# openGemini/openGemini

Measured on NVIDIA H100. Metric: decoded+aggregated rows/s, higher is better.
Workload: dtype f64

## Files before the change

### include/ogpu.h

```cpp
#ifndef OGPU_H
#define OGPU_H

#include <stddef.h>
#include <stdint.h>

#ifdef __cplusplus
extern "C" {
#endif

#define OG_API __attribute__((visibility("default")))

enum {
    OG_OK = 0,
    OG_EOF = 1,
    OG_E_INVAL = -1,
    OG_E_CUDA = -2,
    OG_E_NOMEM = -3,
    OG_E_UNSUPPORTED = -4,
    OG_E_CORRUPT = -5,
    OG_E_ABORTED = -6,
    OG_E_TYPE = -7,
    OG_E_STATE = -8
};

enum { OG_TYPE_INT = 1, OG_TYPE_FLOAT = 3, OG_TYPE_STRING = 4, OG_TYPE_BOOL = 5 };

enum { OG_AGG_COUNT = 1, OG_AGG_SUM = 2, OG_AGG_MIN = 3, OG_AGG_MAX = 4, OG_AGG_FIRST = 5, OG_AGG_LAST = 6 };

enum { OG_F_TERM = 0, OG_F_AND = 1, OG_F_OR = 2 };
enum { OG_OP_LT = 0, OG_OP_LTE = 1, OG_OP_GT = 2, OG_OP_GTE = 3, OG_OP_EQ = 4, OG_OP_NEQ = 5 };

typedef struct og_filter_item {
    int32_t kind;
    int32_t column;
    int32_t op;
    int32_t const_is_float;
    double fval;
    int64_t ival;
} og_filter_item;

typedef struct og_call {
    int32_t func;
    int32_t column;
} og_call;

enum { OG_GROUP_ALL = 0, OG_GROUP_PER_SERIES = 1, OG_GROUP_MAP = 2 };
enum {
    OG_Q_STRICT_ORDER = 1u << 0
    ,
    OG_Q_NO_FUSED = 1u << 1
    ,
    OG_Q_NO_FAST = 1u << 2
    ,
    OG_Q_RESERVED_8 = 1u << 3
    ,
    OG_Q_QUERY_GRID = 1u << 4
};

typedef struct og_query_desc {
    int64_t interval;
    int64_t offset;
    int64_t tmin, tmax;
    int32_t ascending;
    uint32_t n_calls;
    const og_call *calls;
    uint32_t n_filter;
    const og_filter_item *filter;
    int32_t group_mode;
    uint32_t n_groups;
    const uint32_t *series_group;
    int32_t chunk_size;
    uint32_t flags;
} og_query_desc;

typedef struct og_column_desc {
    const char *name;
    int32_t type;
    const uint64_t *page_off;
    const uint32_t *page_len;
} og_column_desc;

enum {
    OG_SHARD_DEVICE_DATA = 1u << 0
};

typedef struct og_shard_desc {
    const uint8_t *data;
    uint64_t data_len;
    uint32_t n_series;
    const uint64_t *sids;
    const uint32_t *series_seg_begin;
    uint32_t n_segments;
    const int64_t *seg_tmin;
    const int64_t *seg_tmax;
    uint32_t n_columns;
    const og_column_desc *columns;
    const uint64_t *time_page_off;
    const uint32_t *time_page_len;
    uint32_t flags;
} og_shard_desc;

typedef struct og_colval_view {
    const uint8_t *val;
    uint64_t val_bytes;
    const uint8_t *bitmap;
    const int64_t *times;
    int32_t type;
    int32_t len;
    int32_t nil_count;
    int32_t bitmap_offset;
} og_colval_view;

typedef struct og_record_view {
    uint32_t n_cols;
    const og_colval_view *cols;
    const int64_t *times;
    int32_t rows;
    uint32_t group;
    uint64_t sid;
} og_record_view;

typedef struct og_dense_col {
    void *values;
    uint8_t *valid;
    int64_t *times;
    int32_t type;
    int32_t func;
} og_dense_col;

typedef struct og_dense_view {
    uint32_t n_groups;
    uint32_t n_buckets;
    int64_t start;
    int64_t interval;
    uint32_t n_cols;
    const og_dense_col *cols;
    void *stream;
} og_dense_view;

typedef struct og_stats {
    uint64_t rows_decoded;
    uint64_t segments_scanned;
    uint64_t page_bytes;
    uint64_t dir_bytes;
    uint64_t out_bytes;
    double kernel_ms;
    double h2d_ms;
    double main_kernel_ms;
    uint32_t kernel_launches;
    int32_t path;
    int32_t il_state;
    int32_t per_series_cells_used;
    double il_build_ms;
    uint64_t il_bytes;
    uint64_t general_segments;
    double merge_ms;
    uint64_t il_packed_segments;
} og_stats;

typedef struct og_shard og_shard;
typedef struct og_query og_query;

OG_API int og_init(int device_ordinal);
OG_API int og_device_count(void);
OG_API const char *og_strerror(int status);
OG_API const char *og_last_error(void);
OG_API const char *og_version(void);
OG_API int og_release_cached_memory(void);

typedef struct og_tssp og_tssp;
OG_API int og_tssp_parse(const uint8_t *file, uint64_t len, og_tssp **out);
OG_API int og_tssp_desc(const og_tssp *t, og_shard_desc *out);
OG_API const char *og_tssp_measurement(const og_tssp *t);
OG_API int og_tssp_time_range(const og_tssp *t, int64_t *min_time, int64_t *max_time);
OG_API void og_tssp_free(og_tssp *t);

OG_API int og_shard_open(const og_shard_desc *desc, og_shard **out);
OG_API void og_shard_close(og_shard *s);
OG_API int og_shard_info(const og_shard *s, uint64_t *n_series, uint64_t *n_segments, uint64_t *n_rows,
                         uint64_t *page_bytes, int64_t *tmin, int64_t *tmax);

enum { OG_FILE_OUT_OF_ORDER = 1u << 0 };
OG_API int og_shard_open_files(const og_shard_desc *files, const uint32_t *file_flags, uint32_t n_files, og_shard **out);
typedef struct og_merge_info {
    uint32_t n_files, n_out_of_order_files;
    uint64_t series_merged;
    uint64_t out_of_order_rows;
    uint64_t rows_replaced;
    uint64_t rows_after_merge;
    uint64_t segments_kept;
    uint64_t segments_rewritten_in, segments_rewritten_out;
    double merge_ms;
} og_merge_info;
OG_API int og_shard_merge_info(const og_shard *s, og_merge_info *out);

OG_API int og_query_create(og_shard *s, const og_query_desc *desc, og_query **out);
OG_API int og_query_run(og_query *q);
OG_API int og_query_next(og_query *q, og_record_view *out);
OG_API int og_query_dense(og_query *q, og_dense_view *out);
OG_API int og_query_stats(const og_query *q, og_stats *out);
OG_API void og_query_abort(og_query *q);
OG_API void og_query_destroy(og_query *q);

OG_API int og_query_merge_dense(og_query *q, const og_dense_view *other);

typedef struct og_comm og_comm;
OG_API int og_comm_unique_id(uint8_t id[128]);
OG_API int og_comm_init_rank(const uint8_t id[128], int rank, int world, og_comm **out);
OG_API void og_comm_destroy(og_comm *c);
OG_API int og_comm_info(const og_comm *c, int *rank, int *world, int *nccl_version);
OG_API int og_comm_allreduce_f64(og_comm *c, double *vals, int n, int op_max);
OG_API int og_query_allreduce(og_query *q, og_comm *c);

OG_API int og_decode_segment(og_shard *s, uint32_t segment, og_record_view *out);
enum { OG_DECODE_DESCENDING = 1u << 0 };
OG_API int og_decode_segment_ex(og_shard *s, uint32_t segment, uint32_t flags, og_record_view *out);
OG_API int og_decode_column_device(og_shard *s, uint32_t column, uint32_t seg_begin, uint32_t seg_end,
                                   void *d_values, uint64_t value_stride_bytes, uint32_t *d_rows_out);

enum { OG_SYNTH_F_HI = 0, OG_SYNTH_F_LO = 1, OG_SYNTH_INT_WALK = 2, OG_SYNTH_BOOL = 3 };
typedef struct og_synth_column {
    int32_t type;
    int32_t dist;
    uint32_t null_permille;
} og_synth_column;
typedef struct og_synth_desc {
    uint32_t n_series;
    uint32_t rows_per_series;
    uint32_t rows_per_segment;
    int64_t t0;
    int64_t dt;
    uint64_t seed;
    uint32_t n_columns;
    const og_synth_column *columns;
    uint32_t series_base;
} og_synth_desc;
OG_API int og_shard_synth(const og_synth_desc *desc, og_shard **out);
typedef struct og_shard_layout {
    uint64_t data_len;
    uint32_t n_series, n_segments, n_columns;
} og_shard_layout;
OG_API int og_shard_layout_get(const og_shard *s, og_shard_layout *out);
OG_API int og_shard_export(const og_shard *s, uint8_t *data, uint64_t *sids, uint32_t *series_seg_begin,
                           int64_t *seg_tmin, int64_t *seg_tmax, uint64_t *page_off ,
                           uint32_t *page_len, int32_t *col_types );

OG_API int og_encode_pages(int32_t type, int32_t is_time, const void *d_values, const uint8_t *d_valid,
                           const uint32_t *d_rows , uint32_t n_segments,
                           uint32_t rows_per_segment, uint8_t *d_out, uint64_t out_cap, uint64_t *d_page_off,
                           uint32_t *d_page_len, uint64_t *total_bytes_out);

typedef struct og_downsampled og_downsampled;
OG_API int og_downsample(og_shard *s, uint32_t column, int64_t interval, int64_t tmin, int64_t tmax, og_downsampled **out);

typedef struct og_downsample_ops {
    int32_t type;
    uint32_t n_funcs;
    const int32_t *funcs;
} og_downsample_ops;
typedef struct og_downsample_desc {
    int64_t interval, tmin, tmax;
    uint32_t n_types;
    const og_downsample_ops *ops;
} og_downsample_desc;
OG_API int og_downsample_shard(og_shard *s, const og_downsample_desc *d, og_downsampled **out);
OG_API int og_downsampled_timing(const og_downsampled *d, double phase_ms[4]);
OG_API int og_downsampled_desc(const og_downsampled *d, og_shard_desc *desc, uint64_t *rows );
OG_API int og_downsampled_export(const og_downsampled *d, uint8_t *host_data );
OG_API void og_downsampled_free(og_downsampled *d);

typedef struct og_tssp_write_desc {
    const char *measurement;
    uint32_t series_begin, series_end;
    uint32_t flags;
} og_tssp_write_desc;
typedef struct og_tssp_image og_tssp_image;
OG_API int og_shard_write_tssp(og_shard *s, const og_tssp_write_desc *d, og_tssp_image **out);
OG_API int og_tssp_image_size(const og_tssp_image *f, uint64_t *bytes);
OG_API int og_tssp_image_export(const og_tssp_image *f, uint8_t *host);
OG_API int og_tssp_image_timing(const og_tssp_image *f, double phase_ms[4]);
OG_API void og_tssp_image_free(og_tssp_image *f);

#ifdef __cplusplus
}
#endif
#endif
```

### opengemini_b200/_lib.py

```python
import ctypes as C
import os

_HERE = os.path.dirname(os.path.abspath(__file__))
LIB_PATH = os.environ.get("OGPU_LIB") or os.path.join(_HERE, "libogpu.so")

OG_OK, OG_EOF = 0, 1
OG_E_INVAL, OG_E_CUDA, OG_E_NOMEM, OG_E_UNSUPPORTED, OG_E_CORRUPT, OG_E_ABORTED, OG_E_TYPE, OG_E_STATE = -1, -2, -3, -4, -5, -6, -7, -8
TYPE_INT, TYPE_FLOAT, TYPE_STRING, TYPE_BOOL = 1, 3, 4, 5
AGG_COUNT, AGG_SUM, AGG_MIN, AGG_MAX, AGG_FIRST, AGG_LAST = 1, 2, 3, 4, 5, 6
F_TERM, F_AND, F_OR = 0, 1, 2
OP_LT, OP_LTE, OP_GT, OP_GTE, OP_EQ, OP_NEQ = 0, 1, 2, 3, 4, 5
GROUP_ALL, GROUP_PER_SERIES, GROUP_MAP = 0, 1, 2
Q_STRICT_ORDER = 1
Q_NO_FUSED = 2
Q_NO_FAST = 4
Q_QUERY_GRID = 16
SYNTH_F_HI, SYNTH_F_LO, SYNTH_INT_WALK, SYNTH_BOOL = 0, 1, 2, 3
SHARD_DEVICE_DATA = 1
FILE_OUT_OF_ORDER = 1

u8p, u32p, u64p, i64p, i32p = C.POINTER(C.c_uint8), C.POINTER(C.c_uint32), C.POINTER(C.c_uint64), C.POINTER(C.c_int64), C.POINTER(C.c_int32)


class FilterItem(C.Structure):
    _fields_ = [("kind", C.c_int32), ("column", C.c_int32), ("op", C.c_int32), ("const_is_float", C.c_int32),
                ("fval", C.c_double), ("ival", C.c_int64)]


class Call(C.Structure):
    _fields_ = [("func", C.c_int32), ("column", C.c_int32)]


class QueryDesc(C.Structure):
    _fields_ = [("interval", C.c_int64), ("offset", C.c_int64), ("tmin", C.c_int64), ("tmax", C.c_int64),
                ("ascending", C.c_int32), ("n_calls", C.c_uint32), ("calls", C.POINTER(Call)),
                ("n_filter", C.c_uint32), ("filter", C.POINTER(FilterItem)), ("group_mode", C.c_int32),
                ("n_groups", C.c_uint32), ("series_group", u32p), ("chunk_size", C.c_int32), ("flags", C.c_uint32)]


class ColumnDesc(C.Structure):
    _fields_ = [("name", C.c_char_p), ("type", C.c_int32), ("page_off", u64p), ("page_len", u32p)]


class ShardDesc(C.Structure):
    _fields_ = [("data", u8p), ("data_len", C.c_uint64), ("n_series", C.c_uint32), ("sids", u64p),
                ("series_seg_begin", u32p), ("n_segments", C.c_uint32), ("seg_tmin", i64p), ("seg_tmax", i64p),
                ("n_columns", C.c_uint32), ("columns", C.POINTER(ColumnDesc)), ("time_page_off", u64p),
                ("time_page_len", u32p), ("flags", C.c_uint32)]


class ColValView(C.Structure):
    _fields_ = [("val", u8p), ("val_bytes", C.c_uint64), ("bitmap", u8p), ("times", i64p), ("type", C.c_int32),
                ("len", C.c_int32), ("nil_count", C.c_int32), ("bitmap_offset", C.c_int32)]


class RecordView(C.Structure):
    _fields_ = [("n_cols", C.c_uint32), ("cols", C.POINTER(ColValView)), ("times", i64p), ("rows", C.c_int32),
                ("group", C.c_uint32), ("sid", C.c_uint64)]


class DenseCol(C.Structure):
    _fields_ = [("values", C.c_void_p), ("valid", C.c_void_p), ("times", C.c_void_p), ("type", C.c_int32), ("func", C.c_int32)]


class DenseView(C.Structure):
    _fields_ = [("n_groups", C.c_uint32), ("n_buckets", C.c_uint32), ("start", C.c_int64), ("interval", C.c_int64),
                ("n_cols", C.c_uint32), ("cols", C.POINTER(DenseCol)), ("stream", C.c_void_p)]


class Stats(C.Structure):
    _fields_ = [("rows_decoded", C.c_uint64), ("segments_scanned", C.c_uint64), ("page_bytes", C.c_uint64),
                ("dir_bytes", C.c_uint64), ("out_bytes", C.c_uint64), ("kernel_ms", C.c_double), ("h2d_ms", C.c_double), ("main_kernel_ms", C.c_double),
                ("kernel_launches", C.c_uint32), ("path", C.c_int32), ("il_state", C.c_int32), ("per_series_cells_used", C.c_int32),
                ("il_build_ms", C.c_double), ("il_bytes", C.c_uint64), ("general_segments", C.c_uint64), ("merge_ms", C.c_double),
                ("il_packed_segments", C.c_uint64)]


class SynthColumn(C.Structure):
    _fields_ = [("type", C.c_int32), ("dist", C.c_int32), ("null_permille", C.c_uint32)]


class SynthDesc(C.Structure):
    _fields_ = [("n_series", C.c_uint32), ("rows_per_series", C.c_uint32), ("rows_per_segment", C.c_uint32),
                ("t0", C.c_int64), ("dt", C.c_int64), ("seed", C.c_uint64), ("n_columns", C.c_uint32),
                ("columns", C.POINTER(SynthColumn)), ("series_base", C.c_uint32)]


class ShardLayout(C.Structure):
    _fields_ = [("data_len", C.c_uint64), ("n_series", C.c_uint32), ("n_segments", C.c_uint32), ("n_columns", C.c_uint32)]


class DownsampleOps(C.Structure):
    _fields_ = [("type", C.c_int32), ("n_funcs", C.c_uint32), ("funcs", i32p)]


class DownsampleDesc(C.Structure):
    _fields_ = [("interval", C.c_int64), ("tmin", C.c_int64), ("tmax", C.c_int64), ("n_types", C.c_uint32),
                ("ops", C.POINTER(DownsampleOps))]


class MergeInfo(C.Structure):
    _fields_ = [("n_files", C.c_uint32), ("n_out_of_order_files", C.c_uint32), ("series_merged", C.c_uint64),
                ("out_of_order_rows", C.c_uint64), ("rows_replaced", C.c_uint64), ("rows_after_merge", C.c_uint64),
                ("segments_kept", C.c_uint64), ("segments_rewritten_in", C.c_uint64), ("segments_rewritten_out", C.c_uint64),
                ("merge_ms", C.c_double)]


class TsspWriteDesc(C.Structure):
    _fields_ = [("measurement", C.c_char_p), ("series_begin", C.c_uint32), ("series_end", C.c_uint32), ("flags", C.c_uint32)]


EXPORTS = [
    "og_init", "og_device_count", "og_strerror", "og_last_error", "og_version", "og_shard_open", "og_shard_close",
    "og_shard_info", "og_query_create", "og_query_run", "og_query_next", "og_query_dense", "og_query_stats",
    "og_query_abort", "og_query_destroy", "og_query_merge_dense", "og_decode_segment", "og_decode_segment_ex", "og_decode_column_device",
    "og_shard_synth", "og_shard_layout_get", "og_shard_export", "og_encode_pages",
    "og_release_cached_memory", "og_comm_unique_id", "og_comm_init_rank", "og_comm_destroy", "og_comm_info", "og_comm_allreduce_f64", "og_query_allreduce",
    "og_downsample", "og_downsampled_desc", "og_downsampled_export", "og_downsampled_free",
    "og_downsample_shard", "og_downsampled_timing",
    "og_tssp_parse", "og_tssp_desc", "og_tssp_measurement", "og_tssp_time_range", "og_tssp_free",
    "og_shard_open_files", "og_shard_merge_info",
    "og_shard_write_tssp", "og_tssp_image_size", "og_tssp_image_export", "og_tssp_image_timing", "og_tssp_image_free",
]

_lib = None


class OgpuError(RuntimeError):
    def __init__(self, status, where):
        self.status = status
        msg = lib().og_last_error().decode(errors="replace")
        super().__init__(f"{where}: {lib().og_strerror(status).decode()} ({status}) {msg}")


def lib():
    global _lib
    if _lib is not None:
        return _lib
    if not os.path.exists(LIB_PATH):
        raise RuntimeError(f"{LIB_PATH} is missing: run `python -c 'import __graft_entry__ as g; g.build()'` "
                           "(nvcc, sm_90a). There is no CPU fallback for the scan/aggregate path.")
    L = C.CDLL(LIB_PATH)
    L.og_strerror.restype = C.c_char_p
    L.og_strerror.argtypes = [C.c_int]
    L.og_last_error.restype = C.c_char_p
    L.og_version.restype = C.c_char_p
    L.og_init.argtypes = [C.c_int]
    L.og_shard_open.argtypes = [C.POINTER(ShardDesc), C.POINTER(C.c_void_p)]
    L.og_shard_open_files.argtypes = [C.POINTER(ShardDesc), u32p, C.c_uint32, C.POINTER(C.c_void_p)]
    L.og_shard_merge_info.argtypes = [C.c_void_p, C.POINTER(MergeInfo)]
    L.og_shard_close.argtypes = [C.c_void_p]
    L.og_shard_close.restype = None
    L.og_shard_info.argtypes = [C.c_void_p, u64p, u64p, u64p, u64p, i64p, i64p]
    L.og_query_create.argtypes = [C.c_void_p, C.POINTER(QueryDesc), C.POINTER(C.c_void_p)]
    L.og_query_run.argtypes = [C.c_void_p]
    L.og_query_next.argtypes = [C.c_void_p, C.POINTER(RecordView)]
    L.og_query_dense.argtypes = [C.c_void_p, C.POINTER(DenseView)]
    L.og_query_stats.argtypes = [C.c_void_p, C.POINTER(Stats)]
    L.og_query_abort.argtypes = [C.c_void_p]
    L.og_query_abort.restype = None
    L.og_query_destroy.argtypes = [C.c_void_p]
    L.og_query_destroy.restype = None
    L.og_query_merge_dense.argtypes = [C.c_void_p, C.POINTER(DenseView)]
    L.og_decode_segment.argtypes = [C.c_void_p, C.c_uint32, C.POINTER(RecordView)]
    L.og_downsample.argtypes = [C.c_void_p, C.c_uint32, C.c_int64, C.c_int64, C.c_int64, C.POINTER(C.c_void_p)]
    L.og_downsample_shard.argtypes = [C.c_void_p, C.POINTER(DownsampleDesc), C.POINTER(C.c_void_p)]
    L.og_downsampled_timing.argtypes = [C.c_void_p, C.POINTER(C.c_double)]
    L.og_downsampled_desc.argtypes = [C.c_void_p, C.POINTER(ShardDesc), C.POINTER(C.c_uint64)]
    L.og_downsampled_export.argtypes = [C.c_void_p, C.c_void_p]
    L.og_downsampled_free.argtypes = [C.c_void_p]
    L.og_downsampled_free.restype = None
    L.og_tssp_parse.argtypes = [C.c_void_p, C.c_uint64, C.POINTER(C.c_void_p)]
    L.og_tssp_desc.argtypes = [C.c_void_p, C.POINTER(ShardDesc)]
    L.og_tssp_measurement.argtypes = [C.c_void_p]
    L.og_tssp_measurement.restype = C.c_char_p
    L.og_tssp_time_range.argtypes = [C.c_void_p, C.POINTER(C.c_int64), C.POINTER(C.c_int64)]
    L.og_tssp_free.argtypes = [C.c_void_p]
    L.og_tssp_free.restype = None
    L.og_shard_write_tssp.argtypes = [C.c_void_p, C.POINTER(TsspWriteDesc), C.POINTER(C.c_void_p)]
    L.og_tssp_image_size.argtypes = [C.c_void_p, u64p]
    L.og_tssp_image_export.argtypes = [C.c_void_p, C.c_void_p]
    L.og_tssp_image_timing.argtypes = [C.c_void_p, C.POINTER(C.c_double)]
    L.og_tssp_image_free.argtypes = [C.c_void_p]
    L.og_tssp_image_free.restype = None
    L.og_decode_segment_ex.argtypes = [C.c_void_p, C.c_uint32, C.c_uint32, C.POINTER(RecordView)]
    L.og_decode_column_device.argtypes = [C.c_void_p, C.c_uint32, C.c_uint32, C.c_uint32, C.c_void_p, C.c_uint64, C.c_void_p]
    L.og_shard_synth.argtypes = [C.POINTER(SynthDesc), C.POINTER(C.c_void_p)]
    L.og_shard_layout_get.argtypes = [C.c_void_p, C.POINTER(ShardLayout)]
    L.og_shard_export.argtypes = [C.c_void_p, C.c_void_p, C.c_void_p, C.c_void_p, C.c_void_p, C.c_void_p, C.c_void_p, C.c_void_p, C.c_void_p]
    L.og_encode_pages.argtypes = [C.c_int32, C.c_int32, C.c_void_p, C.c_void_p, C.c_void_p, C.c_uint32, C.c_uint32,
                                  C.c_void_p, C.c_uint64, C.c_void_p, C.c_void_p, u64p]
    L.og_comm_unique_id.argtypes = [C.c_void_p]
    L.og_comm_init_rank.argtypes = [C.c_void_p, C.c_int, C.c_int, C.POINTER(C.c_void_p)]
    L.og_comm_destroy.argtypes = [C.c_void_p]
    L.og_comm_destroy.restype = None
    L.og_comm_info.argtypes = [C.c_void_p, C.POINTER(C.c_int), C.POINTER(C.c_int), C.POINTER(C.c_int)]
    L.og_comm_allreduce_f64.argtypes = [C.c_void_p, C.POINTER(C.c_double), C.c_int, C.c_int]
    L.og_query_allreduce.argtypes = [C.c_void_p, C.c_void_p]
    _lib = L
    return L


def check(status, where):
    if status != OG_OK:
        raise OgpuError(status, where)
```

### opengemini_b200/csrc/agg_kernels.cuh

```cuda
#pragma once
#include "agg_ops.cuh"
#include "decode.cuh"
#include "internal.h"

namespace ogpu {

#define OG_NO_BUCKET 0xFFFFFFFFu

struct DirP {
    const uint8_t *data;
    const uint64_t *page_off;
    const uint32_t *page_len;
    const uint32_t *seg_series, *seg_rows, *series_seg_begin;
    const int64_t *seg_tmin, *seg_tmax;
    uint32_t n_segments, n_columns;
};

struct ChunkP {
    uint32_t series_begin, series_end;
    uint32_t seg_begin, seg_end;
    Tri cells[OG_MAX_CALLS];
    uint32_t nb;
    Tri edges[OG_MAX_CALLS];
    uint32_t *edge_bucket;
    Tri gcells[OG_MAX_CALLS];
    uint32_t gc_cols, gc_tail0, gc_edge0, gc_col0;
    uint32_t J;
    int *err;
    int *flags;
};

__device__ __forceinline__ size_t cell_idx(const ChunkP &ch, uint32_t series, uint32_t b) { return (size_t)(series - ch.series_begin) * ch.nb + b; }

__device__ __forceinline__ void report_err(int *err, int code, uint32_t seg) {
    if (atomicCAS(&err[0], 0, code) == 0) err[1] = (int)seg;
}

__device__ __forceinline__ void store_part(const Tri &a, size_t i, const Part &p) {
    a.val[i] = p.v; a.ok[i] = (uint8_t)p.ok;
    if (a.tim) a.tim[i] = p.t;
}
__device__ __forceinline__ Part load_part(const Tri &a, size_t i) {
    Part p; p.ok = a.ok[i]; p.v = a.val[i]; p.t = a.tim ? a.tim[i] : 0; return p;
}
__device__ __forceinline__ void store_cell(const ChunkP &ch, int call, uint32_t series, uint32_t b, const Part &p) {
    store_part(ch.cells[call], cell_idx(ch, series, b), p);
    ch.flags[0] = 1;
}

struct SegWindows {
    const QueryP &q; const ChunkP &ch;
    const uint32_t seg; const size_t e; const uint32_t series;
    uint32_t cur_b = OG_NO_BUCKET, head_b = OG_NO_BUCKET; bool head_done = false;
    int64_t we = 0;

    __device__ __forceinline__ SegWindows(const QueryP &q_, const ChunkP &ch_, uint32_t seg_, size_t e_, uint32_t series_)
        : q(q_), ch(ch_), seg(seg_), e(e_), series(series_) {}
    template <int NC> __device__ __forceinline__ void flush(const Part (&parts)[NC], bool final) {
        if (cur_b == OG_NO_BUCKET) return;
#pragma unroll
        for (int c = 0; c < NC; c++) {
            if (!head_done) store_part(ch.edges[c], e, parts[c]);
            else if (final) store_part(ch.edges[c], e + 1, parts[c]);
            else if (parts[c].ok) store_cell(ch, c, series, cur_b, parts[c]);
        }
        if (!head_done) { head_done = true; head_b = cur_b; }
    }
    template <int NC> __device__ __forceinline__ bool enter(int64_t t, Part (&parts)[NC]) {
        if (cur_b != OG_NO_BUCKET && t < we) return true;
        flush(parts, false);
        cur_b = bucket_of(t, q.start, q.interval);
        if (cur_b >= q.n_buckets) { report_err(ch.err, D_CORRUPT, seg); cur_b = OG_NO_BUCKET; return false; }
        we = q.start + (int64_t)(cur_b + 1) * q.interval;
#pragma unroll
        for (int c = 0; c < NC; c++) parts[c] = part_empty();
        return true;
    }
    template <int NC> __device__ __forceinline__ void end(const Part (&parts)[NC]) {
        const uint32_t last_b = cur_b;
        const bool single = !head_done;
        flush(parts, true);
        ch.edge_bucket[e] = head_b;
        ch.edge_bucket[e + 1] = (single || head_b == OG_NO_BUCKET) ? OG_NO_BUCKET : last_b;
        if (head_b != OG_NO_BUCKET) ch.flags[1] = 1;
    }
};

__global__ void k_validate(DirP d, const int32_t *col_types, uint32_t *seg_rows, unsigned long long *totals ,
                           uint32_t *max_rows, int *err) {
    uint32_t seg = blockIdx.x * blockDim.x + threadIdx.x;
    if (seg >= d.n_segments) return;
    size_t ti = (size_t)d.n_columns * d.n_segments + seg;
    TimeDesc t;
    int rc = parse_time_page(d.data + d.page_off[ti], d.page_len[ti], t);
    if (rc == D_OK && t.rows == 0) rc = D_CORRUPT;
    if (rc == D_OK) {
        int64_t last = t.t0; bool unsorted = false;
        if (t.kind == 0) last = (int64_t)((uint64_t)t.t0 + (uint64_t)(t.rows - 1) * t.delta);
        else {
            TimeIter it; it.init(t);
            for (uint32_t i = 0; i < t.rows; i++) { const int64_t x = it.next(); unsorted |= x < last; last = x; }
            it.finish(); rc = it.err;
        }
        if (rc == D_OK && (t.t0 < d.seg_tmin[seg] || last > d.seg_tmax[seg] || last < t.t0 || unsorted)) rc = D_CORRUPT;
    }
    if (rc != D_OK) { report_err(err, rc, seg); seg_rows[seg] = 0; return; }
    seg_rows[seg] = t.rows;
    unsigned long long bytes = d.page_len[ti];
    for (uint32_t c = 0; c < d.n_columns; c++) {
        size_t pi = (size_t)c * d.n_segments + seg;
        uint32_t len = d.page_len[pi];
        if (len == 0) continue;
        bytes += len;
        PageHdr h;
        rc = parse_field_header(d.data + d.page_off[pi], len, col_types[c], t.rows, h);
        if (rc == D_OK && h.rows != t.rows) rc = D_CORRUPT;
        if (rc == D_OK && h.bitmap && hdr_valid_rows(h) != h.rows - h.nil_count) rc = D_CORRUPT;
        if (rc == D_OK && !h.one_row && h.nil_count < h.rows) {
            if (h.block_len < 1) rc = D_CORRUPT;
            else {
                int tag = __ldg(h.block) >> 4, ty = col_types[c];
                if (ty == OG_TYPE_FLOAT) rc = (tag == 0 || tag == 3 || tag == 4 || tag == 5) ? D_OK : (tag == 1 || tag == 2 || tag == 6) ? D_UNSUPPORTED : D_CORRUPT;
                else if (ty == OG_TYPE_INT) rc = (tag == 1 || tag == 2 || tag == 4) ? D_OK : tag == 3 ? D_UNSUPPORTED : D_CORRUPT;
                else if (ty == OG_TYPE_BOOL) rc = tag == 1 ? D_OK : D_CORRUPT;
                else if (ty == OG_TYPE_STRING) rc = D_OK;
                else rc = D_UNSUPPORTED;
            }
        }
        if (rc != D_OK) { report_err(err, rc, seg); return; }
    }
    atomicAdd(&totals[0], (unsigned long long)t.rows);
    atomicAdd(&totals[1], bytes);
    atomicMax(max_rows, t.rows);
    if (t.kind != 0 && t.kind != 3) atomicAdd(&totals[2], 1ull);
}

__global__ void k_fill_seg_series(const uint32_t *series_seg_begin, uint32_t n_series, uint32_t *seg_series) {
    uint32_t s = blockIdx.x;
    if (s >= n_series) return;
    for (uint32_t g = series_seg_begin[s] + threadIdx.x; g < series_seg_begin[s + 1]; g += blockDim.x) seg_series[g] = s;
}

struct TileP {
    uint32_t tile_begin, tile_end, R;
    uint32_t S;
    uint64_t *vals[OG_MAX_COLS];
    uint8_t *okb[OG_MAX_COLS];
    int64_t *times;
    uint8_t *keep;
};

__global__ void k_decode_tile(DirP d, QueryP q, TileP tp, int *err) {
    uint32_t seg = tp.tile_begin + blockIdx.x * blockDim.x + threadIdx.x;
    if (seg >= tp.tile_end) return;
    uint32_t slot = blockIdx.y;
    const size_t base = seg - tp.tile_begin, S = tp.S;
    uint32_t rows = d.seg_rows[seg];
    if (slot == q.n_cols) {
        size_t ti = (size_t)d.n_columns * d.n_segments + seg;
        TimeDesc t;
        int rc = parse_time_page(d.data + d.page_off[ti], d.page_len[ti], t);
        if (rc == D_OK) {
            TimeIter it; it.init(t);
            for (uint32_t i = 0; i < t.rows; i++) tp.times[base + i * S] = it.next();
            it.finish(); rc = it.err;
        }
        if (rc != D_OK) report_err(err, rc, seg);
        return;
    }
    size_t pi = (size_t)q.col_index[slot] * d.n_segments + seg;
    uint64_t *out = tp.vals[slot] + base; uint8_t *okb = tp.okb[slot] + base;
    ColIter it;
    it.init(d.data + d.page_off[pi], d.page_len[pi], q.col_type[slot], rows);
    for (uint32_t i = 0; i < rows; i++) { uint64_t v = 0; okb[i * S] = it.next(v); out[i * S] = v; }
    it.finish();
    if (it.err != D_OK) report_err(err, it.err, seg);
}

__device__ __forceinline__ bool term_pass(const FilterP &f, uint64_t raw) {
    if (f.type == OG_TYPE_FLOAT || (f.type == OG_TYPE_INT && f.const_is_float)) {
        double v = f.type == OG_TYPE_FLOAT ? u2d(raw) : (double)(int64_t)raw;
        double c = f.const_is_float ? f.fval : (double)f.ival;
        switch (f.op) {
        case OG_OP_LT: return !(v >= c);
        case OG_OP_LTE: return !(v > c);
        case OG_OP_GT: return !(v <= c);
        case OG_OP_GTE: return !(v < c);
        case OG_OP_EQ: return !(v != c);
        default: return !(v == c);
        }
    }
    int64_t v = f.type == OG_TYPE_BOOL ? (int64_t)(raw != 0) : (int64_t)raw, c = f.ival;
    switch (f.op) {
    case OG_OP_LT: return !(v >= c);
    case OG_OP_LTE: return !(v > c);
    case OG_OP_GT: return !(v <= c);
    case OG_OP_GTE: return !(v < c);
    case OG_OP_EQ: return !(v != c);
    default: return !(v == c);
    }
}

__global__ void k_filter_tile(DirP d, QueryP q, TileP tp) {
    size_t idx = (size_t)blockIdx.x * blockDim.x + threadIdx.x;
    size_t total = (size_t)tp.S * tp.R;
    if (idx >= total) return;
    uint32_t row = (uint32_t)(idx / tp.S), sl = (uint32_t)(idx % tp.S);
    if (sl >= tp.tile_end - tp.tile_begin) return;
    if (row >= d.seg_rows[tp.tile_begin + sl]) { tp.keep[idx] = 0; return; }
    int64_t t = tp.times[idx];
    bool keep = t >= q.tmin && t <= q.tmax;
    if (keep && q.n_filter) {
        uint32_t stack = 0; int sp = 0;
        for (uint32_t i = 0; i < q.n_filter; i++) {
            const FilterP &f = q.filter[i];
            if (f.kind == OG_F_TERM) {
                bool pass = tp.okb[f.col_slot][idx] && term_pass(f, tp.vals[f.col_slot][idx]);
                stack |= (uint32_t)pass << sp; sp++;
            } else {
                uint32_t b = (stack >> (sp - 1)) & 1, a = (stack >> (sp - 2)) & 1;
                uint32_t r = f.kind == OG_F_AND ? (a & b) : (a | b);
                sp -= 2; stack &= ~(3u << sp); stack |= r << sp; sp++;
            }
        }
        keep = stack & 1;
    }
    tp.keep[idx] = keep;
}

__global__ void k_window_reduce(DirP d, QueryP q, TileP tp, ChunkP ch) {
    uint32_t sl = blockIdx.x * blockDim.x + threadIdx.x;
    uint32_t seg = tp.tile_begin + sl;
    if (seg >= tp.tile_end) return;
    const uint32_t rows = d.seg_rows[seg], series = d.seg_series[seg];
    const size_t S = tp.S, e = 2 * (size_t)(seg - ch.seg_begin);
    Part parts[OG_MAX_CALLS];
    uint32_t cur_b = OG_NO_BUCKET, head_b = OG_NO_BUCKET; bool head_done = false;
    int64_t we = 0;
    auto flush = [&](bool final) {
        if (cur_b == OG_NO_BUCKET) return;
        for (uint32_t c = 0; c < q.n_calls; c++) {
            if (!head_done) store_part(ch.edges[c], e, parts[c]);
            else if (final) store_part(ch.edges[c], e + 1, parts[c]);
            else if (parts[c].ok) store_cell(ch, (int)c, series, cur_b, parts[c]);
        }
        if (!head_done) { head_done = true; head_b = cur_b; }
    };
    for (uint32_t r = 0; r < rows; r++) {
        const size_t ix = (size_t)r * S + sl;
        const int64_t t = tp.times[ix];
        if (t < q.tmin) continue;
        if (t > q.tmax) break;
        if (cur_b == OG_NO_BUCKET || t >= we) {
            flush(false);
            cur_b = bucket_of(t, q.start, q.interval);
            if (cur_b >= q.n_buckets) { report_err(ch.err, D_CORRUPT, seg); cur_b = OG_NO_BUCKET; break; }
            we = q.start + (int64_t)(cur_b + 1) * q.interval;
#pragma unroll
            for (uint32_t c = 0; c < OG_MAX_CALLS; c++) parts[c] = part_empty();
        }
        if (!tp.keep[ix]) continue;
#pragma unroll
        for (uint32_t c = 0; c < OG_MAX_CALLS; c++) {
            if (c >= q.n_calls) break;
            const CallP &cp = q.calls[c];
            if (tp.okb[cp.col_slot][ix]) acc_row(cp.func, cp.type, parts[c], tp.vals[cp.col_slot][ix], t);
        }
    }
    flush(true);
    ch.edge_bucket[e] = head_b;
    ch.edge_bucket[e + 1] = (head_b == OG_NO_BUCKET || cur_b == head_b) ? OG_NO_BUCKET : cur_b;
}

struct EdgeRuns { uint32_t hb, tb, s_end; bool head_leader; };
__device__ __forceinline__ EdgeRuns edge_runs(const DirP &d, const ChunkP &ch, uint32_t seg, uint32_t series) {
    EdgeRuns r;
    const uint32_t s_first = d.series_seg_begin[series];
    r.s_end = d.series_seg_begin[series + 1];
    const uint32_t *eb = ch.edge_bucket;
    const size_t e = 2 * (size_t)(seg - ch.seg_begin);
    r.hb = eb[e]; r.tb = eb[e + 1];
    r.head_leader = true;
    if (r.hb != OG_NO_BUCKET && seg > s_first) {
        const size_t pe = e - 2;
        const uint32_t pb = eb[pe + 1] != OG_NO_BUCKET ? eb[pe + 1] : eb[pe];
        if (pb != OG_NO_BUCKET && pb == r.hb) r.head_leader = false;
    }
    return r;
}
__device__ __forceinline__ Part edge_stitch(const QueryP &q, const ChunkP &ch, const EdgeRuns &r, uint32_t seg, int which, uint32_t c) {
    const CallP &cp = q.calls[c];
    const uint32_t *eb = ch.edge_bucket;
    const size_t e = 2 * (size_t)(seg - ch.seg_begin);
    const uint32_t b = which == 0 ? r.hb : r.tb;
    Part acc = load_part(ch.edges[c], e + which);
    if (which == 1 || r.tb == OG_NO_BUCKET) {
        for (uint32_t nx = seg + 1; nx < r.s_end; nx++) {
            const size_t ne = 2 * (size_t)(nx - ch.seg_begin);
            if (eb[ne] != b) break;
            acc = series_merge(cp.func, cp.type, acc, load_part(ch.edges[c], ne));
            if (eb[ne + 1] != OG_NO_BUCKET) break;
        }
    }
    return acc;
}

__global__ void k_fix_edges(DirP d, QueryP q, ChunkP ch) {
    uint32_t seg = ch.seg_begin + blockIdx.x * blockDim.x + threadIdx.x;
    if (seg >= ch.seg_end) return;
    const uint32_t series = d.seg_series[seg];
    const EdgeRuns r = edge_runs(d, ch, seg, series);
    if (r.hb == OG_NO_BUCKET) return;
    for (int which = 0; which < 2; which++) {
        if (which == 0 && !r.head_leader) continue;
        if (which == 1 && r.tb == OG_NO_BUCKET) continue;
        const uint32_t b = which == 0 ? r.hb : r.tb;
        if (b >= q.n_buckets) { report_err(ch.err, D_CORRUPT, seg); continue; }
        for (uint32_t c = 0; c < q.n_calls; c++) {
            const Part acc = edge_stitch(q, ch, r, seg, which, c);
            if (acc.ok) store_cell(ch, (int)c, series, b, acc);
        }
    }
}

__device__ __forceinline__ Part shfl_xor_part(const Part &p, int o, bool with_time) {
    Part r; r.v = __shfl_xor_sync(0xffffffffu, p.v, o); r.ok = __shfl_xor_sync(0xffffffffu, p.ok, o);
    r.t = with_time ? __shfl_xor_sync(0xffffffffu, p.t, o) : 0;
    return r;
}
__device__ __forceinline__ Part warp_fold(int func, int type, bool multi, Part p, bool with_time) {
#pragma unroll
    for (int o = 16; o; o >>= 1) { const Part other = shfl_xor_part(p, o, with_time); group_update(func, type, multi, p, other); }
    return p;
}
__device__ __forceinline__ bool call_has_time(const QueryP &q, uint32_t c) { return q.calls[c].func >= OG_AGG_MIN && !(q.multi && q.calls[c].func <= OG_AGG_MAX); }
__device__ __forceinline__ int call_ftype(const QueryP &q, uint32_t c) { return q.calls[c].func == OG_AGG_COUNT ? OG_TYPE_INT : q.calls[c].type; }

__global__ void k_fix_edges_fold(DirP d, QueryP q, ChunkP ch) {
    if (ch.flags[1] == 0) return;
    const uint32_t w = (blockIdx.x * blockDim.x + threadIdx.x) >> 5, lane = threadIdx.x & 31;
    const uint32_t n_blk = (ch.series_end - ch.series_begin + 31) / 32;
    if (w >= n_blk * ch.J) return;
    const uint32_t blk = w / ch.J, j = w % ch.J;
    const uint32_t series = ch.series_begin + blk * 32 + lane;
    const bool in = series < ch.series_end;
    const uint32_t seg = in ? d.series_seg_begin[series] + j : 0;
    EdgeRuns r; r.hb = r.tb = OG_NO_BUCKET; r.head_leader = false; r.s_end = 0;
    if (in) r = edge_runs(d, ch, seg, series);
    const uint32_t n_bk = (ch.gc_cols - ch.gc_edge0) / 3;
    for (int which = 0; which < 2; which++) {
        const uint32_t gcol = ch.gc_edge0 + (which ? 2u : (j & 1u)) * n_bk + ch.series_begin / 32 + blk - ch.gc_col0;
        const bool has = r.hb != OG_NO_BUCKET && (which == 0 ? r.head_leader : r.tb != OG_NO_BUCKET);
        const uint32_t b = which == 0 ? r.hb : r.tb;
        const uint32_t hm = __ballot_sync(0xffffffffu, has);
        if (hm == 0) continue;
        const int leader = __ffs(hm) - 1;
        const uint32_t bL = __shfl_sync(0xffffffffu, b, leader);
        const bool unif = __all_sync(0xffffffffu, !has || b == bL) && bL < q.n_buckets;
        if (!unif && has && b >= q.n_buckets) { report_err(ch.err, D_CORRUPT, seg); continue; }
        for (uint32_t c = 0; c < q.n_calls; c++) {
            Part acc = part_empty();
            if (has) acc = edge_stitch(q, ch, r, seg, which, c);
            if (unif) {
                acc = warp_fold(q.calls[c].func, call_ftype(q, c), q.multi != 0, acc, call_has_time(q, c));
                if ((int)lane == leader && acc.ok) store_part(ch.gcells[c], (size_t)bL * ch.gc_cols + gcol, acc);
            } else if (has && acc.ok) store_cell(ch, (int)c, series, b, acc);
        }
    }
}

struct GroupP {
    const uint32_t *grp_begin;
    const uint32_t *grp_series;
    uint32_t n_groups;
    Tri dense[OG_MAX_CALLS];
};

__global__ void k_merge_groups(QueryP q, ChunkP ch, GroupP gp) {
    if (ch.flags[0] == 0) return;
    size_t idx = (size_t)blockIdx.x * blockDim.x + threadIdx.x;
    size_t total = (size_t)gp.n_groups * q.n_buckets;
    if (idx >= total) return;
    uint32_t g = (uint32_t)(idx / q.n_buckets), b = (uint32_t)(idx % q.n_buckets);
    uint32_t lo = gp.grp_begin[g], hi = gp.grp_begin[g + 1];
    {
        uint32_t a = lo, z = hi;
        while (a < z) { uint32_t m = (a + z) >> 1; if (gp.grp_series[m] < ch.series_begin) a = m + 1; else z = m; }
        lo = a;
    }
    if (lo >= hi || gp.grp_series[lo] >= ch.series_end) return;
    {
        const uint32_t c = blockIdx.y;
        const CallP &cp = q.calls[c];
        Part acc = load_part(gp.dense[c], idx);
        const Tri cells = ch.cells[c];
        constexpr int U = 16;
        for (uint32_t i = lo; i < hi; i += U) {
            uint32_t okv[U]; uint64_t vv[U]; int64_t tt[U];
#pragma unroll
            for (int u = 0; u < U; u++) {
                uint32_t ii = i + u;
                uint32_t s = ii < hi ? gp.grp_series[ii] : 0xffffffffu;
                bool in = s < ch.series_end;
                size_t ci = in ? cell_idx(ch, s, b) : 0;
                okv[u] = in ? cells.ok[ci] : 0;
                vv[u] = okv[u] ? cells.val[ci] : 0;
                tt[u] = (okv[u] && cells.tim) ? cells.tim[ci] : 0;
            }
#pragma unroll
            for (int u = 0; u < U; u++) {
                if (!okv[u]) continue;
                Part p; p.ok = 1; p.v = vv[u]; p.t = tt[u];
                group_update(cp.func, cp.out_type == OG_TYPE_INT && cp.func == OG_AGG_COUNT ? OG_TYPE_INT : cp.type, q.multi != 0, acc, p);
            }
        }
        store_part(gp.dense[c], idx, acc);
    }
}

__global__ void k_merge_per_series(QueryP q, ChunkP ch, GroupP gp) {
    const uint32_t c = blockIdx.y;
    const size_t n = (size_t)(ch.series_end - ch.series_begin) * q.n_buckets;
    const size_t i = (size_t)blockIdx.x * blockDim.x + threadIdx.x;
    if (i >= n) return;
    const CallP &cp = q.calls[c];
    const int ftype = cp.out_type == OG_TYPE_INT && cp.func == OG_AGG_COUNT ? OG_TYPE_INT : cp.type;
    const uint32_t b = (uint32_t)(i % q.n_buckets);
    Part p; p.ok = ch.cells[c].ok[i]; p.v = p.ok ? ch.cells[c].val[i] : 0; p.t = (p.ok && ch.cells[c].tim) ? ch.cells[c].tim[i] : 0;
    Part a; a.v = 0; a.ok = 0; a.t = q.multi ? 0 : q.start + (int64_t)b * q.interval;
    group_update(cp.func, ftype, q.multi != 0, a, p);
    store_part(gp.dense[c], (size_t)ch.series_begin * q.n_buckets + i, a);
}

#define OG_MERGE_SB 256u
__global__ void __launch_bounds__(128) k_merge_all_blocks(QueryP q, ChunkP ch, GroupP gp) {
    if (ch.flags[0] == 0) return;
    const uint32_t b = blockIdx.x * blockDim.x + threadIdx.x, blk = blockIdx.y, c = blockIdx.z;
    if (b >= q.n_buckets) return;
    const uint32_t nS = ch.series_end - ch.series_begin;
    const uint32_t s0 = blk * OG_MERGE_SB, s1 = min(nS, s0 + OG_MERGE_SB);
    const int func = q.calls[c].func, ftype = call_ftype(q, c);
    const bool multi = q.multi != 0;
    const Tri cells = ch.cells[c];
    Part acc = part_empty();
    constexpr int U = 8;
    for (uint32_t s = s0; s < s1; s += U) {
        uint32_t okv[U]; uint64_t vv[U]; int64_t tt[U];
#pragma unroll
        for (int u = 0; u < U; u++) {
            const bool in = s + u < s1;
            const size_t ci = in ? (size_t)(s + u) * ch.nb + b : 0;
            okv[u] = in ? cells.ok[ci] : 0;
            vv[u] = okv[u] ? cells.val[ci] : 0;
            tt[u] = (okv[u] && cells.tim) ? cells.tim[ci] : 0;
        }
#pragma unroll
        for (int u = 0; u < U; u++) {
            if (!okv[u]) continue;
            Part p; p.ok = 1; p.v = vv[u]; p.t = tt[u];
            group_update(func, ftype, multi, acc, p);
        }
    }
    if (acc.ok) store_part(ch.gcells[c], (size_t)b * ch.gc_cols + blk, acc);
}

__global__ void k_merge_folded(QueryP q, ChunkP ch, GroupP gp) {
    const uint32_t b = (blockIdx.x * blockDim.x + threadIdx.x) >> 5, lane = threadIdx.x & 31, c = blockIdx.y;
    if (b >= q.n_buckets) return;
    const int func = q.calls[c].func, ftype = call_ftype(q, c);
    const bool wt = call_has_time(q, c), multi = q.multi != 0;
    const Tri g = ch.gcells[c];
    Part acc = part_empty();
    const size_t row = (size_t)b * ch.gc_cols;
    for (uint32_t col = lane; col < ch.gc_cols; col += 32) {
        if (!g.ok[row + col]) continue;
        Part p; p.ok = 1; p.v = g.val[row + col]; p.t = wt ? g.tim[row + col] : 0;
        group_update(func, ftype, multi, acc, p);
    }
    acc = warp_fold(func, ftype, multi, acc, wt);
    if (lane == 0 && acc.ok) {
        Part a = load_part(gp.dense[c], b);
        group_update(func, ftype, multi, a, acc);
        store_part(gp.dense[c], b, a);
    }
}

__global__ void k_init_dense(QueryP q, GroupP gp) {
    size_t idx = (size_t)blockIdx.x * blockDim.x + threadIdx.x;
    size_t total = (size_t)gp.n_groups * q.n_buckets;
    if (idx >= total) return;
    uint32_t b = (uint32_t)(idx % q.n_buckets);
    for (uint32_t c = 0; c < q.n_calls; c++) {
        gp.dense[c].val[idx] = 0; gp.dense[c].ok[idx] = 0;
        if (gp.dense[c].tim) gp.dense[c].tim[idx] = q.multi ? 0 : q.start + (int64_t)b * q.interval;
    }
}

__global__ void k_merge_dense(QueryP q, GroupP mine, GroupP other) {
    size_t idx = (size_t)blockIdx.x * blockDim.x + threadIdx.x;
    size_t total = (size_t)mine.n_groups * q.n_buckets;
    if (idx >= total) return;
    for (uint32_t c = 0; c < q.n_calls; c++) {
        const CallP &cp = q.calls[c];
        Part a = load_part(mine.dense[c], idx), p = load_part(other.dense[c], idx);
        group_update(cp.func, cp.func == OG_AGG_COUNT ? OG_TYPE_INT : cp.type, q.multi != 0, a, p);
        store_part(mine.dense[c], idx, a);
    }
}

}
```

### opengemini_b200/csrc/api.cu

```cuda
#include <algorithm>
#include <cstdarg>
#include <cstdio>
#include <cstring>
#include <numeric>

#include "agg_kernels.cuh"
#include "il_build.cuh"
#include "fused_multi.cuh"
#include "fused_cols.cuh"
#include "snappy_load.cuh"
#include <cub/device/device_scan.cuh>
#include <cub/device/device_radix_sort.cuh>
#include "internal.h"

namespace ogpu {

static thread_local char g_err[512] = "";
void set_error(const char *fmt, ...) {
    va_list ap; va_start(ap, fmt); vsnprintf(g_err, sizeof g_err, fmt, ap); va_end(ap);
}
int cuda_fail(cudaError_t e, const char *what, const char *file, int line) {
    set_error("CUDA error %d (%s) at %s:%d: %s", (int)e, cudaGetErrorString(e), file, line, what);
    return OG_E_CUDA;
}
static int g_device = -1;
cudaError_t dev_mem_info(size_t *free_b, size_t *total_b) {
    cudaError_t e = cudaMemGetInfo(free_b, total_b);
    if (e != cudaSuccess) return e;
    cudaMemPool_t pool; uint64_t reserved = 0, used = 0; int dev = 0;
    if (cudaGetDevice(&dev) == cudaSuccess && cudaDeviceGetDefaultMemPool(&pool, dev) == cudaSuccess &&
        cudaMemPoolGetAttribute(pool, cudaMemPoolAttrReservedMemCurrent, &reserved) == cudaSuccess &&
        cudaMemPoolGetAttribute(pool, cudaMemPoolAttrUsedMemCurrent, &used) == cudaSuccess && reserved > used) *free_b += (size_t)(reserved - used);
    else cudaGetLastError();
    return cudaSuccess;
}

static int map_dev_err(int code) {
    switch (code) {
    case D_UNSUPPORTED: return OG_E_UNSUPPORTED;
    case D_TYPE: return OG_E_TYPE;
    case D_WATCHDOG: return OG_E_CUDA;
    default: return OG_E_CORRUPT;
    }
}

template <class T> static int dalloc(T **p, size_t n) {
    *p = nullptr;
    if (n == 0) n = 1;
    cudaError_t e = dev_malloc((void **)p, n * sizeof(T));
    if (e != cudaSuccess) { set_error("cudaMalloc(%zu bytes) failed: %s", n * sizeof(T), cudaGetErrorString(e)); return e == cudaErrorMemoryAllocation ? OG_E_NOMEM : OG_E_CUDA; }
    return OG_OK;
}

static DirP make_dir(const og_shard *s) {
    DirP d;
    d.data = s->d_data; d.page_off = s->d_page_off; d.page_len = s->d_page_len; d.seg_series = s->d_seg_series;
    d.seg_rows = s->d_seg_rows; d.series_seg_begin = s->d_series_seg_begin; d.seg_tmin = s->d_tmin; d.seg_tmax = s->d_tmax;
    d.n_segments = s->n_segments; d.n_columns = s->n_columns;
    return d;
}

int shard_finalize(og_shard *s, bool scan_snappy) {
    int rc;
    s->il.resize(s->n_columns);
    if ((rc = dalloc(&s->d_seg_series, s->n_segments))) return rc;
    if ((rc = dalloc(&s->d_seg_rows, s->n_segments))) return rc;
    int32_t *d_types; unsigned long long *d_tot; uint32_t *d_max; int *d_err;
    if ((rc = dalloc(&d_types, s->n_columns))) return rc;
    if ((rc = dalloc(&d_tot, 3))) return rc;
    if ((rc = dalloc(&d_max, 1))) return rc;
    if ((rc = dalloc(&d_err, 2))) return rc;
    CU(cudaMemcpy(d_types, s->col_types.data(), s->n_columns * sizeof(int32_t), cudaMemcpyHostToDevice));
    CU(cudaMemset(d_tot, 0, 24)); CU(cudaMemset(d_max, 0, 4)); CU(cudaMemset(d_err, 0, 8));
    if (s->n_series) k_fill_seg_series<<<s->n_series, 128>>>(s->d_series_seg_begin, s->n_series, s->d_seg_series);
    if (s->n_segments && scan_snappy) {
        const size_t n_pages = (size_t)(s->n_columns + 1) * s->n_segments;
        uint32_t *tr_size; unsigned long long *d_cnt;
        if ((rc = dalloc(&tr_size, n_pages))) return rc;
        if ((rc = dalloc(&d_cnt, 3))) { dev_free(tr_size); return rc; }
        struct Free2 { void *a, *b; ~Free2() { dev_free(a); dev_free(b); } } f2{tr_size, d_cnt};
        CU(cudaMemset(d_cnt, 0, 24));
        k_snappy_scan<<<(s->n_segments + 127) / 128, 128>>>(make_dir(s), d_types, tr_size, d_cnt);
        unsigned long long cnt[3];
        CU(cudaMemcpy(cnt, d_cnt, 24, cudaMemcpyDeviceToHost));
        if (cnt[0]) {
            if (!s->owns_data) { set_error("shard has %llu Snappy pages: they are transcoded at open, which needs a library-owned copy of the data (do not pass OG_SHARD_DEVICE_DATA)", cnt[0]); return OG_E_UNSUPPORTED; }
            uint64_t *tr_off; void *tmp = nullptr; size_t tb = 0;
            if ((rc = dalloc(&tr_off, n_pages))) return rc;
            struct Free1 { void *a; ~Free1() { dev_free(a); } } f1{tr_off};
            CU(cub::DeviceScan::ExclusiveSum(nullptr, tb, tr_size, tr_off, (int)n_pages));
            CU(dev_malloc((void **)&tmp, tb ? tb : 1));
            struct Free3 { void *a; ~Free3() { dev_free(a); } } f3{tmp};
            CU(cub::DeviceScan::ExclusiveSum(tmp, tb, tr_size, tr_off, (int)n_pages));
            const uint64_t new_base = (s->data_len + 15) & ~15ull, new_len = new_base + cnt[2];
            uint8_t *nd;
            if ((rc = dalloc(&nd, (size_t)new_len + 1024))) return rc;
            CU(cudaMemcpy(nd, s->d_data, s->data_len, cudaMemcpyDeviceToDevice));
            CU(cudaMemset(nd + s->data_len, 0, new_len + 1024 - s->data_len));
            k_snappy_transcode<<<(unsigned)((n_pages + 127) / 128), 128>>>(make_dir(s), tr_size, tr_off, nd, new_base, s->d_page_off, s->d_page_len, d_err);
            CU(cudaGetLastError());
            CU(cudaDeviceSynchronize());
            dev_free(s->d_data); s->d_data = nd; s->data_len = new_len;
            s->snappy_pages = cnt[0]; s->snappy_bytes_in = cnt[1]; s->snappy_bytes_out = cnt[2];
        }
    }
    if (s->n_segments) k_validate<<<(s->n_segments + 127) / 128, 128>>>(make_dir(s), d_types, s->d_seg_rows, d_tot, d_max, d_err);
    CU(cudaGetLastError());
    unsigned long long tot[3]; int err[2]; uint32_t mx;
    CU(cudaMemcpy(tot, d_tot, 24, cudaMemcpyDeviceToHost));
    CU(cudaMemcpy(err, d_err, 8, cudaMemcpyDeviceToHost));
    CU(cudaMemcpy(&mx, d_max, 4, cudaMemcpyDeviceToHost));
    dev_free(d_types); dev_free(d_tot); dev_free(d_max); dev_free(d_err);
    if (err[0]) {
        set_error("segment %d: %s page (device validation code %d)", err[1], err[0] == D_UNSUPPORTED ? "unsupported codec in" : err[0] == D_TYPE ? "type mismatch in" : "corrupt", err[0]);
        return map_dev_err(err[0]);
    }
    s->n_rows = tot[0]; s->page_bytes = tot[1] - s->snappy_bytes_out + s->snappy_bytes_in;
    s->max_seg_rows = mx; s->irregular_time_pages = tot[2];
    return OG_OK;
}

}

using namespace ogpu;

extern "C" {

OG_API int og_device_count(void) { int n = 0; if (cudaGetDeviceCount(&n) != cudaSuccess) return 0; return n; }

OG_API int og_init(int device_ordinal) {
    int n = og_device_count();
    if (n <= 0) { set_error("no CUDA device visible: libogpu has no CPU path"); return OG_E_CUDA; }
    if (device_ordinal < 0 || device_ordinal >= n) { set_error("device ordinal %d out of range (%d devices)", device_ordinal, n); return OG_E_INVAL; }
    CU(cudaSetDevice(device_ordinal));
    CU(cudaFree(0));
    {
        cudaMemPool_t pool; uint64_t thr = ~0ull;
        if (cudaDeviceGetDefaultMemPool(&pool, device_ordinal) == cudaSuccess) cudaMemPoolSetAttribute(pool, cudaMemPoolAttrReleaseThreshold, &thr);
        else cudaGetLastError();
    }
    g_device = device_ordinal;
    return OG_OK;
}

OG_API const char *og_strerror(int st) {
    switch (st) {
    case OG_OK: return "ok";
    case OG_EOF: return "end of stream";
    case OG_E_INVAL: return "invalid argument";
    case OG_E_CUDA: return "CUDA failure or no device bound";
    case OG_E_NOMEM: return "out of device memory";
    case OG_E_UNSUPPORTED: return "unsupported codec or option on the GPU path";
    case OG_E_CORRUPT: return "corrupt page";
    case OG_E_ABORTED: return "query aborted";
    case OG_E_TYPE: return "column type mismatch";
    case OG_E_STATE: return "call sequence error";
    default: return "unknown status";
    }
}
OG_API const char *og_last_error(void) { return g_err; }
OG_API const char *og_version(void) { return "ogpu 0.2 (sm_90a)"; }
OG_API int og_release_cached_memory(void) {
    if (g_device < 0) return OG_OK;
    CU(cudaSetDevice(g_device));
    CU(cudaDeviceSynchronize());
    cudaMemPool_t pool;
    CU(cudaDeviceGetDefaultMemPool(&pool, g_device));
    CU(cudaMemPoolTrimTo(pool, 0));
    return OG_OK;
}

}
namespace ogpu {
int ensure_device() {
    if (g_device < 0) { int rc = og_init(0); if (rc != OG_OK) return rc; }
    else CU(cudaSetDevice(g_device));
    return OG_OK;
}
}
static int need_device() { return ogpu::ensure_device(); }
extern "C" {

OG_API void og_shard_close(og_shard *s) {
    if (!s) return;
    if (s->owns_data && s->d_data) dev_free(s->d_data);
    dev_free(s->d_series_seg_begin); dev_free(s->d_seg_series); dev_free(s->d_seg_rows); dev_free(s->d_tmin); dev_free(s->d_tmax);
    dev_free(s->d_page_off); dev_free(s->d_page_len); dev_free(s->d_sids);
    if (s->h_seg_buf) cudaFreeHost(s->h_seg_buf);
    if (s->d_seg_buf) dev_free(s->d_seg_buf);
    for (auto &c : s->il) {
        dev_free(c.words); dev_free(c.grp_off); dev_free(c.grp_rows); dev_free(c.grp_col); dev_free(c.lane_seg); dev_free(c.lane_rows); dev_free(c.lane_win);
        dev_free(c.lane_series); dev_free(c.lane_t0); dev_free(c.lane_dt); dev_free(c.gen_list);
    }
    delete s;
}

}
namespace ogpu {
int check_desc(const og_shard_desc *d) {
    if (d->n_columns > 64 || (d->n_segments && (!d->seg_tmin || !d->seg_tmax || !d->time_page_off || !d->time_page_len)) || (d->n_series && !d->series_seg_begin)) { set_error("bad shard descriptor"); return OG_E_INVAL; }
    for (uint32_t s = 0; s < d->n_series; s++) if (d->series_seg_begin[s] > d->series_seg_begin[s + 1]) { set_error("series_seg_begin not monotone at %u", s); return OG_E_INVAL; }
    if (d->n_series && d->series_seg_begin[d->n_series] != d->n_segments) { set_error("series_seg_begin[n_series] != n_segments"); return OG_E_INVAL; }
    for (uint32_t c = 0; c < d->n_columns; c++)
        if (d->columns[c].type != OG_TYPE_INT && d->columns[c].type != OG_TYPE_FLOAT && d->columns[c].type != OG_TYPE_BOOL && d->columns[c].type != OG_TYPE_STRING) {
            set_error("column %u: unknown column type %d", c, d->columns[c].type); return OG_E_UNSUPPORTED;
        }
    for (size_t c = 0; c <= d->n_columns; c++) {
        const uint64_t *po = c < d->n_columns ? d->columns[c].page_off : d->time_page_off;
        const uint32_t *pl = c < d->n_columns ? d->columns[c].page_len : d->time_page_len;
        for (size_t g = 0; g < d->n_segments; g++)
            if (po[g] + pl[g] > d->data_len) { set_error("column %zu segment %zu: page [%llu,+%u) outside data (%llu bytes)", c, g, (unsigned long long)po[g], pl[g], (unsigned long long)d->data_len); return OG_E_INVAL; }
    }
    for (uint32_t sr = 0; sr < d->n_series; sr++)
        for (uint32_t g = d->series_seg_begin[sr]; g < d->series_seg_begin[sr + 1]; g++)
            if (d->seg_tmin[g] > d->seg_tmax[g] || (g > d->series_seg_begin[sr] && d->seg_tmin[g] <= d->seg_tmax[g - 1])) {
                set_error("series %u: segment %u is not time-ordered (only ordered TSSP files are supported)", sr, g); return OG_E_UNSUPPORTED;
            }
    return OG_OK;
}
}
extern "C" {

OG_API int og_shard_open(const og_shard_desc *d, og_shard **out) {
    if (!d || !out) { set_error("null argument"); return OG_E_INVAL; }
    *out = nullptr;
    int rc = need_device(); if (rc) return rc;
    if ((rc = check_desc(d))) return rc;
    og_shard *s = new og_shard;
    s->device = g_device; s->n_series = d->n_series; s->n_segments = d->n_segments; s->n_columns = d->n_columns;
    s->data_len = d->data_len;
    for (uint32_t c = 0; c < d->n_columns; c++) {
        s->col_types.push_back(d->columns[c].type);
        s->col_names.push_back(d->columns[c].name ? d->columns[c].name : "");
    }
    s->sids.assign(d->sids, d->sids + d->n_series);
    s->h_series_seg_begin.assign(d->series_seg_begin, d->series_seg_begin + d->n_series + 1);
    size_t nseg = d->n_segments, ncol1 = (size_t)d->n_columns + 1;
    std::vector<uint64_t> off(ncol1 * nseg); std::vector<uint32_t> len(ncol1 * nseg);
    for (size_t c = 0; c < ncol1; c++) {
        const uint64_t *po = c < d->n_columns ? d->columns[c].page_off : d->time_page_off;
        const uint32_t *pl = c < d->n_columns ? d->columns[c].page_len : d->time_page_len;
        for (size_t g = 0; g < nseg; g++) { off[c * nseg + g] = po[g]; len[c * nseg + g] = pl[g]; }
    }
    s->tmin = INT64_MAX; s->tmax = INT64_MIN;
    if (d->n_series)
        for (uint32_t g = d->series_seg_begin[0]; g < d->series_seg_begin[d->n_series]; g++) { s->tmin = std::min(s->tmin, d->seg_tmin[g]); s->tmax = std::max(s->tmax, d->seg_tmax[g]); }
#define TRY(x) do { rc = (x); if (rc) { og_shard_close(s); return rc; } } while (0)
#define TRYCU(x) do { cudaError_t e_ = (x); if (e_ != cudaSuccess) { rc = cuda_fail(e_, #x, __FILE__, __LINE__); og_shard_close(s); return rc; } } while (0)
    if (d->flags & OG_SHARD_DEVICE_DATA) { s->d_data = (uint8_t *)d->data; s->owns_data = false; }
    else {
        TRY(dalloc(&s->d_data, d->data_len + 1024));
        TRYCU(cudaMemcpy(s->d_data, d->data, d->data_len, cudaMemcpyHostToDevice));
        TRYCU(cudaMemset(s->d_data + d->data_len, 0, 1024));
    }
    TRY(dalloc(&s->d_series_seg_begin, (size_t)d->n_series + 1));
    TRY(dalloc(&s->d_tmin, nseg)); TRY(dalloc(&s->d_tmax, nseg));
    TRY(dalloc(&s->d_page_off, ncol1 * nseg)); TRY(dalloc(&s->d_page_len, ncol1 * nseg)); TRY(dalloc(&s->d_sids, (size_t)d->n_series));
    TRYCU(cudaMemcpy(s->d_series_seg_begin, d->series_seg_begin, ((size_t)d->n_series + 1) * 4, cudaMemcpyHostToDevice));
    TRYCU(cudaMemcpy(s->d_tmin, d->seg_tmin, nseg * 8, cudaMemcpyHostToDevice));
    TRYCU(cudaMemcpy(s->d_tmax, d->seg_tmax, nseg * 8, cudaMemcpyHostToDevice));
    TRYCU(cudaMemcpy(s->d_page_off, off.data(), off.size() * 8, cudaMemcpyHostToDevice));
    TRYCU(cudaMemcpy(s->d_page_len, len.data(), len.size() * 4, cudaMemcpyHostToDevice));
    TRYCU(cudaMemcpy(s->d_sids, d->sids, (size_t)d->n_series * 8, cudaMemcpyHostToDevice));
    TRY(shard_finalize(s, true));
    *out = s;
    return OG_OK;
}

OG_API int og_shard_info(const og_shard *s, uint64_t *n_series, uint64_t *n_segments, uint64_t *n_rows, uint64_t *page_bytes, int64_t *tmin, int64_t *tmax) {
    if (!s) return OG_E_INVAL;
    if (n_series) *n_series = s->n_series;
    if (n_segments) *n_segments = s->n_segments;
    if (n_rows) *n_rows = s->n_rows;
    if (page_bytes) *page_bytes = s->page_bytes;
    if (tmin) *tmin = s->tmin;
    if (tmax) *tmax = s->tmax;
    return OG_OK;
}

OG_API int og_shard_layout_get(const og_shard *s, og_shard_layout *out) {
    if (!s || !out) return OG_E_INVAL;
    out->data_len = s->data_len; out->n_series = s->n_series; out->n_segments = s->n_segments; out->n_columns = s->n_columns;
    return OG_OK;
}

OG_API int og_shard_export(const og_shard *s, uint8_t *data, uint64_t *sids, uint32_t *series_seg_begin, int64_t *seg_tmin,
                           int64_t *seg_tmax, uint64_t *page_off, uint32_t *page_len, int32_t *col_types) {
    if (!s) return OG_E_INVAL;
    CU(cudaSetDevice(s->device));
    size_t nseg = s->n_segments, ncol1 = (size_t)s->n_columns + 1;
    if (data) CU(cudaMemcpy(data, s->d_data, s->data_len, cudaMemcpyDeviceToHost));
    if (sids) memcpy(sids, s->sids.data(), s->sids.size() * 8);
    if (series_seg_begin) memcpy(series_seg_begin, s->h_series_seg_begin.data(), s->h_series_seg_begin.size() * 4);
    if (seg_tmin) CU(cudaMemcpy(seg_tmin, s->d_tmin, nseg * 8, cudaMemcpyDeviceToHost));
    if (seg_tmax) CU(cudaMemcpy(seg_tmax, s->d_tmax, nseg * 8, cudaMemcpyDeviceToHost));
    if (page_off) CU(cudaMemcpy(page_off, s->d_page_off, ncol1 * nseg * 8, cudaMemcpyDeviceToHost));
    if (page_len) CU(cudaMemcpy(page_len, s->d_page_len, ncol1 * nseg * 4, cudaMemcpyDeviceToHost));
    if (col_types) memcpy(col_types, s->col_types.data(), s->col_types.size() * 4);
    return OG_OK;
}

static const int64_t MIN_TIME = INT64_MIN + 2, MAX_TIME = INT64_MAX - 1;
static void window_of(int64_t interval, int64_t offset, int64_t tmin, int64_t tmax, int64_t t, int64_t *s, int64_t *e) {
    if (interval == 0) { *s = tmin; *e = tmax + 1; return; }
    t -= offset;
    int64_t dt = t % interval;
    if (dt < 0) dt += interval;
    int64_t st = ((int64_t)((uint64_t)MIN_TIME + (uint64_t)dt) >= t) ? MIN_TIME : t - dt;
    st += offset;
    int64_t d2 = interval - dt;
    int64_t en = (MAX_TIME - d2 <= t) ? MAX_TIME : t + d2;
    en += offset;
    *s = st; *e = en;
}
static bool window_clamped(int64_t interval, int64_t offset, int64_t t) {
    const __int128 x = (__int128)t - offset;
    __int128 r = x % interval;
    if (r < 0) r += interval;
    const __int128 s = x - r, e = s + interval;
    return s < MIN_TIME || e > MAX_TIME || s + offset < INT64_MIN || e + offset > INT64_MAX;
}

}
namespace { void free_plan(void *plan); }
extern "C" {
void og_query_free_merge_state(void *p);
OG_API void og_query_destroy(og_query *q) {
    if (!q) return;
    if (q->merge_state) og_query_free_merge_state(q->merge_state);
    free_plan(q->plan);
    for (void *p : q->scratch) dev_free(p);
    for (int c = 0; c < OG_MAX_CALLS; c++) { dev_free(q->dense[c].val); dev_free(q->dense[c].ok); dev_free(q->dense[c].tim); }
    dev_free(q->d_group_of_series);
    if (q->ev0) cudaEventDestroy(q->ev0);
    if (q->ev1) cudaEventDestroy(q->ev1);
    for (cudaEvent_t e : q->main_ev) cudaEventDestroy(e);
    if (q->stream) cudaStreamDestroy(q->stream);
    delete q;
}

OG_API int og_query_create(og_shard *s, const og_query_desc *d_in, og_query **out) {
    if (!s || !d_in || !out) { set_error("null argument"); return OG_E_INVAL; }
    *out = nullptr;
    og_query_desc d_clamped = *d_in;
    d_clamped.tmin = std::max(d_in->tmin, MIN_TIME); d_clamped.tmax = std::min(d_in->tmax, MAX_TIME);
    const og_query_desc *d = &d_clamped;
    CU(cudaSetDevice(s->device));
    if (d->n_calls == 0 || d->n_calls > OG_MAX_CALLS) { set_error("n_calls must be 1..%d", OG_MAX_CALLS); return OG_E_INVAL; }
    if (d->n_filter > OG_MAX_FILTER) { set_error("filter too long (max %d items)", OG_MAX_FILTER); return OG_E_INVAL; }
    if (d->interval < 0 || d->tmin > d->tmax) { set_error("bad interval or time range"); return OG_E_INVAL; }
    og_query *q = new og_query;
    q->sh = s; q->desc = *d;
    q->calls.assign(d->calls, d->calls + d->n_calls);
    if (d->n_filter) q->filter.assign(d->filter, d->filter + d->n_filter);
    q->desc.calls = q->calls.data(); q->desc.filter = q->filter.data();
    QueryP &p = q->qp;
    memset(&p, 0, sizeof p);
    auto slot_of = [&](int col) -> int {
        for (uint32_t i = 0; i < p.n_cols; i++) if (p.col_index[i] == col) return (int)i;
        if (p.n_cols >= OG_MAX_COLS) return -1;
        p.col_index[p.n_cols] = col; p.col_type[p.n_cols] = s->col_types[col];
        return (int)p.n_cols++;
    };
    for (uint32_t i = 0; i < d->n_calls; i++) {
        const og_call &c = d->calls[i];
        if (c.column < 0 || (uint32_t)c.column >= s->n_columns || c.func < OG_AGG_COUNT || c.func > OG_AGG_LAST) { set_error("call %u: bad column or function", i); delete q; return OG_E_INVAL; }
        int type = s->col_types[c.column];
        if (type == OG_TYPE_STRING && c.func != OG_AGG_COUNT) { set_error("call %u: only count() is pushed down for string columns (their values are never decoded on the GPU path)", i); delete q; return OG_E_UNSUPPORTED; }
        if (c.func == OG_AGG_SUM && type == OG_TYPE_BOOL) { set_error("sum() over a boolean column (unsupported sum iterator type, series_call_processor.go:140)"); delete q; return OG_E_INVAL; }
        int sl = slot_of(c.column);
        if (sl < 0) { set_error("too many distinct columns"); delete q; return OG_E_INVAL; }
        p.calls[i].func = c.func; p.calls[i].col_slot = sl; p.calls[i].type = type;
        p.calls[i].out_type = c.func == OG_AGG_COUNT ? OG_TYPE_INT : type;
    }
    p.n_calls = d->n_calls; p.multi = d->n_calls > 1;
    int sp = 0;
    for (uint32_t i = 0; i < d->n_filter; i++) {
        const og_filter_item &f = d->filter[i];
        FilterP &fp = p.filter[i];
        fp.kind = f.kind;
        if (f.kind == OG_F_TERM) {
            if (f.column < 0 || (uint32_t)f.column >= s->n_columns || f.op < OG_OP_LT || f.op > OG_OP_NEQ) { set_error("filter item %u: bad column or op", i); delete q; return OG_E_INVAL; }
            if (s->col_types[f.column] == OG_TYPE_STRING) { set_error("filter item %u: WHERE on a string column is not pushed down", i); delete q; return OG_E_UNSUPPORTED; }
            int sl = slot_of(f.column);
            if (sl < 0) { set_error("too many distinct columns"); delete q; return OG_E_INVAL; }
            fp.col_slot = sl; fp.op = f.op; fp.type = s->col_types[f.column]; fp.const_is_float = f.const_is_float; fp.fval = f.fval; fp.ival = f.ival;
            sp++;
        } else if (f.kind == OG_F_AND || f.kind == OG_F_OR) {
            if (sp < 2) { set_error("filter RPN underflow at item %u", i); delete q; return OG_E_INVAL; }
            sp--;
        } else { set_error("filter item %u: bad kind", i); delete q; return OG_E_INVAL; }
    }
    if (d->n_filter && sp != 1) { set_error("filter RPN does not reduce to one value"); delete q; return OG_E_INVAL; }
    p.n_filter = d->n_filter;
    int64_t gmin = std::max(d->tmin, s->tmin), gmax = std::min(d->tmax, s->tmax);
    bool overlap = gmin <= gmax;
    if (!overlap) gmin = gmax = d->tmin;
    if (d->flags & OG_Q_QUERY_GRID) {
        if (d_in->tmin <= MIN_TIME || d_in->tmax >= MAX_TIME) { set_error("OG_Q_QUERY_GRID needs a bounded time range"); delete q; return OG_E_INVAL; }
        gmin = d->tmin; gmax = d->tmax; overlap = true;
    }
    int64_t s0, e0, s1, e1;
    if (d->interval == 0) { s0 = gmin; e0 = gmax + 1; s1 = s0; e1 = e0; }
    else {
        if (overlap && (window_clamped(d->interval, d->offset, gmin) || window_clamped(d->interval, d->offset, gmax))) {
            set_error("the first or last window of the range is clamped at the int64 time limits"); delete q; return OG_E_UNSUPPORTED;
        }
        window_of(d->interval, d->offset, d->tmin, d->tmax, gmin, &s0, &e0);
        window_of(d->interval, d->offset, d->tmin, d->tmax, gmax + 1, &s1, &e1);
    }
    p.tmin = d->tmin; p.tmax = d->tmax; p.start = s0; p.interval = e0 - s0;
    if (p.interval <= 0) { set_error("degenerate window"); delete q; return OG_E_INVAL; }
    uint64_t nb = d->interval ? (uint64_t)(e1 - s0) / (uint64_t)p.interval : 1;
    if (nb == 0 || nb > 0x7fffffffull) { set_error("query range yields %llu buckets", (unsigned long long)nb); delete q; return OG_E_INVAL; }
    p.n_buckets = (uint32_t)nb;
    q->n_groups = d->group_mode == OG_GROUP_ALL ? 1 : d->group_mode == OG_GROUP_PER_SERIES ? s->n_series : d->n_groups;
    if (d->group_mode == OG_GROUP_MAP) {
        if (!d->series_group || d->n_groups == 0) { set_error("OG_GROUP_MAP needs series_group and n_groups"); delete q; return OG_E_INVAL; }
        q->series_group.assign(d->series_group, d->series_group + s->n_series);
        for (uint32_t g : q->series_group) if (g >= d->n_groups) { set_error("series_group entry out of range"); delete q; return OG_E_INVAL; }
    } else if (d->group_mode != OG_GROUP_ALL && d->group_mode != OG_GROUP_PER_SERIES) { set_error("bad group_mode"); delete q; return OG_E_INVAL; }
    if (q->n_groups == 0) q->n_groups = 1;
    cudaError_t e = cudaStreamCreateWithFlags(&q->stream, cudaStreamNonBlocking);
    if (e != cudaSuccess) { delete q; return cuda_fail(e, "cudaStreamCreate", __FILE__, __LINE__); }
    cudaEventCreate(&q->ev0); cudaEventCreate(&q->ev1);
    *out = q;
    return OG_OK;
}

OG_API void og_query_abort(og_query *q) { if (q) q->aborted = 1; }

}
namespace {
struct Plan {
    ChunkP ch; TileP tp; GroupP gp;
    bool fused;
    bool cols;
    bool multi;
    bool fast;
    bool blockmerge;
    bool fold;
    int fm; bool times;
    IlP il;
    const og_shard::IlCol *ic;
};
void free_plan(void *plan) { delete (Plan *)plan; }
template <class T> int salloc(og_query *q, T **p, size_t n) { int rc = dalloc(p, n); if (rc == OG_OK) q->scratch.push_back(*p); return rc; }

template <int NC> void launch_fused(const DirP &d, const QueryP &p, const ChunkP &ch, const uint32_t *list, uint32_t n, cudaStream_t st) {
    if (n) k_fused_segment<NC><<<(n + 127) / 128, 128, 0, st>>>(d, p, ch, list, n);
}
template <int FM, bool TIMES> void launch_fast_t(bool fold, const IlP &il, uint32_t g0, uint32_t g1, const QueryP &p, const ChunkP &ch, cudaStream_t st) {
    constexpr uint32_t WPB = OG_FAST_THREADS / 32;
    dim3 grid((g1 - g0 + WPB - 1) / WPB), block(OG_FAST_THREADS);
    if (fold) k_fused_il<FM, TIMES, true><<<grid, block, WPB * il_acc_bytes(p.n_calls, TIMES), st>>>(p, ch, il, g0, g1);
    else k_fused_il<FM, TIMES, false><<<grid, block, 0, st>>>(p, ch, il, g0, g1);
}
void launch_fast(int fm, bool times, bool fold, const IlP &il, uint32_t g0, uint32_t g1, const QueryP &p, const ChunkP &ch, cudaStream_t st) {
    if (g1 <= g0) return;
    if (!times) {
        switch (fm) {
        case FM_SUM | FM_COUNT: return launch_fast_t<FM_SUM | FM_COUNT, false>(fold, il, g0, g1, p, ch, st);
        case FM_SUM | FM_COUNT | FM_MAX: return launch_fast_t<FM_SUM | FM_COUNT | FM_MAX, false>(fold, il, g0, g1, p, ch, st);
        case FM_SUM | FM_COUNT | FM_MIN | FM_MAX: return launch_fast_t<FM_SUM | FM_COUNT | FM_MIN | FM_MAX, false>(fold, il, g0, g1, p, ch, st);
        case FM_COUNT: return launch_fast_t<FM_COUNT, false>(fold, il, g0, g1, p, ch, st);
        default: break;
        }
    } else {
        switch (fm) {
        case FM_MAX | FM_COUNT: return launch_fast_t<FM_MAX | FM_COUNT, true>(fold, il, g0, g1, p, ch, st);
        case FM_MIN | FM_COUNT: return launch_fast_t<FM_MIN | FM_COUNT, true>(fold, il, g0, g1, p, ch, st);
        default: break;
        }
    }
    return launch_fast_t<63, true>(fold, il, g0, g1, p, ch, st);
}

template <int NCOL, int NCALL> void launch_multi_t(const QueryP &p, const DirP &d, const ChunkP &ch, uint32_t nseg, cudaStream_t st) {
    bool simple = true;
    for (uint32_t c = 0; c < p.n_calls; c++) simple &= p.calls[c].func == OG_AGG_COUNT || p.calls[c].func == OG_AGG_SUM;
    const unsigned gb = (nseg + 127) / 128;
    if (simple) k_fused_multi<NCOL, NCALL, true><<<gb, 128, 0, st>>>(d, p, ch);
    else k_fused_multi<NCOL, NCALL, false><<<gb, 128, 0, st>>>(d, p, ch);
}
template <int NCOL> void launch_multi_c(const QueryP &p, const DirP &d, const ChunkP &ch, uint32_t nseg, cudaStream_t st) {
    switch (p.n_calls) {
    case 1: return launch_multi_t<NCOL, 1>(p, d, ch, nseg, st);
    case 2: return launch_multi_t<NCOL, 2>(p, d, ch, nseg, st);
    case 3: return launch_multi_t<NCOL, 3>(p, d, ch, nseg, st);
    case 4: return launch_multi_t<NCOL, 4>(p, d, ch, nseg, st);
    case 5: return launch_multi_t<NCOL, 5>(p, d, ch, nseg, st);
    case 6: return launch_multi_t<NCOL, 6>(p, d, ch, nseg, st);
    case 7: return launch_multi_t<NCOL, 7>(p, d, ch, nseg, st);
    default: return launch_multi_t<NCOL, 8>(p, d, ch, nseg, st);
    }
}
void launch_cols(const QueryP &p, const DirP &d, const ChunkP &ch, uint32_t nseg, cudaStream_t st) {
    bool simple = true;
    for (uint32_t c = 0; c < p.n_calls; c++) simple &= p.calls[c].func == OG_AGG_COUNT || p.calls[c].func == OG_AGG_SUM;
    const unsigned gb = (nseg + 127) / 128;
    if (simple) k_fused_cols<true><<<gb, 128, 0, st>>>(d, p, ch);
    else k_fused_cols<false><<<gb, 128, 0, st>>>(d, p, ch);
}
void launch_multi(const QueryP &p, const DirP &d, const ChunkP &ch, uint32_t nseg, cudaStream_t st) {
    switch (p.n_cols) {
    case 1: return launch_multi_c<1>(p, d, ch, nseg, st);
    case 2: return launch_multi_c<2>(p, d, ch, nseg, st);
    case 3: return launch_multi_c<3>(p, d, ch, nseg, st);
#ifdef OG_WIDE_MULTI
    case 5: return launch_multi_c<5>(p, d, ch, nseg, st);
    case 6: return launch_multi_c<6>(p, d, ch, nseg, st);
    case 7: return launch_multi_c<7>(p, d, ch, nseg, st);
    case 8: return launch_multi_c<8>(p, d, ch, nseg, st);
#endif
    default: return launch_multi_c<4>(p, d, ch, nseg, st);
    }
}

struct TmpBufs { std::vector<void *> v; ~TmpBufs() { for (void *p : v) dev_free(p); } template <class T> int get(T **p, size_t n) { int rc = dalloc(p, n); if (rc == OG_OK) v.push_back(*p); return rc; } };

int ensure_il(og_shard *s, int col, cudaStream_t st) {
    std::lock_guard<std::mutex> lock(s->il_mu);
    if (s->il.size() != s->n_columns) s->il.resize(s->n_columns);
    og_shard::IlCol &ic = s->il[col];
    if (ic.state != 0) return OG_OK;
    ic.state = -1;
    if (s->n_segments == 0 || s->col_types[col] != OG_TYPE_FLOAT) return OG_OK;
    const uint32_t nseg = s->n_segments;
    uint32_t J = s->n_series ? s->h_series_seg_begin[1] - s->h_series_seg_begin[0] : 0;
    for (uint32_t i = 0; i < s->n_series && J; i++) if (s->h_series_seg_begin[i + 1] - s->h_series_seg_begin[i] != J) J = 0;
    const uint32_t n_super = J ? (s->n_series + OG_IL_SUPER - 1) / OG_IL_SUPER : 1;
    const uint64_t n_dom64 = J ? (uint64_t)n_super * J : 1;
    if (n_dom64 >= (1ull << 31)) return OG_OK;
    const uint32_t n_dom = (uint32_t)n_dom64;
    int rc;
    struct Ev { cudaEvent_t e = nullptr; Ev() { cudaEventCreate(&e); } ~Ev() { if (e) cudaEventDestroy(e); } } ev0, ev1;
    cudaEventRecord(ev0.e, st);
    TmpBufs tmp;
    IlScanOut so{};
    uint32_t *seg_words; uint64_t *keys2; uint32_t *vals2;
    if ((rc = tmp.get(&so.seg_win, nseg)) || (rc = tmp.get(&so.n_packed, 1)) ||
        (rc = tmp.get(&seg_words, nseg)) || (rc = tmp.get(&so.seg_t0, nseg)) || (rc = tmp.get(&so.seg_dt, nseg)) || (rc = tmp.get(&so.keys, nseg)) ||
        (rc = tmp.get(&so.vals, nseg)) || (rc = tmp.get(&keys2, nseg)) || (rc = tmp.get(&vals2, nseg)) || (rc = tmp.get(&so.dom_cnt, n_dom))) return rc;
    so.seg_words = seg_words;
    if ((rc = tmp.get(&so.misaligned, 1))) return rc;
    CU(cudaMemsetAsync(so.dom_cnt, 0, (size_t)n_dom * 4, st));
    CU(cudaMemsetAsync(so.misaligned, 0, 4, st));
    CU(cudaMemsetAsync(so.n_packed, 0, 8, st));
    DirP d = make_dir(s);
    k_il_scan<<<(nseg + 255) / 256, 256, 0, st>>>(d, col, s->col_types[col], J, so);
    CU(cudaGetLastError());
    int dbits = 1; while ((1ull << dbits) < n_dom64 + 1) dbits++;
    {
        size_t tb = 0;
        CU(cub::DeviceRadixSort::SortPairs(nullptr, tb, so.keys, keys2, so.vals, vals2, (int)nseg, 0, (int)OG_IL_WORD_BITS + dbits, st));
        void *dtmp; if ((rc = tmp.get((uint8_t **)&dtmp, tb))) return rc;
        CU(cub::DeviceRadixSort::SortPairs(dtmp, tb, so.keys, keys2, so.vals, vals2, (int)nseg, 0, (int)OG_IL_WORD_BITS + dbits, st));
    }
    std::vector<uint32_t> dom_cnt(n_dom); uint32_t misaligned = 1; unsigned long long n_packed = 0;
    CU(cudaMemcpyAsync(dom_cnt.data(), so.dom_cnt, (size_t)n_dom * 4, cudaMemcpyDeviceToHost, st));
    CU(cudaMemcpyAsync(&misaligned, so.misaligned, 4, cudaMemcpyDeviceToHost, st));
    CU(cudaMemcpyAsync(&n_packed, so.n_packed, 8, cudaMemcpyDeviceToHost, st));
    CU(cudaStreamSynchronize(st));
    std::vector<uint32_t> elem_first(n_dom), grp_first(n_dom);
    uint64_t n_elig = 0, ng64 = 0;
    for (uint32_t i = 0; i < n_dom; i++) { elem_first[i] = (uint32_t)n_elig; grp_first[i] = (uint32_t)ng64; n_elig += dom_cnt[i]; ng64 += (dom_cnt[i] + 31) / 32; }
    const uint32_t n_gen = nseg - (uint32_t)n_elig;
    if (n_gen) {
        if ((rc = dalloc(&ic.gen_list, (size_t)n_gen))) return rc;
        CU(cudaMemcpyAsync(ic.gen_list, vals2 + n_elig, (size_t)n_gen * 4, cudaMemcpyDeviceToDevice, st));
        ic.gen_host.resize(n_gen);
        CU(cudaMemcpyAsync(ic.gen_host.data(), vals2 + n_elig, (size_t)n_gen * 4, cudaMemcpyDeviceToHost, st));
        CU(cudaStreamSynchronize(st));
    }
    if (n_elig == 0) return OG_OK;
    const uint32_t ng = (uint32_t)ng64;
    ic.n_groups = ng; ic.J = J; ic.aligned = J != 0 && misaligned == 0; ic.n_super = n_super; ic.cols_per_super = OG_IL_SUPER / 32 + 1;
    ic.super_grp_first.assign(n_super + 1, ng);
    for (uint32_t sp = 0; sp < n_super; sp++) ic.super_grp_first[sp] = grp_first[J ? sp * J : 0];
    uint32_t *d_elem_first, *d_grp_first;
    if ((rc = tmp.get(&d_elem_first, n_dom)) || (rc = tmp.get(&d_grp_first, n_dom))) return rc;
    CU(cudaMemcpyAsync(d_elem_first, elem_first.data(), (size_t)n_dom * 4, cudaMemcpyHostToDevice, st));
    CU(cudaMemcpyAsync(d_grp_first, grp_first.data(), (size_t)n_dom * 4, cudaMemcpyHostToDevice, st));
    const size_t n_slots = (size_t)ng * 32;
    if ((rc = dalloc(&ic.lane_seg, n_slots)) || (rc = dalloc(&ic.lane_rows, n_slots)) || (rc = dalloc(&ic.lane_win, n_slots)) || (rc = dalloc(&ic.lane_series, n_slots)) ||
        (rc = dalloc(&ic.lane_t0, n_slots)) || (rc = dalloc(&ic.lane_dt, n_slots)) || (rc = dalloc(&ic.grp_col, (size_t)ng)) ||
        (rc = dalloc(&ic.grp_rows, (size_t)ng)) || (rc = dalloc(&ic.grp_off, (size_t)ng))) return rc;
    CU(cudaMemsetAsync(ic.lane_seg, 0xff, n_slots * 4, st));
    CU(cudaMemsetAsync(ic.lane_rows, 0, n_slots * 4, st));
    CU(cudaMemsetAsync(ic.lane_win, 0, n_slots * 2, st));
    IlAssign as{};
    as.keys = keys2; as.segs = vals2; as.elem_first = d_elem_first; as.grp_first = d_grp_first;
    as.seg_words = seg_words; as.seg_t0 = so.seg_t0; as.seg_dt = so.seg_dt; as.seg_win = so.seg_win;
    as.lane_seg = ic.lane_seg; as.lane_rows = ic.lane_rows; as.lane_series = ic.lane_series; as.grp_col = ic.grp_col; as.lane_win = ic.lane_win; as.lane_t0 = ic.lane_t0; as.lane_dt = ic.lane_dt;
    as.n_elig = (uint32_t)n_elig; as.J = J; as.cols_per_super = ic.cols_per_super;
    k_il_assign<<<(unsigned)((n_elig + 255) / 256), 256, 0, st>>>(d, as);
    k_il_group_rows<<<(unsigned)((n_slots + 255) / 256), 256, 0, st>>>(ng, ic.lane_seg, seg_words, ic.grp_rows);
    CU(cudaGetLastError());
    std::vector<uint32_t> gw(ng); std::vector<uint64_t> go(ng);
    CU(cudaMemcpyAsync(gw.data(), ic.grp_rows, (size_t)ng * 4, cudaMemcpyDeviceToHost, st));
    CU(cudaStreamSynchronize(st));
    uint64_t total = 0;
    for (uint32_t g = 0; g < ng; g++) { go[g] = total; total += (uint64_t)gw[g] * 32; }
    size_t free_b = 0, total_b = 0;
    CU(dev_mem_info(&free_b, &total_b));
    size_t headroom = (size_t)8 << 30;
    if (const char *ov = getenv("OGPU_IL_HEADROOM_MB")) headroom = (size_t)atoll(ov) << 20;
    if (total * 4 + headroom > free_b || dev_malloc((void **)&ic.words, total * 4) != cudaSuccess) {
        cudaGetLastError(); ic.words = nullptr; ic.state = -2;
        return OG_OK;
    }
    CU(cudaMemcpyAsync(ic.grp_off, go.data(), (size_t)ng * 8, cudaMemcpyHostToDevice, st));
    k_il_repack<<<(unsigned)((n_slots + 127) / 128), 128, 0, st>>>(d, col, ic.lane_seg, ic.lane_win, ic.grp_off, ic.grp_rows, ng, ic.words);
    CU(cudaGetLastError());
    cudaEventRecord(ev1.e, st);
    CU(cudaStreamSynchronize(st));
    float ms = 0; cudaEventElapsedTime(&ms, ev0.e, ev1.e);
    ic.n_words = total; ic.n_packed = n_packed; ic.build_ms = ms; ic.state = 1;
    return OG_OK;
}

int build_plan(og_query *q) {
    og_shard *s = q->sh;
    const QueryP &p = q->qp;
    cudaStream_t st = q->stream;
    int rc;
    Plan *pl = new Plan;
    memset((void *)pl, 0, sizeof *pl);
    q->plan = pl;
    size_t cells_dense = (size_t)q->n_groups * p.n_buckets;
    for (uint32_t c = 0; c < p.n_calls; c++) {
        bool sel = p.calls[c].func >= OG_AGG_MIN && !(p.multi && p.calls[c].func <= OG_AGG_MAX);
        if ((rc = dalloc(&q->dense[c].val, cells_dense))) return rc;
        if ((rc = dalloc(&q->dense[c].ok, cells_dense))) return rc;
        if (sel && (rc = dalloc(&q->dense[c].tim, cells_dense))) return rc;
    }
    std::vector<uint32_t> grp_begin(q->n_groups + 1, 0), grp_series(s->n_series);
    if (q->desc.group_mode == OG_GROUP_MAP) {
        for (uint32_t sr = 0; sr < s->n_series; sr++) grp_begin[q->series_group[sr] + 1]++;
        for (uint32_t g = 0; g < q->n_groups; g++) grp_begin[g + 1] += grp_begin[g];
        std::vector<uint32_t> cur(grp_begin.begin(), grp_begin.end() - 1);
        for (uint32_t sr = 0; sr < s->n_series; sr++) grp_series[cur[q->series_group[sr]]++] = sr;
    } else if (q->desc.group_mode == OG_GROUP_PER_SERIES) {
        for (uint32_t g = 0; g <= q->n_groups; g++) grp_begin[g] = std::min(g, s->n_series);
        std::iota(grp_series.begin(), grp_series.end(), 0u);
    } else { grp_begin[1] = s->n_series; std::iota(grp_series.begin(), grp_series.end(), 0u); }
    uint32_t *d_grp_begin, *d_grp_series;
    if ((rc = salloc(q, &d_grp_begin, grp_begin.size()))) return rc;
    if ((rc = salloc(q, &d_grp_series, grp_series.size()))) return rc;
    if ((rc = salloc(q, &q->d_err, 16))) return rc;
    CU(cudaMemcpyAsync(d_grp_begin, grp_begin.data(), grp_begin.size() * 4, cudaMemcpyHostToDevice, st));
    CU(cudaMemcpyAsync(d_grp_series, grp_series.data(), grp_series.size() * 4, cudaMemcpyHostToDevice, st));
    CU(cudaStreamSynchronize(st));
    pl->gp.grp_begin = d_grp_begin; pl->gp.grp_series = d_grp_series; pl->gp.n_groups = q->n_groups;
    for (uint32_t c = 0; c < p.n_calls; c++) pl->gp.dense[c] = q->dense[c];

    bool has_string = false;
    for (uint32_t k = 0; k < p.n_cols; k++) has_string |= p.col_type[k] == OG_TYPE_STRING;
    pl->fused = p.n_cols == 1 && p.n_filter == 0 && !has_string && !(q->desc.flags & OG_Q_NO_FUSED);
    const bool multi_ok = !pl->fused && (has_string || !(q->desc.flags & OG_Q_NO_FUSED));
    pl->cols = false;
    if (multi_ok && !(q->desc.flags & OG_Q_NO_FAST) && s->irregular_time_pages == 0 && s->max_seg_rows <= OG_COLS_MAXROWS &&
        (p.n_filter == 0 || (p.n_filter == 1 && p.filter[0].kind == OG_F_TERM)) && !getenv("OGPU_NO_COLS")) {
        pl->cols = true;
        for (uint32_t k = 0; k < p.n_cols; k++) {
            int n = 0;
            for (uint32_t c = 0; c < p.n_calls; c++) n += p.calls[c].col_slot == (int)k;
            if (n > OG_COLS_MAXMINE) pl->cols = false;
        }
    }
    if (has_string && !pl->cols && p.n_cols > OG_MULTI_MAXC) { set_error("a query that counts a string column may touch at most %d columns on this shard", OG_MULTI_MAXC); return OG_E_UNSUPPORTED; }
    pl->multi = pl->cols || (multi_ok && p.n_cols <= OG_MULTI_MAXC);
    q->path_used = pl->fused ? 1 : pl->cols ? 5 : pl->multi ? 4 : 0;
    const bool want_fast = pl->fused && p.col_type[0] == OG_TYPE_FLOAT && !(q->desc.flags & OG_Q_NO_FAST) && s->n_segments;
    if (want_fast && (rc = ensure_il(s, p.col_index[0], st))) return rc;
    pl->fast = want_fast && s->il[p.col_index[0]].state == 1;
    const og_shard::IlCol *ic = pl->fast ? &s->il[p.col_index[0]] : nullptr;
    pl->ic = ic;
    pl->fold = pl->fast && ic->J != 0 && ic->aligned && q->desc.group_mode == OG_GROUP_ALL && !(q->desc.flags & OG_Q_STRICT_ORDER);

    size_t cell_bytes_per_series = 0;
    for (uint32_t c = 0; c < p.n_calls; c++) cell_bytes_per_series += (size_t)p.n_buckets * (9 + (p.calls[c].func >= OG_AGG_MIN ? 8 : 0));
    size_t free_b = 0, total_b = 0;
    CU(dev_mem_info(&free_b, &total_b));
    size_t budget = std::min<size_t>(free_b / 3, (size_t)24 << 30);
    q->chunk_series = (uint32_t)std::max<size_t>(1, std::min<size_t>(s->n_series, budget / std::max<size_t>(1, cell_bytes_per_series)));
    if (const char *ov = getenv("OGPU_CHUNK_SERIES")) {
        long v = atol(ov);
        if (v > 0) q->chunk_series = (uint32_t)std::min<long>(v, (long)std::max<uint32_t>(1, s->n_series));
    }
    if (q->chunk_series < s->n_series) {
        if (q->chunk_series >= OG_IL_SUPER) q->chunk_series = q->chunk_series / OG_IL_SUPER * OG_IL_SUPER;
        else q->chunk_series = std::max<uint32_t>(32, q->chunk_series & ~31u);
    }
    uint32_t max_chunk_segs = 0;
    for (uint32_t a = 0; a < s->n_series; a += q->chunk_series) {
        uint32_t b = std::min(s->n_series, a + q->chunk_series);
        max_chunk_segs = std::max(max_chunk_segs, s->h_series_seg_begin[b] - s->h_series_seg_begin[a]);
    }
    ChunkP &ch = pl->ch;
    ch.err = q->d_err; ch.flags = q->d_err + 2;
    ch.nb = p.n_buckets;
    ch.J = ic ? ic->J : 0;
    size_t chunk_cells = (size_t)std::min(q->chunk_series, s->n_series) * p.n_buckets;
    for (uint32_t c = 0; c < p.n_calls; c++) {
        bool sel = p.calls[c].func >= OG_AGG_MIN;
        if ((rc = salloc(q, &ch.cells[c].val, chunk_cells))) return rc;
        if ((rc = salloc(q, &ch.cells[c].ok, chunk_cells))) return rc;
        if (sel && (rc = salloc(q, &ch.cells[c].tim, chunk_cells))) return rc;
        if ((rc = salloc(q, &ch.edges[c].val, 2 * (size_t)max_chunk_segs))) return rc;
        if ((rc = salloc(q, &ch.edges[c].ok, 2 * (size_t)max_chunk_segs))) return rc;
        if (sel && (rc = salloc(q, &ch.edges[c].tim, 2 * (size_t)max_chunk_segs))) return rc;
    }
    if ((rc = salloc(q, &ch.edge_bucket, 2 * (size_t)max_chunk_segs))) return rc;
    pl->blockmerge = !pl->fold && q->desc.group_mode == OG_GROUP_ALL && !(q->desc.flags & OG_Q_STRICT_ORDER) &&
                     (s->n_series > 2 * OG_MERGE_SB || getenv("OGPU_FORCE_BLOCKMERGE") );
    if (pl->blockmerge) {
        ch.gc_edge0 = 0; ch.gc_col0 = 0;
        ch.gc_cols = (std::min(q->chunk_series, s->n_series) + OG_MERGE_SB - 1) / OG_MERGE_SB;
        const size_t n = (size_t)p.n_buckets * ch.gc_cols;
        for (uint32_t c = 0; c < p.n_calls; c++) {
            bool sel = p.calls[c].func >= OG_AGG_MIN;
            if ((rc = salloc(q, &ch.gcells[c].val, n))) return rc;
            if ((rc = salloc(q, &ch.gcells[c].ok, n))) return rc;
            if (sel && (rc = salloc(q, &ch.gcells[c].tim, n))) return rc;
        }
    }
    if (pl->fold) {
        ch.gc_tail0 = ic->n_super * ic->cols_per_super; ch.gc_edge0 = 2 * ch.gc_tail0; ch.gc_col0 = 0;
        ch.gc_cols = ch.gc_edge0 + 3 * ((s->n_series + 31) / 32);
        const size_t n = (size_t)p.n_buckets * ch.gc_cols;
        for (uint32_t c = 0; c < p.n_calls; c++) {
            bool sel = p.calls[c].func >= OG_AGG_MIN;
            if ((rc = salloc(q, &ch.gcells[c].val, n))) return rc;
            if ((rc = salloc(q, &ch.gcells[c].ok, n))) return rc;
            if (sel && (rc = salloc(q, &ch.gcells[c].tim, n))) return rc;
        }
    }
    if (pl->fast) {
        pl->il.words = ic->words; pl->il.grp_off = ic->grp_off; pl->il.grp_rows = ic->grp_rows; pl->il.grp_col = ic->grp_col;
        pl->il.lane_seg = ic->lane_seg; pl->il.lane_rows = ic->lane_rows; pl->il.lane_win = ic->lane_win; pl->il.lane_series = ic->lane_series; pl->il.lane_t0 = ic->lane_t0; pl->il.lane_dt = ic->lane_dt;
        pl->fm = 0; pl->times = false;
        for (uint32_t c = 0; c < p.n_calls; c++) {
            pl->fm |= 1 << (p.calls[c].func - 1);
            if (p.calls[c].func >= OG_AGG_MIN && !(p.multi && p.calls[c].func <= OG_AGG_MAX)) pl->times = true;
        }
        pl->fm |= FM_COUNT;
        q->path_used = pl->fold ? 3 : 2;
    }
    if (!pl->fused && !pl->multi) {
        TileP &tp = pl->tp;
        tp.R = std::max<uint32_t>(1, s->max_seg_rows);
        size_t per_seg = (size_t)tp.R * (p.n_cols * 9 + 8 + 1);
        size_t fb = 0, tb = 0;
        CU(dev_mem_info(&fb, &tb));
        const size_t tile_budget = std::max<size_t>((size_t)96 << 20, std::min<size_t>(fb / 4, (size_t)12 << 30));
        q->tile_segs = (uint32_t)std::max<size_t>(1, std::min<size_t>(std::max<uint32_t>(1, max_chunk_segs), tile_budget / per_seg));
        q->tile_segs = std::max<uint32_t>(32, q->tile_segs & ~31u);
        tp.S = q->tile_segs;
        for (uint32_t k = 0; k < p.n_cols; k++) {
            if ((rc = salloc(q, &tp.vals[k], (size_t)q->tile_segs * tp.R))) return rc;
            if ((rc = salloc(q, &tp.okb[k], (size_t)q->tile_segs * tp.R))) return rc;
        }
        if ((rc = salloc(q, &tp.times, (size_t)q->tile_segs * tp.R))) return rc;
        if ((rc = salloc(q, &tp.keep, (size_t)q->tile_segs * tp.R))) return rc;
    }
    q->planned = true;
    return OG_OK;
}
}
extern "C" {

OG_API int og_query_run(og_query *q) {
    if (!q) return OG_E_INVAL;
    og_shard *s = q->sh;
    CU(cudaSetDevice(s->device));
    const QueryP &p = q->qp;
    cudaStream_t st = q->stream;
    int rc;
    q->host_ready = false; q->next_group = 0; q->next_row = 0;
    if (!q->planned) {
        if (q->plan) { set_error("query plan failed earlier"); return OG_E_STATE; }
        if ((rc = build_plan(q))) return rc;
    }
    Plan *pl = (Plan *)q->plan;
    ChunkP ch = pl->ch; TileP tp = pl->tp; const GroupP &gp = pl->gp;
    size_t cells_dense = (size_t)q->n_groups * p.n_buckets;
    DirP dir = make_dir(s);
    uint32_t launches = 0, n_chunks = (s->n_series + q->chunk_series - 1) / q->chunk_series;
    while (q->main_ev.size() < 2 * (size_t)n_chunks) { cudaEvent_t e; CU(cudaEventCreate(&e)); q->main_ev.push_back(e); }
    CU(cudaMemsetAsync(q->d_err, 0, 64, st));
    CU(cudaEventRecord(q->ev0, st));
    const bool per_series = q->desc.group_mode == OG_GROUP_PER_SERIES;
    if (!per_series) { k_init_dense<<<(unsigned)((cells_dense + 255) / 256), 256, 0, st>>>(p, gp); launches++; }
    const bool clear_cells = !pl->fold || q->cells_dirty || n_chunks > 1;
    uint64_t segs_scanned = 0; uint32_t ci = 0, chunks_run = 0;
    for (uint32_t a = 0; a < s->n_series; a += q->chunk_series, ci++) {
        if (q->aborted) { cudaStreamSynchronize(st); set_error("query aborted"); return OG_E_ABORTED; }
        uint32_t b = std::min(s->n_series, a + q->chunk_series);
        ch.series_begin = a; ch.series_end = b;
        ch.seg_begin = s->h_series_seg_begin[a]; ch.seg_end = s->h_series_seg_begin[b];
        uint32_t nseg = ch.seg_end - ch.seg_begin;
        const size_t chunk_cells = (size_t)(b - a) * p.n_buckets;
        if (nseg == 0) {
            if (per_series) {
                for (uint32_t c = 0; c < p.n_calls; c++) CU(cudaMemsetAsync(ch.cells[c].ok, 0, chunk_cells, st));
                k_merge_per_series<<<dim3((unsigned)((chunk_cells + 255) / 256), p.n_calls), 256, 0, st>>>(p, ch, gp);
                launches++;
            }
            continue;
        }
        segs_scanned += nseg;
        if (clear_cells) for (uint32_t c = 0; c < p.n_calls; c++) CU(cudaMemsetAsync(ch.cells[c].ok, 0, chunk_cells, st));
        if (pl->fold || pl->blockmerge) for (uint32_t c = 0; c < p.n_calls; c++) CU(cudaMemsetAsync(ch.gcells[c].ok, 0, (size_t)p.n_buckets * ch.gc_cols, st));
        if (pl->fold && ci > 0) CU(cudaMemsetAsync(ch.flags + 1, 0, sizeof(int), st));
        CU(cudaEventRecord(q->main_ev[2 * chunks_run], st));
        if (pl->fused) {
            const uint32_t *gl = nullptr; uint32_t gn = nseg;
            if (pl->fast) {
                const og_shard::IlCol &ic = *pl->ic;
                uint32_t g0 = 0, g1 = ic.n_groups;
                if (ic.J) { g0 = ic.super_grp_first[a / OG_IL_SUPER]; g1 = ic.super_grp_first[std::min<uint32_t>(ic.n_super, (b + OG_IL_SUPER - 1) / OG_IL_SUPER)]; }
                launch_fast(pl->fm, pl->times, pl->fold, pl->il, g0, g1, p, ch, st); launches++;
                auto lo = std::lower_bound(ic.gen_host.begin(), ic.gen_host.end(), ch.seg_begin);
                auto hi = std::lower_bound(ic.gen_host.begin(), ic.gen_host.end(), ch.seg_end);
                gl = ic.gen_list + (lo - ic.gen_host.begin()); gn = (uint32_t)(hi - lo);
            }
            if (gn) {
                switch (p.n_calls) {
                case 1: launch_fused<1>(dir, p, ch, gl, gn, st); break;
                case 2: launch_fused<2>(dir, p, ch, gl, gn, st); break;
                case 3: launch_fused<3>(dir, p, ch, gl, gn, st); break;
                case 4: launch_fused<4>(dir, p, ch, gl, gn, st); break;
                case 5: launch_fused<5>(dir, p, ch, gl, gn, st); break;
                case 6: launch_fused<6>(dir, p, ch, gl, gn, st); break;
                case 7: launch_fused<7>(dir, p, ch, gl, gn, st); break;
                default: launch_fused<8>(dir, p, ch, gl, gn, st); break;
                }
                launches++;
            }
        } else if (pl->cols) {
            launch_cols(p, dir, ch, nseg, st);
        } else if (pl->multi) {
            launch_multi(p, dir, ch, nseg, st);
            launches++;
        } else {
            for (uint32_t t0 = ch.seg_begin; t0 < ch.seg_end; t0 += q->tile_segs) {
                tp.tile_begin = t0; tp.tile_end = std::min(ch.seg_end, t0 + q->tile_segs);
                uint32_t n = tp.tile_end - tp.tile_begin;
                dim3 g((n + 127) / 128, p.n_cols + 1);
                k_decode_tile<<<g, 128, 0, st>>>(dir, p, tp, q->d_err);
                size_t rows_total = (size_t)tp.S * tp.R;
                k_filter_tile<<<(unsigned)((rows_total + 255) / 256), 256, 0, st>>>(dir, p, tp);
                k_window_reduce<<<(n + 127) / 128, 128, 0, st>>>(dir, p, tp, ch);
                launches += 3;
            }
        }
        CU(cudaEventRecord(q->main_ev[2 * chunks_run + 1], st));
        chunks_run++;
        if (pl->fold) k_fix_edges_fold<<<(unsigned)(((size_t)((b - a + 31) / 32) * ch.J * 32 + 127) / 128), 128, 0, st>>>(dir, p, ch);
        else k_fix_edges<<<(nseg + 127) / 128, 128, 0, st>>>(dir, p, ch);
        if (per_series) k_merge_per_series<<<dim3((unsigned)((chunk_cells + 255) / 256), p.n_calls), 256, 0, st>>>(p, ch, gp);
        else if (pl->blockmerge) k_merge_all_blocks<<<dim3((p.n_buckets + 127) / 128, (b - a + OG_MERGE_SB - 1) / OG_MERGE_SB, p.n_calls), 128, 0, st>>>(p, ch, gp);
        else k_merge_groups<<<dim3((unsigned)((cells_dense + 127) / 128), p.n_calls), 128, 0, st>>>(p, ch, gp);
        launches += 2;
        if (pl->fold || pl->blockmerge) { k_merge_folded<<<dim3((unsigned)(((size_t)p.n_buckets * 32 + 127) / 128), p.n_calls), 128, 0, st>>>(p, ch, gp); launches++; }
    }
    CU(cudaEventRecord(q->ev1, st));
    CU(cudaGetLastError());
    CU(cudaStreamSynchronize(st));
    int err[16];
    CU(cudaMemcpy(err, q->d_err, 64, cudaMemcpyDeviceToHost));
    if (getenv("OGPU_IL_STATS")) {
        unsigned long long wait, life, pro, epi;
        memcpy(&wait, err + 8, 8); memcpy(&life, err + 10, 8); memcpy(&pro, err + 12, 8); memcpy(&epi, err + 14, 8);
        const double pc = life ? 100.0 / (double)life : 0.0;
        fprintf(stderr, "[ogpu] fused rounds: common %d rare %d (lanes not resident in %d, sit-outs %d); warp cycles: %llu waiting for batches of %llu (%.1f %%), "
                "prologue %llu (%.1f %%), epilogue %llu (%.1f %%)\n",
                err[4], err[5], err[6], err[7], wait, life, pc * (double)wait, pro, pc * (double)pro, epi, pc * (double)epi);
    }
    q->cells_dirty = err[2] != 0;
    if (err[0]) { set_error("segment %d failed to decode (device code %d)", err[1], err[0]); return map_dev_err(err[0]); }
    float ms = 0; cudaEventElapsedTime(&ms, q->ev0, q->ev1);
    double main_ms = 0;
    for (uint32_t i = 0; i < chunks_run; i++) { float m = 0; cudaEventElapsedTime(&m, q->main_ev[2 * i], q->main_ev[2 * i + 1]); main_ms += m; }
    og_stats &stt = q->stats;
    uint64_t keep_pb = stt.page_bytes, keep_rows = stt.rows_decoded, keep_segs = stt.segments_scanned;
    memset(&stt, 0, sizeof stt);
    stt.kernel_ms = ms; stt.main_kernel_ms = main_ms; stt.kernel_launches = launches; stt.path = q->path_used;
    stt.page_bytes = keep_pb; stt.rows_decoded = keep_pb ? keep_rows : s->n_rows; stt.segments_scanned = keep_pb ? keep_segs : segs_scanned;
    stt.dir_bytes = (uint64_t)segs_scanned * 32;
    stt.out_bytes = 0;
    for (uint32_t c = 0; c < p.n_calls; c++) stt.out_bytes += cells_dense * (9 + (q->dense[c].tim ? 8 : 0));
    if (p.n_cols == 1 && p.col_type[0] == OG_TYPE_FLOAT && p.col_index[0] < (int)s->il.size()) {
        const og_shard::IlCol &ic = s->il[p.col_index[0]];
        stt.il_state = ic.state; stt.il_build_ms = ic.build_ms; stt.il_bytes = ic.n_words * 4; stt.il_packed_segments = ic.state == 1 ? ic.n_packed : 0;
        stt.general_segments = ic.state == 1 ? (uint64_t)ic.gen_host.size() : s->n_segments;
    }
    stt.per_series_cells_used = err[2] != 0;
    q->ran = true;
    return OG_OK;
}

OG_API int og_query_dense(og_query *q, og_dense_view *out) {
    if (!q || !out) return OG_E_INVAL;
    if (!q->ran) { set_error("og_query_dense before og_query_run"); return OG_E_STATE; }
    const QueryP &p = q->qp;
    out->n_groups = q->n_groups; out->n_buckets = p.n_buckets; out->start = q->desc.interval ? p.start : 0; out->interval = q->desc.interval ? p.interval : 0;
    out->n_cols = p.n_calls;
    for (uint32_t c = 0; c < p.n_calls; c++) {
        q->dense_cols[c].values = q->dense[c].val; q->dense_cols[c].valid = q->dense[c].ok; q->dense_cols[c].times = q->dense[c].tim;
        q->dense_cols[c].type = p.calls[c].out_type; q->dense_cols[c].func = p.calls[c].func;
    }
    out->cols = q->dense_cols; out->stream = q->stream;
    return OG_OK;
}

}
namespace {
__global__ void k_sum_page_bytes(DirP d, QueryP q, int64_t tmin, int64_t tmax, unsigned long long *out ) {
    uint32_t seg = blockIdx.x * blockDim.x + threadIdx.x;
    if (seg >= d.n_segments) return;
    if (d.seg_tmax[seg] < tmin || d.seg_tmin[seg] > tmax) return;
    unsigned long long b = d.page_len[(size_t)d.n_columns * d.n_segments + seg];
    for (uint32_t k = 0; k < q.n_cols; k++) b += d.page_len[(size_t)q.col_index[k] * d.n_segments + seg];
    atomicAdd(&out[0], b); atomicAdd(&out[1], (unsigned long long)d.seg_rows[seg]); atomicAdd(&out[2], 1ull);
}
}
extern "C" {

OG_API int og_query_stats(const og_query *q, og_stats *out) {
    if (!q || !out) return OG_E_INVAL;
    og_query *mq = const_cast<og_query *>(q);
    if (q->ran && q->stats.page_bytes == 0) {
        CU(cudaSetDevice(q->sh->device));
        unsigned long long *d_o; int rc = dalloc(&d_o, 3); if (rc) return rc;
        cudaMemset(d_o, 0, 24);
        if (q->sh->n_segments) k_sum_page_bytes<<<(q->sh->n_segments + 255) / 256, 256>>>(make_dir(q->sh), q->qp, q->qp.tmin, q->qp.tmax, d_o);
        unsigned long long h[3]; CU(cudaMemcpy(h, d_o, 24, cudaMemcpyDeviceToHost)); dev_free(d_o);
        mq->stats.page_bytes = h[0]; mq->stats.rows_decoded = h[1]; mq->stats.segments_scanned = h[2];
    }
    *out = q->stats;
    return OG_OK;
}

OG_API int og_query_merge_dense(og_query *q, const og_dense_view *other) {
    if (!q || !other) return OG_E_INVAL;
    if (!q->ran) return OG_E_STATE;
    const QueryP &p = q->qp;
    if (other->n_groups != q->n_groups || other->n_buckets != p.n_buckets || other->n_cols != p.n_calls) { set_error("dense shapes differ"); return OG_E_INVAL; }
    if (other->start != (q->desc.interval ? p.start : 0) || other->interval != (q->desc.interval ? p.interval : 0)) {
        set_error("dense grids differ (start %lld vs %lld, interval %lld vs %lld): create the queries with OG_Q_QUERY_GRID", (long long)other->start,
                  (long long)(q->desc.interval ? p.start : 0), (long long)other->interval, (long long)(q->desc.interval ? p.interval : 0));
        return OG_E_INVAL;
    }
    CU(cudaSetDevice(q->sh->device));
    GroupP mine, oth; memset(&mine, 0, sizeof mine); memset(&oth, 0, sizeof oth);
    mine.n_groups = oth.n_groups = q->n_groups;
    for (uint32_t c = 0; c < p.n_calls; c++) {
        mine.dense[c] = q->dense[c];
        oth.dense[c].val = (uint64_t *)other->cols[c].values; oth.dense[c].ok = other->cols[c].valid; oth.dense[c].tim = other->cols[c].times;
        if ((q->dense[c].tim != nullptr) != (oth.dense[c].tim != nullptr)) { set_error("dense column %u: times presence differs", c); return OG_E_INVAL; }
    }
    size_t total = (size_t)q->n_groups * p.n_buckets;
    k_merge_dense<<<(unsigned)((total + 255) / 256), 256, 0, q->stream>>>(p, mine, oth);
    CU(cudaGetLastError());
    CU(cudaStreamSynchronize(q->stream));
    q->host_ready = false;
    return OG_OK;
}

OG_API int og_query_next(og_query *q, og_record_view *out) {
    if (!q || !out) return OG_E_INVAL;
    if (!q->ran) { set_error("og_query_next before og_query_run"); return OG_E_STATE; }
    if (q->aborted) return OG_E_ABORTED;
    const QueryP &p = q->qp;
    size_t total = (size_t)q->n_groups * p.n_buckets;
    if (!q->host_ready) {
        CU(cudaSetDevice(q->sh->device));
        for (uint32_t c = 0; c < p.n_calls; c++) {
            q->h_val[c].resize(total); q->h_ok[c].resize(total);
            CU(cudaMemcpy(q->h_val[c].data(), q->dense[c].val, total * 8, cudaMemcpyDeviceToHost));
            CU(cudaMemcpy(q->h_ok[c].data(), q->dense[c].ok, total, cudaMemcpyDeviceToHost));
            if (q->dense[c].tim) { q->h_tim[c].resize(total); CU(cudaMemcpy(q->h_tim[c].data(), q->dense[c].tim, total * 8, cudaMemcpyDeviceToHost)); }
        }
        q->host_ready = true; q->next_group = 0; q->next_row = 0;
    }
    int chunk = q->desc.chunk_size > 0 ? q->desc.chunk_size : 1024;
    uint32_t nc = p.n_calls;
    q->rv_val.assign(nc, {}); q->rv_bitmap.assign(nc, {}); q->rv_coltimes.assign(nc, {}); q->rv_times.clear(); q->rv_cols.assign(nc, og_colval_view{});
    while (q->next_group < q->n_groups) {
        uint32_t g = q->next_group;
        std::vector<int32_t> nil(nc, 0);
        int rows = 0;
        uint32_t b = q->next_row;
        uint32_t b_end = (uint32_t)std::min<uint64_t>(p.n_buckets, (uint64_t)b + (uint64_t)chunk);
        for (; b < b_end; b++) {
            const uint32_t bb = q->desc.ascending ? b : p.n_buckets - 1 - b;
            size_t i = (size_t)g * p.n_buckets + bb;
            bool any = false;
            for (uint32_t c = 0; c < nc; c++) any |= q->h_ok[c][i] != 0;
            if (!any) continue;
            int64_t row_time = p.start + (int64_t)bb * p.interval;
            if (q->desc.interval == 0) row_time = 0;
            for (uint32_t c = 0; c < nc; c++) {
                bool ok = q->h_ok[c][i] != 0;
                if ((size_t)(rows >> 3) >= q->rv_bitmap[c].size()) q->rv_bitmap[c].push_back(0);
                if (ok) {
                    q->rv_bitmap[c][rows >> 3] |= (uint8_t)(1 << (rows & 7));
                    if (p.calls[c].out_type == OG_TYPE_BOOL) q->rv_val[c].push_back((uint8_t)(q->h_val[c][i] != 0));
                    else { const uint8_t *pv = (const uint8_t *)&q->h_val[c][i]; q->rv_val[c].insert(q->rv_val[c].end(), pv, pv + 8); }
                } else nil[c]++;
                if (q->dense[c].tim) {
                    if (p.multi) q->rv_coltimes[c].push_back(ok ? q->h_tim[c][i] : 0);
                    else if (ok) row_time = q->h_tim[c][i];
                }
            }
            q->rv_times.push_back(row_time);
            rows++;
        }
        q->next_row = b_end;
        if (q->next_row >= p.n_buckets) { q->next_group++; q->next_row = 0; }
        if (rows == 0) continue;
        for (uint32_t c = 0; c < nc; c++) {
            og_colval_view &v = q->rv_cols[c];
            v.val = q->rv_val[c].data(); v.val_bytes = q->rv_val[c].size(); v.bitmap = q->rv_bitmap[c].data();
            v.times = (p.multi && q->dense[c].tim) ? q->rv_coltimes[c].data() : nullptr;
            v.type = p.calls[c].out_type; v.len = rows; v.nil_count = nil[c]; v.bitmap_offset = 0;
        }
        out->n_cols = nc; out->cols = q->rv_cols.data(); out->times = q->rv_times.data(); out->rows = rows; out->group = g;
        out->sid = q->desc.group_mode == OG_GROUP_PER_SERIES ? q->sh->sids[g] : 0;
        return OG_OK;
    }
    return OG_EOF;
}

}
namespace {
__global__ void k_decode_column(DirP d, uint32_t column, int type, uint32_t seg_begin, uint32_t seg_end, uint8_t *out, uint64_t stride,
                                uint32_t *rows_out, uint8_t *bitmap_out, uint32_t bitmap_stride, int *err) {
    uint32_t seg = seg_begin + blockIdx.x * blockDim.x + threadIdx.x;
    if (seg >= seg_end) return;
    uint8_t *o = out + (size_t)(seg - seg_begin) * stride;
    uint32_t rows = d.seg_rows[seg];
    size_t pi = (size_t)column * d.n_segments + seg;
    if (column == d.n_columns) {
        TimeDesc t;
        int rc = parse_time_page(d.data + d.page_off[pi], d.page_len[pi], t);
        if (rc == D_OK) {
            TimeIter it; it.init(t);
            for (uint32_t i = 0; i < t.rows; i++) ((int64_t *)o)[i] = it.next();
            it.finish(); rc = it.err;
        }
        if (rc != D_OK) report_err(err, rc, seg);
        if (rows_out) rows_out[seg - seg_begin] = rows;
        return;
    }
    uint32_t len = d.page_len[pi];
    uint8_t *bm = bitmap_out ? bitmap_out + (size_t)(seg - seg_begin) * bitmap_stride : nullptr;
    if (len == 0) {
        if (rows_out) rows_out[seg - seg_begin] = 0;
        if (bm) for (uint32_t i = 0; i < (rows + 7) / 8; i++) bm[i] = 0;
        return;
    }
    ColIter it;
    it.init(d.data + d.page_off[pi], len, type, rows);
    int rc = it.err;
    if (rc == D_OK && type == OG_TYPE_STRING) rc = D_UNSUPPORTED;
    if (rc == D_OK) {
        const PageHdr &h = it.h;
        for (uint32_t r = 0, j = 0; r < rows; r++) {
            uint64_t v;
            if (!it.next(v)) continue;
            if (type == OG_TYPE_BOOL) o[j++] = (uint8_t)v; else ((uint64_t *)o)[j++] = v;
        }
        it.finish(); rc = it.err;
        if (rows_out) rows_out[seg - seg_begin] = h.rows - h.nil_count;
        if (bm) {
            for (uint32_t i = 0; i < (rows + 7) / 8; i++) {
                uint8_t v = 0;
                for (uint32_t k = 0; k < 8 && i * 8 + k < rows; k++) v |= (uint8_t)(hdr_row_valid(h, i * 8 + k) ? 1 : 0) << k;
                bm[i] = v;
            }
        }
    }
    if (rc != D_OK) report_err(err, rc, seg);
}
}
extern "C" {

OG_API int og_decode_column_device(og_shard *s, uint32_t column, uint32_t seg_begin, uint32_t seg_end, void *d_values,
                                   uint64_t value_stride_bytes, uint32_t *d_rows_out) {
    if (!s || !d_values || column > s->n_columns || seg_begin > seg_end || seg_end > s->n_segments) { set_error("bad argument"); return OG_E_INVAL; }
    CU(cudaSetDevice(s->device));
    if (seg_begin == seg_end) return OG_OK;
    int *d_err; int rc = dalloc(&d_err, 2); if (rc) return rc;
    cudaMemset(d_err, 0, 8);
    int type = column == s->n_columns ? OG_TYPE_INT : s->col_types[column];
    uint32_t n = seg_end - seg_begin;
    k_decode_column<<<(n + 127) / 128, 128>>>(make_dir(s), column, type, seg_begin, seg_end, (uint8_t *)d_values, value_stride_bytes, d_rows_out, nullptr, 0, d_err);
    int err[2]; cudaError_t e = cudaMemcpy(err, d_err, 8, cudaMemcpyDeviceToHost); dev_free(d_err);
    if (e != cudaSuccess) return cuda_fail(e, "k_decode_column", __FILE__, __LINE__);
    if (err[0]) { set_error("segment %d failed to decode (device code %d)", err[1], err[0]); return map_dev_err(err[0]); }
    return OG_OK;
}

__global__ void k_reverse_segment(uint8_t *vals, uint32_t elem_bytes, uint32_t n_vals, uint8_t *bitmap, uint32_t rows) {
    for (uint32_t i = threadIdx.x; i < n_vals / 2; i += blockDim.x) {
        const uint32_t j = n_vals - 1 - i;
        if (elem_bytes == 8) { uint64_t *v = (uint64_t *)vals; const uint64_t a = v[i]; v[i] = v[j]; v[j] = a; }
        else { const uint8_t a = vals[i]; vals[i] = vals[j]; vals[j] = a; }
    }
    if (!bitmap) return;
    __syncthreads();
    __shared__ uint8_t sbm[8192];
    const uint32_t nb = (rows + 7) / 8;
    for (uint32_t i = threadIdx.x; i < nb; i += blockDim.x) sbm[i] = bitmap[i];
    __syncthreads();
    for (uint32_t i = threadIdx.x; i < nb; i += blockDim.x) {
        uint8_t o = 0;
        for (uint32_t k = 0; k < 8 && i * 8 + k < rows; k++) { const uint32_t src = rows - 1 - (i * 8 + k); o |= (uint8_t)((sbm[src >> 3] >> (src & 7)) & 1) << k; }
        bitmap[i] = o;
    }
}
}
static int decode_segment_impl(og_shard *s, uint32_t segment, uint32_t flags, og_record_view *out);
extern "C" {
OG_API int og_decode_segment(og_shard *s, uint32_t segment, og_record_view *out) { return decode_segment_impl(s, segment, 0, out); }
OG_API int og_decode_segment_ex(og_shard *s, uint32_t segment, uint32_t flags, og_record_view *out) { return decode_segment_impl(s, segment, flags, out); }
}
static int decode_segment_impl(og_shard *s, uint32_t segment, uint32_t flags, og_record_view *out) {
    if (!s || !out || segment >= s->n_segments) { set_error("bad argument"); return OG_E_INVAL; }
    CU(cudaSetDevice(s->device));
    uint32_t R = std::max<uint32_t>(1, s->max_seg_rows);
    size_t ncol1 = (size_t)s->n_columns + 1;
    size_t val_stride = (size_t)R * 8, bm_stride = (((size_t)R + 7) / 8 + 7) & ~(size_t)7;
    size_t need = ncol1 * (val_stride + bm_stride + 16);
    if (s->d_seg_buf_bytes < need) {
        if (s->d_seg_buf) dev_free(s->d_seg_buf);
        if (s->h_seg_buf) cudaFreeHost(s->h_seg_buf);
        CU(dev_malloc((void **)&s->d_seg_buf, need)); CU(cudaMallocHost(&s->h_seg_buf, need));
        s->d_seg_buf_bytes = s->h_seg_buf_bytes = need;
    }
    uint8_t *dv = (uint8_t *)s->d_seg_buf, *dbm = dv + ncol1 * val_stride;
    uint32_t *drows = (uint32_t *)(dbm + ncol1 * bm_stride);
    int *d_err; int rc = dalloc(&d_err, 2); if (rc) return rc;
    cudaMemset(d_err, 0, 8);
    DirP dir = make_dir(s);
    for (uint32_t c = 0; c <= s->n_columns; c++) {
        int type = c == s->n_columns ? OG_TYPE_INT : s->col_types[c];
        k_decode_column<<<1, 32>>>(dir, c, type, segment, segment + 1, dv + c * val_stride, val_stride, drows + c, dbm + c * bm_stride, (uint32_t)bm_stride, d_err);
    }
    int err[2]; cudaError_t e = cudaMemcpy(err, d_err, 8, cudaMemcpyDeviceToHost); dev_free(d_err);
    if (e != cudaSuccess) return cuda_fail(e, "k_decode_column", __FILE__, __LINE__);
    if (err[0]) { set_error("segment %d failed to decode (device code %d)", err[1], err[0]); return map_dev_err(err[0]); }
    if (flags & OG_DECODE_DESCENDING) {
        if (R > 65536) { set_error("descending materialisation supports segments of up to 65536 rows"); return OG_E_UNSUPPORTED; }
        uint32_t hr[65];
        CU(cudaMemcpy(hr, drows, (ncol1) * 4, cudaMemcpyDeviceToHost));
        const uint32_t rows_seg = hr[s->n_columns];
        for (uint32_t c = 0; c <= s->n_columns; c++) {
            const bool is_time = c == s->n_columns;
            const uint32_t eb = (!is_time && s->col_types[c] == OG_TYPE_BOOL) ? 1 : 8;
            k_reverse_segment<<<1, 256>>>(dv + c * val_stride, eb, is_time ? rows_seg : hr[c], is_time ? nullptr : dbm + c * bm_stride, rows_seg);
        }
        CU(cudaGetLastError());
    }
    CU(cudaMemcpy(s->h_seg_buf, s->d_seg_buf, need, cudaMemcpyDeviceToHost));
    uint8_t *hv = (uint8_t *)s->h_seg_buf, *hbm = hv + ncol1 * val_stride;
    uint32_t *hrows = (uint32_t *)(hbm + ncol1 * bm_stride);
    uint32_t rows = hrows[s->n_columns];
    s->seg_views.assign(s->n_columns, og_colval_view{});
    for (uint32_t c = 0; c < s->n_columns; c++) {
        og_colval_view &v = s->seg_views[c];
        uint32_t nv = hrows[c];
        v.val = hv + c * val_stride; v.val_bytes = (uint64_t)nv * (s->col_types[c] == OG_TYPE_BOOL ? 1 : 8);
        v.bitmap = hbm + c * bm_stride; v.times = nullptr; v.type = s->col_types[c]; v.len = (int32_t)rows; v.nil_count = (int32_t)(rows - nv); v.bitmap_offset = 0;
    }
    out->n_cols = s->n_columns; out->cols = s->seg_views.data(); out->times = (const int64_t *)(hv + s->n_columns * val_stride); out->rows = (int32_t)rows; out->group = 0;
    uint32_t sr = (uint32_t)(std::upper_bound(s->h_series_seg_begin.begin(), s->h_series_seg_begin.end(), segment) - s->h_series_seg_begin.begin()) - 1;
    out->sid = s->sids[sr];
    return OG_OK;
}
```

### opengemini_b200/csrc/fused_il.cuh

```cuda
#pragma once
#include "agg_kernels.cuh"

namespace ogpu {

__device__ __forceinline__ uint32_t smem_u32(const void *p) { return (uint32_t)__cvta_generic_to_shared(p); }
__device__ __forceinline__ uint32_t opaque(uint32_t x) { asm volatile("mov.u32 %0, %0;" : "+r"(x)); return x; }
template <int OFF> __device__ __forceinline__ uint32_t lds32o(uint32_t a) { uint32_t v; asm volatile("ld.shared.u32 %0, [%1+%2];" : "=r"(v) : "r"(a), "n"(OFF)); return v; }
__device__ __forceinline__ void mbar_init(uint32_t bar, uint32_t count) { asm volatile("mbarrier.init.shared::cta.b64 [%0], %1;" ::"r"(bar), "r"(count) : "memory"); }
__device__ __forceinline__ void mbar_init_fence() { asm volatile("fence.mbarrier_init.release.cluster;\nfence.proxy.async.shared::cta;" ::: "memory"); }
__device__ __forceinline__ void mbar_expect_tx(uint32_t bar, uint32_t bytes) { asm volatile("mbarrier.arrive.expect_tx.shared::cta.b64 _, [%0], %1;" ::"r"(bar), "r"(bytes) : "memory"); }
__device__ __forceinline__ void bulk_g2s(uint32_t dst, const void *src, uint32_t bytes, uint32_t bar) {
    asm volatile("cp.async.bulk.shared::cluster.global.mbarrier::complete_tx::bytes [%0], [%1], %2, [%3];" ::"r"(dst), "l"(src), "r"(bytes), "r"(bar) : "memory");
}
__device__ __forceinline__ bool mbar_wait(uint32_t bar, uint32_t parity) {
#pragma unroll 1
    for (uint32_t i = 0; i < (1u << 16); i++) {
        uint32_t ok;
        asm volatile("{\n.reg .pred p;\nmbarrier.try_wait.parity.shared::cta.b64 p, [%1], %2;\nselp.u32 %0, 1, 0, p;\n}" : "=r"(ok) : "r"(bar), "r"(parity) : "memory");
        if (ok) return true;
    }
    return false;
}

enum { FM_COUNT = 1, FM_SUM = 2, FM_MIN = 4, FM_MAX = 8, FM_FIRST = 16, FM_LAST = 32 };
enum { SEG_GENERAL = 0, SEG_FAST = 1, SEG_PACKED = 2 };

#ifndef OG_FAST_THREADS
#define OG_FAST_THREADS 128
#endif
#ifndef OG_FAST_MAXREG
#define OG_FAST_MAXREG 80
#endif
#ifndef OG_IL_NW
#define OG_IL_NW 64u
#endif
#ifndef OG_IL_B
#define OG_IL_B 16u
#endif
#ifndef OG_IL_K
#define OG_IL_K 10u
#endif
#ifndef OG_IL_UNROLL
#define OG_IL_UNROLL 2
#endif
#define OG_IL_NB (OG_IL_NW / OG_IL_B)
#define OG_IL_ROWS (OG_IL_NW + 2u)
#define OG_IL_PAD_WORDS 6u
#define OG_IL_HDR 7u
#define OG_IL_RAW_HDR 6u
#define OG_IL_NONE 0xffffffffu
#define OG_IL_PACKED 0x8000u
#define OG_IL_LOOKBITS (77u * OG_IL_K + 29u + 13u + 64u + 64u)
static_assert(OG_IL_K >= 2, "packed lanes: K*64 + 63 + 128 <= OG_IL_LOOKBITS needs K >= 2");
static_assert(OG_IL_NW % OG_IL_B == 0 && (OG_IL_NW & (OG_IL_NW - 1)) == 0, "ring geometry");
static_assert(OG_IL_NW - OG_IL_B > (OG_IL_LOOKBITS + 31u) / 32u + 2u, "ring too small for the round length: the slowest lane could not proceed");

struct IlP {
    const uint32_t *words;
    const uint64_t *grp_off;
    const uint32_t *grp_rows;
    const uint32_t *grp_col;
    const uint32_t *lane_seg;
    const uint32_t *lane_rows;
    const uint16_t *lane_win;
    const uint32_t *lane_series;
    const int64_t *lane_t0;
    const uint64_t *lane_dt;
};

__device__ __forceinline__ uint64_t udiv_est(uint64_t a, uint64_t b, double inv_b) {
    const double qd = __ull2double_rn(a) * inv_b;
    if ((a >> 63) || !(qd < 1125899906842624.0)) return a / b;
    uint64_t q = (uint64_t)qd;
    uint64_t r = a - q * b;
    if ((int64_t)r < 0) { do { q--; r += b; } while ((int64_t)r < 0); }
    else while (r >= b) { q++; r -= b; }
    return q;
}

__device__ __forceinline__ uint64_t fetch64(uint32_t col, uint32_t p) {
    uint32_t a = col + ((p << 2) & ((OG_IL_NW - 1) << 7));
    uint32_t a0 = lds32o<0>(a), a1 = lds32o<128>(a), a2 = lds32o<256>(a);
    uint32_t hi = __funnelshift_l(a1, a0, p), lo = __funnelshift_l(a2, a1, p);
    return ((uint64_t)hi << 32) | lo;
}

__device__ __forceinline__ Part fold32(int func, int type, bool multi, Part p, bool with_time) {
    constexpr uint32_t FULL = 0xffffffffu;
    if (func == OG_AGG_COUNT) { p.v = __reduce_add_sync(FULL, p.ok ? (uint32_t)p.v : 0u); p.ok = p.v != 0; return p; }
    if (type == OG_TYPE_FLOAT && func == OG_AGG_SUM) {
        double s = p.ok ? u2d(p.v) : 0.0;
#pragma unroll
        for (int o = 16; o; o >>= 1) s += __shfl_xor_sync(FULL, s, o);
        p.ok = __any_sync(FULL, p.ok != 0); p.v = d2u(s); return p;
    }
    if (type == OG_TYPE_FLOAT && !with_time && (func == OG_AGG_MIN || func == OG_AGG_MAX)) {
        double v = u2d(p.v); uint32_t ok = p.ok;
#pragma unroll
        for (int o = 16; o; o >>= 1) {
            const double ov = __shfl_xor_sync(FULL, v, o); const uint32_t ook = __shfl_xor_sync(FULL, ok, o);
            const bool keep = ok && (func == OG_AGG_MIN ? v <= ov : v >= ov);
            if (ook && !keep) v = ov;
            ok |= ook;
        }
        p.v = d2u(v); p.ok = ok; return p;
    }
    return warp_fold(func, type, multi, p, with_time);
}

#define OG_IL_WCAP 24u
__host__ __device__ inline uint32_t il_acc_bytes(uint32_t n_calls, bool times) { return OG_IL_WCAP * n_calls * (times ? 17u : 9u) + 8u & ~7u; }

template <int FM, bool TIMES, bool FOLD>
__global__ void __maxnreg__(OG_FAST_MAXREG) k_fused_il(QueryP q, ChunkP ch, IlP il, uint32_t grp_begin, uint32_t grp_end) {
    constexpr uint32_t NW = OG_IL_NW, B = OG_IL_B, NB = OG_IL_NB, K = OG_IL_K;
    constexpr uint32_t FULL = 0xffffffffu;
    constexpr uint32_t WPB = OG_FAST_THREADS / 32;
    constexpr int UNR = OG_IL_UNROLL;
    __shared__ __align__(128) uint32_t s_win[WPB * OG_IL_ROWS * 32];
    __shared__ __align__(8) uint64_t s_bar[WPB * NB];
    extern __shared__ __align__(8) uint8_t s_acc[];

#ifdef OG_IL_STATS
    const long long st_clk0 = clock64();
    long long st_wait = 0;
#endif
    const uint32_t lane = threadIdx.x & 31;
    const uint32_t wid = __reduce_max_sync(FULL, threadIdx.x >> 5);
    const uint32_t grp = grp_begin + blockIdx.x * WPB + wid;
    if (grp >= grp_end) return;
    const uint32_t rows_w = __reduce_max_sync(FULL, il.grp_rows[grp]);
    if (rows_w == 0) return;
    const size_t slot = (size_t)grp * 32 + lane;
    const uint32_t seg = il.lane_seg[slot];
    bool active = seg != OG_IL_NONE && seg >= ch.seg_begin && seg < ch.seg_end;
    if (!__any_sync(FULL, active)) return;
    const size_t e = 2 * (size_t)(seg - ch.seg_begin);

    uint32_t rows = 0, series = 0, r_lo = 0, r_hi = 0, lwin = 0;
    int64_t t0 = 0, dt = 1; uint64_t dtu = 1; double inv_dt = 1.0;
    const double inv_iv = 1.0 / __ull2double_rn((uint64_t)q.interval);
    if (active) {
        rows = il.lane_rows[slot]; lwin = il.lane_win[slot]; series = il.lane_series[slot];
        t0 = il.lane_t0[slot]; dtu = il.lane_dt[slot]; dt = (int64_t)dtu;
        inv_dt = 1.0 / __ull2double_rn(dtu);
        r_lo = 0; r_hi = rows - 1;
        if (t0 < q.tmin) { uint64_t k = udiv_est((uint64_t)(q.tmin - t0) + dtu - 1, dtu, inv_dt); r_lo = k > rows ? rows : (uint32_t)k; }
        { int64_t t_last = t0 + (int64_t)(rows - 1) * dt; if (t_last > q.tmax) { if (q.tmax < t0) r_lo = rows; else r_hi = (uint32_t)udiv_est((uint64_t)(q.tmax - t0), dtu, inv_dt); } }
        const uint64_t span = (uint64_t)q.n_buckets * (uint64_t)q.interval;
        const bool outside = r_lo <= r_hi && r_lo < rows &&
                             ((uint64_t)(t0 + (int64_t)r_lo * dt - q.start) >= span || (uint64_t)(t0 + (int64_t)r_hi * dt - q.start) >= span);
        if (outside) report_err(ch.err, D_CORRUPT, seg);
        if (r_lo > r_hi || r_lo >= rows || outside) { *(uint2 *)(ch.edge_bucket + e) = make_uint2(OG_NO_BUCKET, OG_NO_BUCKET); active = false; }
    }
    if (!__any_sync(FULL, active)) return;

    const uint32_t win = smem_u32(s_win) + wid * (OG_IL_ROWS * 128);
    const uint32_t col = opaque(win + lane * 4);
    const uint32_t bar0 = smem_u32(s_bar) + wid * (NB * 8);
    if (lane == 0) {
#pragma unroll
        for (uint32_t i = 0; i < NB; i++) mbar_init(bar0 + i * 8, 1);
        mbar_init_fence();
    }
    __syncwarp();
    const uint32_t total_b = rows_w / B;
    uint64_t goff = il.grp_off[grp];
    goff = ((uint64_t)__reduce_max_sync(FULL, (uint32_t)(goff >> 32)) << 32) | __reduce_max_sync(FULL, (uint32_t)goff);
    const uint32_t *gsrc = il.words + goff;
    uint32_t issued_b = 0, ready_b = 0;
    uint32_t hung = 0;
    uint64_t pol;
    asm("createpolicy.fractional.L2::evict_first.b64 %0, 1.0;" : "=l"(pol));
    auto issue = [&](uint32_t k_any) {
        const uint32_t k = __reduce_max_sync(FULL, k_any);
        const uint32_t s = k % NB, dst = win + s * (B * 128), bar = bar0 + s * 8;
        const uint32_t *src = gsrc + (size_t)k * (B * 32);
        if (s == 0)
            asm volatile("{\n.reg .pred p;\nelect.sync _|p, 0xffffffff;\n@p mbarrier.arrive.expect_tx.shared::cta.b64 _, [%0], %1;\n"
                         "@p cp.async.bulk.shared::cluster.global.mbarrier::complete_tx::bytes.L2::cache_hint [%2], [%3], %4, [%0], %6;\n"
                         "@p cp.async.bulk.shared::cluster.global.mbarrier::complete_tx::bytes.L2::cache_hint [%5], [%3], 256, [%0], %6;\n}"
                         ::"r"(bar), "r"(B * 128 + 256u), "r"(dst), "l"(src), "r"(B * 128), "r"(win + NW * 128), "l"(pol) : "memory");
        else
            asm volatile("{\n.reg .pred p;\nelect.sync _|p, 0xffffffff;\n@p mbarrier.arrive.expect_tx.shared::cta.b64 _, [%0], %1;\n"
                         "@p cp.async.bulk.shared::cluster.global.mbarrier::complete_tx::bytes.L2::cache_hint [%2], [%3], %1, [%0], %4;\n}"
                         ::"r"(bar), "r"(B * 128), "r"(dst), "l"(src), "l"(pol) : "memory");
    };
    {
        const uint32_t first = total_b < NB ? total_b : NB;
        for (uint32_t k = 0; k < first; k++) issue(k);
        issued_b = first;
    }

    uint32_t cur_b = 0, rb = 0xffffffffu, step_q = 0; uint64_t rem = 0, step_r = 0;
    if (active) {
        const int64_t t_lo = t0 + (int64_t)r_lo * dt;
        cur_b = (uint32_t)udiv_est((uint64_t)(t_lo - q.start), (uint64_t)q.interval, inv_iv);
        const uint64_t ivl = (uint64_t)q.interval;
        const uint64_t sq64 = udiv_est(ivl, dtu, inv_dt);
        step_q = sq64 > 0xffffffffull ? 0xffffffffu : (uint32_t)sq64;
        step_r = ivl - sq64 * dtu;
        uint64_t D = (uint64_t)(q.start + (int64_t)(cur_b + 1) * q.interval - t0) + dtu - 1;
        uint64_t qq = udiv_est(D, dtu, inv_dt); rem = D - qq * dtu; rb = qq > 0xffffffffull ? 0xffffffffu : (uint32_t)qq;
    }

    bool uni = false; uint32_t b0 = 0, b_end = 0;
    uint64_t *acc_v = nullptr; int64_t *acc_t = nullptr; uint8_t *acc_k = nullptr;
    if (FOLD) {
        const int leader = __ffs(__ballot_sync(FULL, active)) - 1;
        const int64_t t0L = __shfl_sync(FULL, t0, leader); const uint64_t dtL = __shfl_sync(FULL, dtu, leader);
        const uint32_t loL = __shfl_sync(FULL, r_lo, leader), hiL = __shfl_sync(FULL, r_hi, leader);
        b0 = __shfl_sync(FULL, cur_b, leader);
        const bool same = t0 == t0L && dtu == dtL && r_lo == loL && r_hi == hiL;
        const uint32_t b_last = active ? (uint32_t)udiv_est((uint64_t)(t0 + (int64_t)r_hi * dt - q.start), (uint64_t)q.interval, inv_iv) : b0;
        uni = __all_sync(FULL, !active || (same && b_last - b0 < OG_IL_WCAP));
        if (uni) {
            b_end = __reduce_max_sync(FULL, active ? b_last : 0u);
            const uint32_t nacc = OG_IL_WCAP * q.n_calls;
            uint8_t *base = s_acc + (size_t)wid * il_acc_bytes(q.n_calls, TIMES);
            acc_v = (uint64_t *)base; acc_t = (int64_t *)(base + (size_t)nacc * 8); acc_k = base + (size_t)nacc * (TIMES ? 16 : 8);
            for (uint32_t i = lane; i < nacc; i += 32) acc_k[i] = 0;
            __syncwarp();
        }
    }
    const uint32_t gcol = FOLD ? il.grp_col[grp] - ch.gc_col0 : 0;
    const bool fold_edges = FOLD && uni && b_end > b0;

    double sum = 0.0, mn = 0.0, mx = 0.0; uint64_t fi = 0, lastv = 0;
    uint32_t n_mn = 0, n_mx = 0;
    uint32_t w_row0 = r_lo;
    bool head_done = false; uint32_t head_b = OG_NO_BUCKET;
    uint32_t stop = 0, n_ev = 0;
    auto part_of = [&](int func, uint32_t cnt) -> Part {
        Part pp; pp.ok = cnt != 0; pp.v = 0; pp.t = 0;
        switch (func) {
        case OG_AGG_COUNT: pp.v = cnt; break;
        case OG_AGG_SUM: if (FM & FM_SUM) pp.v = d2u(sum); break;
        case OG_AGG_MIN: if (FM & FM_MIN) { pp.v = d2u(mn); if (TIMES) pp.t = t0 + (int64_t)(stop - n_mn) * dt; } break;
        case OG_AGG_MAX: if (FM & FM_MAX) { pp.v = d2u(mx); if (TIMES) pp.t = t0 + (int64_t)(stop - n_mx) * dt; } break;
        case OG_AGG_FIRST: if (FM & FM_FIRST) { pp.v = fi; pp.t = t0 + (int64_t)w_row0 * dt; } break;
        default: if (FM & FM_LAST) { pp.v = lastv; pp.t = t0 + (int64_t)(stop - 1) * dt; } break;
        }
        return pp;
    };
    auto kind_of = [&]() -> int { return !head_done ? 0 : stop > r_hi ? 1 : 2; };
    auto flush_lane = [&](int kind) {
        const uint32_t cnt = stop - w_row0;
#pragma unroll 1
        for (uint32_t c = 0; c < q.n_calls; c++) {
            const Part pp = part_of(q.calls[c].func, cnt);
            if (kind == 2) { if (pp.ok) store_cell(ch, (int)c, series, cur_b, pp); }
            else store_part(ch.edges[c], e + kind, pp);
        }
        if (kind == 0) { head_done = true; head_b = cur_b; }
    };
    auto flush_fold = [&](bool ev) {
        uint32_t pend = __ballot_sync(FULL, ev);
#pragma unroll 1
        while (pend) {
            const int leader = __ffs(pend) - 1;
            const uint32_t bL = __shfl_sync(FULL, cur_b, leader);
            const bool mine = ev && cur_b == bL;
            const uint32_t cnt = mine ? stop - w_row0 : 0;
            const uint32_t w = bL - b0;
#pragma unroll 1
            for (uint32_t c = 0; c < q.n_calls; c++) {
                const int func = q.calls[c].func, ftype = func == OG_AGG_COUNT ? OG_TYPE_INT : q.calls[c].type;
                const bool wt = func >= OG_AGG_MIN && !(q.multi && func <= OG_AGG_MAX);
                Part pp = fold32(func, ftype, q.multi != 0, part_of(func, cnt), wt);
                if ((int)lane == leader && pp.ok) {
                    const uint32_t i = c * OG_IL_WCAP + w;
                    Part a; a.ok = acc_k[i]; a.v = a.ok ? acc_v[i] : 0; a.t = (TIMES && a.ok) ? acc_t[i] : 0;
                    group_update(func, ftype, q.multi != 0, a, pp);
                    acc_v[i] = a.v; acc_k[i] = 1; if (TIMES) acc_t[i] = a.t;
                }
            }
            pend &= ~__ballot_sync(FULL, mine);
        }
        __syncwarp();
    };

    uint32_t qp = 0, sr = 0, kfast = 0, CM = 0, CE = 0, m = 64, tr = 0, bad = 0; uint64_t MASK = 0;
    bool done = !active;
    uint64_t val = 0;

#ifdef OG_IL_STATS
    long long st_w0 = clock64();
#endif
    if (issued_b && !mbar_wait(bar0, 0)) hung = 1; else ready_b = issued_b ? 1 : 0;
#ifdef OG_IL_STATS
    st_wait += clock64() - st_w0;
#endif
    if (active && !hung) {
        val = fetch64(col, 0); qp = 64;
        if (lwin & OG_IL_PACKED) {
            const uint32_t lead = (lwin >> 8) & 63u, mw = lwin & 127u;
            qp = 64 - lead; kfast = mw;
            MASK = mw ? (~0ull >> (64 - mw)) << (64 - lead - mw) : 0ull;
        } else { CM = 0; CE = 1; }
    }

    bool skipping = r_lo > 0;
    stop = skipping ? r_lo : (rb < r_hi + 1 ? rb : r_hi + 1);
    n_ev = stop;
    if (!skipping) { fi = val; mn = mx = u2d(val); n_mn = n_mx = n_ev; }
    if (done) n_ev = 0xffffffffu;

    auto retire = [&]() { done = true; n_ev = 0xffffffffu; CM = 0; CE = 0; MASK = 0; kfast = 0; };
    auto advance = [&]() {
        bool fin = false;
        if (skipping) { skipping = false; sum = 0.0; }
        else {
            fin = stop > r_hi;
            sum = 0.0;
            if (!fin) while (stop >= rb) {
                cur_b++;
                rem += step_r; uint32_t adv = step_q;
                if (rem >= dtu) { rem -= dtu; adv++; }
                rb = (rb > 0xffffffffu - adv) ? 0xffffffffu : rb + adv;
            }
        }
        if (fin) retire();
        else {
            w_row0 = stop;
            uint32_t nstop = rb < r_hi + 1 ? rb : r_hi + 1;
            n_ev = nstop - stop; stop = nstop;
            fi = val; mn = mx = u2d(val); n_mn = n_mx = n_ev;
        }
    };
    auto slow_record = [&]() {
        uint32_t p = qp + sr;
        const uint64_t x = fetch64(col, p);
        const uint32_t ctrl = (uint32_t)(x >> 62);
        if (ctrl < 2) { qp += 1; return; }
        if (ctrl == 3) {
            const uint32_t lm = (uint32_t)(x >> 51) & 0x7ff;
            uint32_t lead = lm >> 6; m = lm & 0x3f;
            if (m == 0) { m = 64; tr = 0; lead = 0; }
            else { if (lead + m > 64) { if (!done) bad = 1; lead = 0; m = 64; } tr = 64 - lead - m; }
            p += 13;
            const bool slowwin = lead < 2;
            sr = slowwin ? 0 : lead - 2;
            CM = slowwin ? 0u : 3u << (30 - sr); CE = slowwin ? 1u : 2u << (30 - sr);
            kfast = 2 + m;
            MASK = (m == 64 ? ~0ull : ((1ull << m) - 1)) << tr;
        } else p += 2;
        const uint64_t y = fetch64(col, p);
        const uint64_t sig = m == 64 ? y : (y >> (64 - m));
        p += m;
        val ^= sig << tr;
        qp = p - sr;
    };
    auto accumulate = [&](uint32_t k_in_run) {
        if (FM & FM_SUM) sum = sum + u2d(val);
        if (FM & FM_MIN) { if (mn > u2d(val)) { mn = u2d(val); if (TIMES) n_mn = n_ev - k_in_run; } }
        if (FM & FM_MAX) { if (mx < u2d(val)) { mx = u2d(val); if (TIMES) n_mx = n_ev - k_in_run; } }
        if (FM & FM_LAST) lastv = val;
    };
    auto record = [&](uint32_t k_in_run) {
        accumulate(k_in_run);
        const uint64_t x = fetch64(col, qp);
        const bool slow = (((uint32_t)(x >> 32) & CM) ^ CE) != 0;
        if (slow) slow_record();
        else { val ^= x & MASK; qp += kfast; }
    };
    auto record2 = [&](uint32_t k_in_run) {
        const uint64_t x0 = fetch64(col, qp), x1 = fetch64(col, qp + kfast);
        accumulate(k_in_run);
#ifdef OG_IL_REC2B
        uint64_t x1b = x1;
        if ((((uint32_t)(x0 >> 32) & CM) ^ CE) != 0) { slow_record(); x1b = fetch64(col, qp); }
        else { val ^= x0 & MASK; qp += kfast; }
        accumulate(k_in_run + 1);
        if ((((uint32_t)(x1b >> 32) & CM) ^ CE) != 0) slow_record();
        else { val ^= x1b & MASK; qp += kfast; }
#else
        if ((((uint32_t)(x0 >> 32) & CM) ^ CE) != 0) { slow_record(); record(k_in_run + 1); return; }
        val ^= x0 & MASK; qp += kfast;
        accumulate(k_in_run + 1);
        if ((((uint32_t)(x1 >> 32) & CM) ^ CE) != 0) slow_record();
        else { val ^= x1 & MASK; qp += kfast; }
#endif
    };

    uint32_t rounds_left = hung ? 0u : 40u * (__reduce_max_sync(FULL, rows) / K + 8u);
#ifdef OG_IL_STATS
    uint32_t st_common = 0, st_rare = 0, st_sit = 0, st_notgo = 0;
    const long long st_pro = clock64() - st_clk0;
#endif
    for (;;) {
        const uint32_t qmin = __reduce_min_sync(FULL, done ? 0xffffffffu : qp);
        if (qmin == 0xffffffffu) break;
        const uint32_t f = qmin < 32 ? 0u : (qmin - 32) >> 5;
#pragma unroll 1
        while (issued_b < total_b && (issued_b + 1) * B <= f + NW) { issue(issued_b); issued_b++; }
        const uint32_t qmax = __reduce_max_sync(FULL, done ? 0u : qp);
        uint32_t need_max = ((qmax + OG_IL_LOOKBITS) >> 5) + 1; if (need_max > rows_w) need_max = rows_w;
        uint32_t want_b = (need_max + B - 1) / B; if (want_b > issued_b) want_b = issued_b;
#ifdef OG_IL_STATS
        st_w0 = clock64();
#endif
#pragma unroll 1
        while (ready_b < want_b) { if (!mbar_wait(bar0 + (ready_b % NB) * 8, (ready_b / NB) & 1)) { hung = 1; break; } ready_b++; }
#ifdef OG_IL_STATS
        st_wait += clock64() - st_w0;
#endif
        if (hung) break;
        uint32_t need = ((qp + OG_IL_LOOKBITS) >> 5) + 1; if (need > rows_w) need = rows_w;
        bool go = done || need <= ready_b * B;
        uint32_t run = __reduce_min_sync(FULL, go ? n_ev : 0u);
        if (run >= K) {
            static_assert(K % 2 == 0, "records are decoded in pairs");
#pragma unroll UNR
            for (uint32_t k = 0; k < K; k += 2) record2(k);
            n_ev -= K;
#ifdef OG_IL_STATS
            st_common++;
#endif
            continue;
        }
#ifdef OG_IL_STATS
        st_rare++;
#endif
        if (rounds_left-- == 0) { hung = 2; break; }
        const bool all_go = __all_sync(FULL, go);
#ifdef OG_IL_STATS
        if (!all_go) { st_notgo++; st_sit += __popc(__ballot_sync(FULL, !go)); }
#endif
        uint32_t left = K;
        for (;;) {
            run = __reduce_min_sync(FULL, go ? n_ev : 0xffffffffu);
            if (run > left) run = left;
            if (all_go) {
#pragma unroll 1
                for (uint32_t k = 0; k < run; k++) record(k);
            } else {
#pragma unroll 1
                for (uint32_t k = 0; k < run; k++) if (go) record(k);
            }
            if (go) n_ev -= run;
            left -= run;
            if (left == 0) break;
            const bool ev = go && !done && n_ev == 0;
            if (FOLD && uni) {
                const bool fl = ev && !skipping;
                const int kind = kind_of();
                const bool to_acc = fl && (kind == 2 || fold_edges);
                if (fl && !to_acc) flush_lane(kind);
                if (__any_sync(FULL, to_acc)) flush_fold(to_acc);
                if (to_acc && kind == 0) head_done = true;
            } else if (ev && !skipping) flush_lane(kind_of());
            if (ev) advance();
            if (__all_sync(FULL, ev || done)) break;
        }
    }
    if (active && (qp >> 5) >= rows_w) bad = 1;
#ifdef OG_IL_STATS
    const long long st_e0 = clock64();
    if (lane == 0) { atomicAdd((unsigned *)&ch.err[4], st_common); atomicAdd((unsigned *)&ch.err[5], st_rare); atomicAdd((unsigned *)&ch.err[6], st_notgo); atomicAdd((unsigned *)&ch.err[7], st_sit); }
#endif
    while (ready_b < issued_b && hung != 1) { if (!mbar_wait(bar0 + (ready_b % NB) * 8, (ready_b / NB) & 1)) hung = 1; ready_b++; }
    if (hung && lane == 0) report_err(ch.err, D_WATCHDOG, (grp << 2) | hung);
    if (FOLD && uni) {
        __syncwarp();
        const uint32_t w_tail = fold_edges ? b_end - b0 : OG_IL_WCAP;
        for (uint32_t i = lane; i < OG_IL_WCAP * q.n_calls; i += 32) {
            if (!acc_k[i]) continue;
            const uint32_t c = i / OG_IL_WCAP, w = i % OG_IL_WCAP;
            Part a; a.ok = 1; a.v = acc_v[i]; a.t = TIMES ? acc_t[i] : 0;
            store_part(ch.gcells[c], (size_t)(b0 + w) * ch.gc_cols + (w == w_tail ? ch.gc_tail0 + gcol : gcol), a);
        }
    }
    if (FOLD && __any_sync(FULL, active && head_b != OG_NO_BUCKET) && lane == 0) ch.flags[1] = 1;
    if (active) {
        if (bad) report_err(ch.err, D_CORRUPT, seg);
        *(uint2 *)(ch.edge_bucket + e) = make_uint2(head_b, (head_b == OG_NO_BUCKET || cur_b == head_b) ? OG_NO_BUCKET : cur_b);
    }
#ifdef OG_IL_STATS
    if (lane == 0) {
        atomicAdd((unsigned long long *)(ch.err + 8), (unsigned long long)st_wait);
        const long long st_end = clock64();
        atomicAdd((unsigned long long *)(ch.err + 10), (unsigned long long)(st_end - st_clk0));
        atomicAdd((unsigned long long *)(ch.err + 12), (unsigned long long)st_pro);
        atomicAdd((unsigned long long *)(ch.err + 14), (unsigned long long)(st_end - st_e0));
    }
#endif
}

}
```

### opengemini_b200/csrc/internal.h

```cpp
#pragma once
#include <cuda_runtime.h>

#include <cstdint>
#include <string>
#include <mutex>
#include <vector>

#include "../../include/ogpu.h"

#define OG_MAX_CALLS 8
#define OG_MAX_FILTER 16
#define OG_MAX_COLS 8

namespace ogpu {

void set_error(const char *fmt, ...);
int cuda_fail(cudaError_t e, const char *what, const char *file, int line);
int ensure_device();

inline cudaError_t dev_malloc(void **p, size_t bytes) { return cudaMallocAsync(p, bytes ? bytes : 1, (cudaStream_t)0); }
inline void dev_free(void *p) { if (p) cudaFreeAsync(p, (cudaStream_t)0); }
cudaError_t dev_mem_info(size_t *free_b, size_t *total_b);
#define CU(call) do { cudaError_t e__ = (call); if (e__ != cudaSuccess) return ::ogpu::cuda_fail(e__, #call, __FILE__, __LINE__); } while (0)

struct DevBuf {
    void *p = nullptr; size_t bytes = 0;
};

}

struct og_shard {
    int device = 0;
    uint8_t *d_data = nullptr; uint64_t data_len = 0; bool owns_data = true;
    uint32_t n_series = 0, n_segments = 0, n_columns = 0;
    uint32_t max_seg_rows = 0;
    uint64_t irregular_time_pages = 0;
    uint64_t n_rows = 0, page_bytes = 0;
    uint64_t snappy_pages = 0, snappy_bytes_in = 0, snappy_bytes_out = 0;
    og_merge_info merge{1, 0, 0, 0, 0, 0, 0, 0, 0, 0};
    int64_t tmin = 0, tmax = 0;
    std::vector<uint64_t> sids;
    std::vector<int32_t> col_types;
    std::vector<std::string> col_names;
    std::vector<uint32_t> h_series_seg_begin;
    uint32_t *d_series_seg_begin = nullptr;
    uint32_t *d_seg_series = nullptr;
    uint32_t *d_seg_rows = nullptr;
    int64_t *d_tmin = nullptr, *d_tmax = nullptr;
    uint64_t *d_page_off = nullptr;
    uint32_t *d_page_len = nullptr;
    uint64_t *d_sids = nullptr;
    void *h_seg_buf = nullptr; size_t h_seg_buf_bytes = 0;
    void *d_seg_buf = nullptr; size_t d_seg_buf_bytes = 0;
    std::vector<og_colval_view> seg_views;
    struct IlCol { int state = 0;
                   uint32_t *words = nullptr; uint64_t *grp_off = nullptr; uint32_t *grp_rows = nullptr, *grp_col = nullptr;
                   uint32_t *lane_seg = nullptr, *lane_rows = nullptr, *lane_series = nullptr; uint16_t *lane_win = nullptr; int64_t *lane_t0 = nullptr; uint64_t *lane_dt = nullptr;
                   uint32_t *gen_list = nullptr; std::vector<uint32_t> gen_host;
                   uint32_t n_groups = 0, J = 0;
                   bool aligned = false;
                   uint32_t n_super = 1, cols_per_super = 0; std::vector<uint32_t> super_grp_first;
                   uint64_t n_words = 0, n_packed = 0;  double build_ms = 0; };
    std::vector<IlCol> il;
    std::mutex il_mu;
};

namespace ogpu {

struct CallP { int32_t func, col_slot, type, out_type; };
struct FilterP { int32_t kind, col_slot, op, type, const_is_float; double fval; int64_t ival; };

struct Tri { uint64_t *val; int64_t *tim; uint8_t *ok; };

struct QueryP {
    int64_t tmin, tmax, start, interval;
    uint32_t n_buckets, n_calls, n_filter, n_cols;
    int32_t multi;
    CallP calls[OG_MAX_CALLS];
    FilterP filter[OG_MAX_FILTER];
    int32_t col_index[OG_MAX_COLS];
    int32_t col_type[OG_MAX_COLS];
};

}

struct og_query {
    og_shard *sh = nullptr;
    og_query_desc desc{};
    std::vector<og_call> calls;
    std::vector<og_filter_item> filter;
    std::vector<uint32_t> series_group;
    cudaStream_t stream = nullptr;
    cudaEvent_t ev0 = nullptr, ev1 = nullptr;
    ogpu::QueryP qp{};
    uint32_t n_groups = 0;
    bool ran = false; volatile int aborted = 0;
    ogpu::Tri dense[OG_MAX_CALLS]{};
    og_dense_col dense_cols[OG_MAX_CALLS]{};
    uint32_t *d_group_of_series = nullptr;
    std::vector<void *> scratch;
    og_stats stats{};
    std::vector<uint64_t> h_val[OG_MAX_CALLS];
    std::vector<uint8_t> h_ok[OG_MAX_CALLS];
    std::vector<int64_t> h_tim[OG_MAX_CALLS];
    bool host_ready = false;
    uint32_t next_group = 0, next_row = 0;
    std::vector<std::vector<uint8_t>> rv_val, rv_bitmap;
    std::vector<std::vector<int64_t>> rv_coltimes;
    std::vector<int64_t> rv_times;
    std::vector<og_colval_view> rv_cols;
    int path_used = 0;
    bool cells_dirty = true;
    bool planned = false;
    uint32_t chunk_series = 0, tile_segs = 0;
    int *d_err = nullptr;
    void *plan = nullptr;
    std::vector<cudaEvent_t> main_ev;
    void *merge_state = nullptr;
};
```

Before: 487.8 billion.

## Add warp-uniform packed decode loop and self-clearing folded cell merge

Adds a specialised path in the fused interleaved kernel for warps whose lanes all share the same packed window and row count. It decodes record pairs with shared masks in a simpler loop and trims the bulk copies to the bytes actually needed. k_merge_folded now unrolls its loads, clears the ok flags as it consumes them, and skips edge columns when no edges were produced. This replaces the per-chunk memset of gcells with a single one applied only when the cells are dirty. k_fix_edges_fold becomes grid-stride with a capped grid, and a uniform-group counter is added to the stats.

```diff
diff --git a/include/ogpu.h b/include/ogpu.h
--- a/include/ogpu.h
+++ b/include/ogpu.h
@@ -156,6 +156,7 @@
     uint64_t general_segments;
     double merge_ms;
     uint64_t il_packed_segments;
+    uint64_t il_uniform_groups;
 } og_stats;
 
 typedef struct og_shard og_shard;
diff --git a/opengemini_b200/_lib.py b/opengemini_b200/_lib.py
--- a/opengemini_b200/_lib.py
+++ b/opengemini_b200/_lib.py
@@ -73,7 +73,7 @@
                 ("dir_bytes", C.c_uint64), ("out_bytes", C.c_uint64), ("kernel_ms", C.c_double), ("h2d_ms", C.c_double), ("main_kernel_ms", C.c_double),
                 ("kernel_launches", C.c_uint32), ("path", C.c_int32), ("il_state", C.c_int32), ("per_series_cells_used", C.c_int32),
                 ("il_build_ms", C.c_double), ("il_bytes", C.c_uint64), ("general_segments", C.c_uint64), ("merge_ms", C.c_double),
-                ("il_packed_segments", C.c_uint64)]
+                ("il_packed_segments", C.c_uint64), ("il_uniform_groups", C.c_uint64)]
 
 
 class SynthColumn(C.Structure):
diff --git a/opengemini_b200/csrc/agg_kernels.cuh b/opengemini_b200/csrc/agg_kernels.cuh
--- a/opengemini_b200/csrc/agg_kernels.cuh
+++ b/opengemini_b200/csrc/agg_kernels.cuh
@@ -6,6 +6,8 @@
 namespace ogpu {
 
 #define OG_NO_BUCKET 0xFFFFFFFFu
+#define OG_ERR_UNIFORM 16
+#define OG_ERR_INTS 18
 
 struct DirP {
     const uint8_t *data;
@@ -338,33 +340,35 @@
 
 __global__ void k_fix_edges_fold(DirP d, QueryP q, ChunkP ch) {
     if (ch.flags[1] == 0) return;
-    const uint32_t w = (blockIdx.x * blockDim.x + threadIdx.x) >> 5, lane = threadIdx.x & 31;
+    const uint32_t lane = threadIdx.x & 31;
     const uint32_t n_blk = (ch.series_end - ch.series_begin + 31) / 32;
-    if (w >= n_blk * ch.J) return;
-    const uint32_t blk = w / ch.J, j = w % ch.J;
-    const uint32_t series = ch.series_begin + blk * 32 + lane;
-    const bool in = series < ch.series_end;
-    const uint32_t seg = in ? d.series_seg_begin[series] + j : 0;
-    EdgeRuns r; r.hb = r.tb = OG_NO_BUCKET; r.head_leader = false; r.s_end = 0;
-    if (in) r = edge_runs(d, ch, seg, series);
-    const uint32_t n_bk = (ch.gc_cols - ch.gc_edge0) / 3;
-    for (int which = 0; which < 2; which++) {
-        const uint32_t gcol = ch.gc_edge0 + (which ? 2u : (j & 1u)) * n_bk + ch.series_begin / 32 + blk - ch.gc_col0;
-        const bool has = r.hb != OG_NO_BUCKET && (which == 0 ? r.head_leader : r.tb != OG_NO_BUCKET);
-        const uint32_t b = which == 0 ? r.hb : r.tb;
-        const uint32_t hm = __ballot_sync(0xffffffffu, has);
-        if (hm == 0) continue;
-        const int leader = __ffs(hm) - 1;
-        const uint32_t bL = __shfl_sync(0xffffffffu, b, leader);
-        const bool unif = __all_sync(0xffffffffu, !has || b == bL) && bL < q.n_buckets;
-        if (!unif && has && b >= q.n_buckets) { report_err(ch.err, D_CORRUPT, seg); continue; }
-        for (uint32_t c = 0; c < q.n_calls; c++) {
-            Part acc = part_empty();
-            if (has) acc = edge_stitch(q, ch, r, seg, which, c);
-            if (unif) {
-                acc = warp_fold(q.calls[c].func, call_ftype(q, c), q.multi != 0, acc, call_has_time(q, c));
-                if ((int)lane == leader && acc.ok) store_part(ch.gcells[c], (size_t)bL * ch.gc_cols + gcol, acc);
-            } else if (has && acc.ok) store_cell(ch, (int)c, series, b, acc);
+    const uint32_t n_w = n_blk * ch.J, stride = (gridDim.x * blockDim.x) >> 5;
+    for (uint32_t w = (blockIdx.x * blockDim.x + threadIdx.x) >> 5; w < n_w; w += stride) {
+        const uint32_t blk = w / ch.J, j = w % ch.J;
+        const uint32_t series = ch.series_begin + blk * 32 + lane;
+        const bool in = series < ch.series_end;
+        const uint32_t seg = in ? d.series_seg_begin[series] + j : 0;
+        EdgeRuns r; r.hb = r.tb = OG_NO_BUCKET; r.head_leader = false; r.s_end = 0;
+        if (in) r = edge_runs(d, ch, seg, series);
+        const uint32_t n_bk = (ch.gc_cols - ch.gc_edge0) / 3;
+        for (int which = 0; which < 2; which++) {
+            const uint32_t gcol = ch.gc_edge0 + (which ? 2u : (j & 1u)) * n_bk + ch.series_begin / 32 + blk - ch.gc_col0;
+            const bool has = r.hb != OG_NO_BUCKET && (which == 0 ? r.head_leader : r.tb != OG_NO_BUCKET);
+            const uint32_t b = which == 0 ? r.hb : r.tb;
+            const uint32_t hm = __ballot_sync(0xffffffffu, has);
+            if (hm == 0) continue;
+            const int leader = __ffs(hm) - 1;
+            const uint32_t bL = __shfl_sync(0xffffffffu, b, leader);
+            const bool unif = __all_sync(0xffffffffu, !has || b == bL) && bL < q.n_buckets;
+            if (!unif && has && b >= q.n_buckets) { report_err(ch.err, D_CORRUPT, seg); continue; }
+            for (uint32_t c = 0; c < q.n_calls; c++) {
+                Part acc = part_empty();
+                if (has) acc = edge_stitch(q, ch, r, seg, which, c);
+                if (unif) {
+                    acc = warp_fold(q.calls[c].func, call_ftype(q, c), q.multi != 0, acc, call_has_time(q, c));
+                    if ((int)lane == leader && acc.ok) store_part(ch.gcells[c], (size_t)bL * ch.gc_cols + gcol, acc);
+                } else if (has && acc.ok) store_cell(ch, (int)c, series, b, acc);
+            }
         }
     }
 }
@@ -464,7 +468,7 @@
     if (acc.ok) store_part(ch.gcells[c], (size_t)b * ch.gc_cols + blk, acc);
 }
 
-__global__ void k_merge_folded(QueryP q, ChunkP ch, GroupP gp) {
+__global__ void k_merge_folded(QueryP q, ChunkP ch, GroupP gp, bool edge_cols) {
     const uint32_t b = (blockIdx.x * blockDim.x + threadIdx.x) >> 5, lane = threadIdx.x & 31, c = blockIdx.y;
     if (b >= q.n_buckets) return;
     const int func = q.calls[c].func, ftype = call_ftype(q, c);
@@ -472,10 +476,24 @@
     const Tri g = ch.gcells[c];
     Part acc = part_empty();
     const size_t row = (size_t)b * ch.gc_cols;
-    for (uint32_t col = lane; col < ch.gc_cols; col += 32) {
-        if (!g.ok[row + col]) continue;
-        Part p; p.ok = 1; p.v = g.val[row + col]; p.t = wt ? g.tim[row + col] : 0;
-        group_update(func, ftype, multi, acc, p);
+    const uint32_t n_cols = edge_cols && ch.flags[1] == 0 ? ch.gc_edge0 : ch.gc_cols;
+    constexpr uint32_t U = 8;
+    for (uint32_t c0 = lane; c0 < n_cols; c0 += 32 * U) {
+        uint8_t okv[U]; uint64_t vv[U]; int64_t tt[U];
+#pragma unroll
+        for (uint32_t u = 0; u < U; u++) { const uint32_t col = c0 + 32 * u; okv[u] = col < n_cols ? g.ok[row + col] : 0; }
+#pragma unroll
+        for (uint32_t u = 0; u < U; u++) {
+            const size_t i = row + c0 + 32 * u;
+            vv[u] = okv[u] ? g.val[i] : 0; tt[u] = (okv[u] && wt) ? g.tim[i] : 0;
+        }
+#pragma unroll
+        for (uint32_t u = 0; u < U; u++) {
+            if (!okv[u]) continue;
+            g.ok[row + c0 + 32 * u] = 0;
+            Part p; p.ok = 1; p.v = vv[u]; p.t = tt[u];
+            group_update(func, ftype, multi, acc, p);
+        }
     }
     acc = warp_fold(func, ftype, multi, acc, wt);
     if (lane == 0 && acc.ok) {
diff --git a/opengemini_b200/csrc/api.cu b/opengemini_b200/csrc/api.cu
--- a/opengemini_b200/csrc/api.cu
+++ b/opengemini_b200/csrc/api.cu
@@ -450,30 +450,32 @@
 template <int NC> void launch_fused(const DirP &d, const QueryP &p, const ChunkP &ch, const uint32_t *list, uint32_t n, cudaStream_t st) {
     if (n) k_fused_segment<NC><<<(n + 127) / 128, 128, 0, st>>>(d, p, ch, list, n);
 }
-template <int FM, bool TIMES> void launch_fast_t(bool fold, const IlP &il, uint32_t g0, uint32_t g1, const QueryP &p, const ChunkP &ch, cudaStream_t st) {
+template <int FM, bool TIMES> void launch_fast_t(bool fold, bool uni, const IlP &il, uint32_t g0, uint32_t g1, const QueryP &p, const ChunkP &ch, cudaStream_t st) {
     constexpr uint32_t WPB = OG_FAST_THREADS / 32;
     dim3 grid((g1 - g0 + WPB - 1) / WPB), block(OG_FAST_THREADS);
+    if constexpr (!(FM == 63 && TIMES))
+        if (fold && uni) { k_fused_il<FM, TIMES, true, true><<<grid, block, WPB * il_acc_bytes(p.n_calls, TIMES), st>>>(p, ch, il, g0, g1); return; }
     if (fold) k_fused_il<FM, TIMES, true><<<grid, block, WPB * il_acc_bytes(p.n_calls, TIMES), st>>>(p, ch, il, g0, g1);
     else k_fused_il<FM, TIMES, false><<<grid, block, 0, st>>>(p, ch, il, g0, g1);
 }
-void launch_fast(int fm, bool times, bool fold, const IlP &il, uint32_t g0, uint32_t g1, const QueryP &p, const ChunkP &ch, cudaStream_t st) {
+void launch_fast(int fm, bool times, bool fold, bool uni, const IlP &il, uint32_t g0, uint32_t g1, const QueryP &p, const ChunkP &ch, cudaStream_t st) {
     if (g1 <= g0) return;
     if (!times) {
         switch (fm) {
-        case FM_SUM | FM_COUNT: return launch_fast_t<FM_SUM | FM_COUNT, false>(fold, il, g0, g1, p, ch, st);
-        case FM_SUM | FM_COUNT | FM_MAX: return launch_fast_t<FM_SUM | FM_COUNT | FM_MAX, false>(fold, il, g0, g1, p, ch, st);
-        case FM_SUM | FM_COUNT | FM_MIN | FM_MAX: return launch_fast_t<FM_SUM | FM_COUNT | FM_MIN | FM_MAX, false>(fold, il, g0, g1, p, ch, st);
-        case FM_COUNT: return launch_fast_t<FM_COUNT, false>(fold, il, g0, g1, p, ch, st);
+        case FM_SUM | FM_COUNT: return launch_fast_t<FM_SUM | FM_COUNT, false>(fold, uni, il, g0, g1, p, ch, st);
+        case FM_SUM | FM_COUNT | FM_MAX: return launch_fast_t<FM_SUM | FM_COUNT | FM_MAX, false>(fold, uni, il, g0, g1, p, ch, st);
+        case FM_SUM | FM_COUNT | FM_MIN | FM_MAX: return launch_fast_t<FM_SUM | FM_COUNT | FM_MIN | FM_MAX, false>(fold, uni, il, g0, g1, p, ch, st);
+        case FM_COUNT: return launch_fast_t<FM_COUNT, false>(fold, uni, il, g0, g1, p, ch, st);
         default: break;
         }
     } else {
         switch (fm) {
-        case FM_MAX | FM_COUNT: return launch_fast_t<FM_MAX | FM_COUNT, true>(fold, il, g0, g1, p, ch, st);
-        case FM_MIN | FM_COUNT: return launch_fast_t<FM_MIN | FM_COUNT, true>(fold, il, g0, g1, p, ch, st);
+        case FM_MAX | FM_COUNT: return launch_fast_t<FM_MAX | FM_COUNT, true>(fold, uni, il, g0, g1, p, ch, st);
+        case FM_MIN | FM_COUNT: return launch_fast_t<FM_MIN | FM_COUNT, true>(fold, uni, il, g0, g1, p, ch, st);
         default: break;
         }
     }
-    return launch_fast_t<63, true>(fold, il, g0, g1, p, ch, st);
+    return launch_fast_t<63, true>(fold, uni, il, g0, g1, p, ch, st);
 }
 
 template <int NCOL, int NCALL> void launch_multi_t(const QueryP &p, const DirP &d, const ChunkP &ch, uint32_t nseg, cudaStream_t st) {
@@ -616,7 +618,7 @@
     cudaEventRecord(ev1.e, st);
     CU(cudaStreamSynchronize(st));
     float ms = 0; cudaEventElapsedTime(&ms, ev0.e, ev1.e);
-    ic.n_words = total; ic.n_packed = n_packed; ic.build_ms = ms; ic.state = 1;
+    ic.n_words = total; ic.n_packed = n_packed; ic.all_packed = n_packed == n_elig; ic.build_ms = ms; ic.state = 1;
     return OG_OK;
 }
 
@@ -648,7 +650,7 @@
     uint32_t *d_grp_begin, *d_grp_series;
     if ((rc = salloc(q, &d_grp_begin, grp_begin.size()))) return rc;
     if ((rc = salloc(q, &d_grp_series, grp_series.size()))) return rc;
-    if ((rc = salloc(q, &q->d_err, 16))) return rc;
+    if ((rc = salloc(q, &q->d_err, OG_ERR_INTS))) return rc;
     CU(cudaMemcpyAsync(d_grp_begin, grp_begin.data(), grp_begin.size() * 4, cudaMemcpyHostToDevice, st));
     CU(cudaMemcpyAsync(d_grp_series, grp_series.data(), grp_series.size() * 4, cudaMemcpyHostToDevice, st));
     CU(cudaStreamSynchronize(st));
@@ -789,11 +791,13 @@
     DirP dir = make_dir(s);
     uint32_t launches = 0, n_chunks = (s->n_series + q->chunk_series - 1) / q->chunk_series;
     while (q->main_ev.size() < 2 * (size_t)n_chunks) { cudaEvent_t e; CU(cudaEventCreate(&e)); q->main_ev.push_back(e); }
-    CU(cudaMemsetAsync(q->d_err, 0, 64, st));
+    CU(cudaMemsetAsync(q->d_err, 0, OG_ERR_INTS * sizeof(int), st));
     CU(cudaEventRecord(q->ev0, st));
     const bool per_series = q->desc.group_mode == OG_GROUP_PER_SERIES;
     if (!per_series) { k_init_dense<<<(unsigned)((cells_dense + 255) / 256), 256, 0, st>>>(p, gp); launches++; }
     const bool clear_cells = !pl->fold || q->cells_dirty || n_chunks > 1;
+    if (pl->fold && q->gcells_dirty) for (uint32_t c = 0; c < p.n_calls; c++) CU(cudaMemsetAsync(ch.gcells[c].ok, 0, (size_t)p.n_buckets * ch.gc_cols, st));
+    q->gcells_dirty = true;
     uint64_t segs_scanned = 0; uint32_t ci = 0, chunks_run = 0;
     for (uint32_t a = 0; a < s->n_series; a += q->chunk_series, ci++) {
         if (q->aborted) { cudaStreamSynchronize(st); set_error("query aborted"); return OG_E_ABORTED; }
@@ -812,7 +816,7 @@
         }
         segs_scanned += nseg;
         if (clear_cells) for (uint32_t c = 0; c < p.n_calls; c++) CU(cudaMemsetAsync(ch.cells[c].ok, 0, chunk_cells, st));
-        if (pl->fold || pl->blockmerge) for (uint32_t c = 0; c < p.n_calls; c++) CU(cudaMemsetAsync(ch.gcells[c].ok, 0, (size_t)p.n_buckets * ch.gc_cols, st));
+        if (pl->blockmerge) for (uint32_t c = 0; c < p.n_calls; c++) CU(cudaMemsetAsync(ch.gcells[c].ok, 0, (size_t)p.n_buckets * ch.gc_cols, st));
         if (pl->fold && ci > 0) CU(cudaMemsetAsync(ch.flags + 1, 0, sizeof(int), st));
         CU(cudaEventRecord(q->main_ev[2 * chunks_run], st));
         if (pl->fused) {
@@ -821,7 +825,7 @@
                 const og_shard::IlCol &ic = *pl->ic;
                 uint32_t g0 = 0, g1 = ic.n_groups;
                 if (ic.J) { g0 = ic.super_grp_first[a / OG_IL_SUPER]; g1 = ic.super_grp_first[std::min<uint32_t>(ic.n_super, (b + OG_IL_SUPER - 1) / OG_IL_SUPER)]; }
-                launch_fast(pl->fm, pl->times, pl->fold, pl->il, g0, g1, p, ch, st); launches++;
+                launch_fast(pl->fm, pl->times, pl->fold, ic.all_packed, pl->il, g0, g1, p, ch, st); launches++;
                 auto lo = std::lower_bound(ic.gen_host.begin(), ic.gen_host.end(), ch.seg_begin);
                 auto hi = std::lower_bound(ic.gen_host.begin(), ic.gen_host.end(), ch.seg_end);
                 gl = ic.gen_list + (lo - ic.gen_host.begin()); gn = (uint32_t)(hi - lo);
@@ -858,19 +862,19 @@
         }
         CU(cudaEventRecord(q->main_ev[2 * chunks_run + 1], st));
         chunks_run++;
-        if (pl->fold) k_fix_edges_fold<<<(unsigned)(((size_t)((b - a + 31) / 32) * ch.J * 32 + 127) / 128), 128, 0, st>>>(dir, p, ch);
+        if (pl->fold) k_fix_edges_fold<<<(unsigned)std::min<size_t>(((size_t)((b - a + 31) / 32) * ch.J * 32 + 127) / 128, 2048), 128, 0, st>>>(dir, p, ch);
         else k_fix_edges<<<(nseg + 127) / 128, 128, 0, st>>>(dir, p, ch);
         if (per_series) k_merge_per_series<<<dim3((unsigned)((chunk_cells + 255) / 256), p.n_calls), 256, 0, st>>>(p, ch, gp);
         else if (pl->blockmerge) k_merge_all_blocks<<<dim3((p.n_buckets + 127) / 128, (b - a + OG_MERGE_SB - 1) / OG_MERGE_SB, p.n_calls), 128, 0, st>>>(p, ch, gp);
         else k_merge_groups<<<dim3((unsigned)((cells_dense + 127) / 128), p.n_calls), 128, 0, st>>>(p, ch, gp);
         launches += 2;
-        if (pl->fold || pl->blockmerge) { k_merge_folded<<<dim3((unsigned)(((size_t)p.n_buckets * 32 + 127) / 128), p.n_calls), 128, 0, st>>>(p, ch, gp); launches++; }
+        if (pl->fold || pl->blockmerge) { k_merge_folded<<<dim3((unsigned)(((size_t)p.n_buckets * 32 + 127) / 128), p.n_calls), 128, 0, st>>>(p, ch, gp, pl->fold); launches++; }
     }
     CU(cudaEventRecord(q->ev1, st));
     CU(cudaGetLastError());
     CU(cudaStreamSynchronize(st));
-    int err[16];
-    CU(cudaMemcpy(err, q->d_err, 64, cudaMemcpyDeviceToHost));
+    int err[OG_ERR_INTS];
+    CU(cudaMemcpy(err, q->d_err, sizeof err, cudaMemcpyDeviceToHost));
     if (getenv("OGPU_IL_STATS")) {
         unsigned long long wait, life, pro, epi;
         memcpy(&wait, err + 8, 8); memcpy(&life, err + 10, 8); memcpy(&pro, err + 12, 8); memcpy(&epi, err + 14, 8);
@@ -880,6 +884,7 @@
                 err[4], err[5], err[6], err[7], wait, life, pc * (double)wait, pro, pc * (double)pro, epi, pc * (double)epi);
     }
     q->cells_dirty = err[2] != 0;
+    q->gcells_dirty = false;
     if (err[0]) { set_error("segment %d failed to decode (device code %d)", err[1], err[0]); return map_dev_err(err[0]); }
     float ms = 0; cudaEventElapsedTime(&ms, q->ev0, q->ev1);
     double main_ms = 0;
@@ -895,6 +900,7 @@
     if (p.n_cols == 1 && p.col_type[0] == OG_TYPE_FLOAT && p.col_index[0] < (int)s->il.size()) {
         const og_shard::IlCol &ic = s->il[p.col_index[0]];
         stt.il_state = ic.state; stt.il_build_ms = ic.build_ms; stt.il_bytes = ic.n_words * 4; stt.il_packed_segments = ic.state == 1 ? ic.n_packed : 0;
+        stt.il_uniform_groups = (uint32_t)err[OG_ERR_UNIFORM];
         stt.general_segments = ic.state == 1 ? (uint64_t)ic.gen_host.size() : s->n_segments;
     }
     stt.per_series_cells_used = err[2] != 0;
diff --git a/opengemini_b200/csrc/fused_il.cuh b/opengemini_b200/csrc/fused_il.cuh
--- a/opengemini_b200/csrc/fused_il.cuh
+++ b/opengemini_b200/csrc/fused_il.cuh
@@ -43,6 +43,10 @@
 #ifndef OG_IL_UNROLL
 #define OG_IL_UNROLL 2
 #endif
+#ifndef OG_IL_USTEP
+#define OG_IL_USTEP 8u
+#endif
+static_assert(OG_IL_USTEP % 2 == 0, "the uniform loop decodes record pairs");
 #define OG_IL_NB (OG_IL_NW / OG_IL_B)
 #define OG_IL_ROWS (OG_IL_NW + 2u)
 #define OG_IL_PAD_WORDS 6u
@@ -111,7 +115,7 @@
 #define OG_IL_WCAP 24u
 __host__ __device__ inline uint32_t il_acc_bytes(uint32_t n_calls, bool times) { return OG_IL_WCAP * n_calls * (times ? 17u : 9u) + 8u & ~7u; }
 
-template <int FM, bool TIMES, bool FOLD>
+template <int FM, bool TIMES, bool FOLD, bool UNI = false>
 __global__ void __maxnreg__(OG_FAST_MAXREG) k_fused_il(QueryP q, ChunkP ch, IlP il, uint32_t grp_begin, uint32_t grp_end) {
     constexpr uint32_t NW = OG_IL_NW, B = OG_IL_B, NB = OG_IL_NB, K = OG_IL_K;
     constexpr uint32_t FULL = 0xffffffffu;
@@ -164,7 +168,8 @@
         mbar_init_fence();
     }
     __syncwarp();
-    const uint32_t total_b = rows_w / B;
+    uint32_t total_b = rows_w / B;
+    uint32_t rows_cp = rows_w;
     uint64_t goff = il.grp_off[grp];
     goff = ((uint64_t)__reduce_max_sync(FULL, (uint32_t)(goff >> 32)) << 32) | __reduce_max_sync(FULL, (uint32_t)goff);
     const uint32_t *gsrc = il.words + goff;
@@ -176,15 +181,16 @@
         const uint32_t k = __reduce_max_sync(FULL, k_any);
         const uint32_t s = k % NB, dst = win + s * (B * 128), bar = bar0 + s * 8;
         const uint32_t *src = gsrc + (size_t)k * (B * 32);
+        const uint32_t left = rows_cp - k * B, bytes = (left < B ? left : B) * 128;
         if (s == 0)
             asm volatile("{\n.reg .pred p;\nelect.sync _|p, 0xffffffff;\n@p mbarrier.arrive.expect_tx.shared::cta.b64 _, [%0], %1;\n"
                          "@p cp.async.bulk.shared::cluster.global.mbarrier::complete_tx::bytes.L2::cache_hint [%2], [%3], %4, [%0], %6;\n"
                          "@p cp.async.bulk.shared::cluster.global.mbarrier::complete_tx::bytes.L2::cache_hint [%5], [%3], 256, [%0], %6;\n}"
-                         ::"r"(bar), "r"(B * 128 + 256u), "r"(dst), "l"(src), "r"(B * 128), "r"(win + NW * 128), "l"(pol) : "memory");
+                         ::"r"(bar), "r"(bytes + 256u), "r"(dst), "l"(src), "r"(bytes), "r"(win + NW * 128), "l"(pol) : "memory");
         else
             asm volatile("{\n.reg .pred p;\nelect.sync _|p, 0xffffffff;\n@p mbarrier.arrive.expect_tx.shared::cta.b64 _, [%0], %1;\n"
                          "@p cp.async.bulk.shared::cluster.global.mbarrier::complete_tx::bytes.L2::cache_hint [%2], [%3], %1, [%0], %4;\n}"
-                         ::"r"(bar), "r"(B * 128), "r"(dst), "l"(src), "l"(pol) : "memory");
+                         ::"r"(bar), "r"(bytes), "r"(dst), "l"(src), "l"(pol) : "memory");
     };
     {
         const uint32_t first = total_b < NB ? total_b : NB;
@@ -225,6 +231,13 @@
     }
     const uint32_t gcol = FOLD ? il.grp_col[grp] - ch.gc_col0 : 0;
     const bool fold_edges = FOLD && uni && b_end > b0;
+    constexpr bool UNI_LOOP = UNI && FOLD && !(FM == 63 && TIMES);
+    bool pku = false;
+    if (UNI_LOOP && uni) {
+        const int leader = __ffs(__ballot_sync(FULL, active)) - 1;
+        const uint32_t winL = __shfl_sync(FULL, lwin, leader), rowsL = __shfl_sync(FULL, rows, leader);
+        pku = __all_sync(FULL, !active || ((lwin & OG_IL_PACKED) && lwin == winL && rows == rowsL));
+    }
 
     double sum = 0.0, mn = 0.0, mx = 0.0; uint64_t fi = 0, lastv = 0;
     uint32_t n_mn = 0, n_mx = 0;
@@ -388,7 +401,75 @@
     uint32_t st_common = 0, st_rare = 0, st_sit = 0, st_notgo = 0;
     const long long st_pro = clock64() - st_clk0;
 #endif
-    for (;;) {
+
+    if (pku && !hung) {
+        const uint32_t lw = __reduce_max_sync(FULL, active ? lwin : 0u), rows_u = __reduce_max_sync(FULL, active ? rows : 0u);
+        const uint32_t mu = lw & 127u, lead = (lw >> 8) & 63u;
+        const uint64_t MU = mu ? (~0ull >> (64 - mu)) << (64 - lead - mu) : 0ull;
+        uint32_t qu = 64 - lead, row = 0;
+        {
+            const uint32_t last = ((64u - lead + (rows_u - 1) * mu) >> 5) + 3u;
+            rows_cp = last < rows_w ? last : rows_w;
+            const uint32_t tb = (rows_cp + B - 1) / B;
+            if (tb < total_b) total_b = tb;
+        }
+        auto run_rows = [&](uint32_t end, bool acc) {
+            constexpr uint32_t S = OG_IL_USTEP;
+            while (row < end && !hung) {
+                const uint32_t n = end - row < S ? end - row : S;
+                const uint32_t f = qu >> 5;
+#pragma unroll 1
+                while (issued_b < total_b && (issued_b + 1) * B <= f + NW) { issue(issued_b); issued_b++; }
+                uint32_t need = ((qu + (n - 1) * mu) >> 5) + 3u; if (need > rows_cp) need = rows_cp;
+                uint32_t want_b = (need + B - 1) / B; if (want_b > issued_b) want_b = issued_b;
+#ifdef OG_IL_STATS
+                st_w0 = clock64();
+#endif
+#pragma unroll 1
+                while (ready_b < want_b) { if (!mbar_wait(bar0 + (ready_b % NB) * 8, (ready_b / NB) & 1)) { hung = 1; break; } ready_b++; }
+#ifdef OG_IL_STATS
+                st_wait += clock64() - st_w0;
+#endif
+                if (hung) break;
+                if (n == S) {
+#pragma unroll
+                    for (uint32_t k = 0; k < S; k += 2) {
+                        const uint64_t x0 = fetch64(col, qu), x1 = fetch64(col, qu + mu);
+                        if (acc) accumulate(k);
+                        val ^= x0 & MU;
+                        if (acc) accumulate(k + 1);
+                        val ^= x1 & MU;
+                        qu += 2 * mu;
+                    }
+                } else {
+#pragma unroll 1
+                    for (uint32_t k = 0; k < n; k++) { const uint64_t x = fetch64(col, qu); if (acc) accumulate(k); val ^= x & MU; qu += mu; }
+                }
+                if (acc) n_ev -= n;
+                row += n;
+            }
+        };
+        if (__any_sync(FULL, active && skipping)) {
+            run_rows(__reduce_max_sync(FULL, active ? r_lo : 0u), false);
+            if (active) advance();
+        }
+        while (!hung && __any_sync(FULL, active && !done)) {
+            const uint32_t end = __reduce_max_sync(FULL, active && !done ? stop : 0u);
+            if (end <= row || rounds_left-- == 0) { hung = 2; break; }
+            run_rows(end, true);
+            if (hung) break;
+            const bool ev = active && !done;
+            const int kind = kind_of();
+            const bool to_acc = ev && (kind == 2 || fold_edges);
+            if (ev && !to_acc) flush_lane(kind);
+            if (__any_sync(FULL, to_acc)) flush_fold(to_acc);
+            if (to_acc && kind == 0) head_done = true;
+            if (ev) advance();
+        }
+        qp = qu;
+        if (lane == 0) atomicAdd((unsigned *)&ch.err[OG_ERR_UNIFORM], 1u);
+    }
+    if (!pku) for (;;) {
         const uint32_t qmin = __reduce_min_sync(FULL, done ? 0xffffffffu : qp);
         if (qmin == 0xffffffffu) break;
         const uint32_t f = qmin < 32 ? 0u : (qmin - 32) >> 5;
diff --git a/opengemini_b200/csrc/internal.h b/opengemini_b200/csrc/internal.h
--- a/opengemini_b200/csrc/internal.h
+++ b/opengemini_b200/csrc/internal.h
@@ -60,7 +60,8 @@
                    uint32_t n_groups = 0, J = 0;
                    bool aligned = false;
                    uint32_t n_super = 1, cols_per_super = 0; std::vector<uint32_t> super_grp_first;
-                   uint64_t n_words = 0, n_packed = 0;  double build_ms = 0; };
+                   uint64_t n_words = 0, n_packed = 0;  double build_ms = 0;
+                   bool all_packed = false;  };
     std::vector<IlCol> il;
     std::mutex il_mu;
 };
@@ -111,6 +112,7 @@
     std::vector<og_colval_view> rv_cols;
     int path_used = 0;
     bool cells_dirty = true;
+    bool gcells_dirty = true;
     bool planned = false;
     uint32_t chunk_series = 0, tile_segs = 0;
     int *d_err = nullptr;
```

New measurement: 498.5 billion, median of 6. +2.2%, better.
